# aschneuw/road-segmentation-unet

Measured on AMD Instinct MI355X. Metric: 388x388 patches/sec fwd+bwd (1/2/4/8 GPU) + conv MFMA % of peak, higher is better.
Workload: dtype bf16; 1 GPU; U-Net fwd+bwd+momentum step, num_layers=5 root_size=64 patch_size=388 input=572; batch_per_gpu=4, global_batch=4, parallelism=dp1

## Files before the change

### road_segmentation_unet_amd/_lib.py

```python
import ctypes
import os

_HERE = os.path.dirname(os.path.abspath(__file__))
LIB_PATH = os.environ.get("RSU_LIB_PATH") or os.path.join(_HERE, "librsu_hip.so")

_vp, _i, _l, _f, _sz, _u = ctypes.c_void_p, ctypes.c_int, ctypes.c_long, ctypes.c_float, ctypes.c_size_t, ctypes.c_uint


class RsuSrc(ctypes.Structure):
    _fields_ = [("ptr", _vp), ("H", _i), ("W", _i), ("C", _i), ("oy", _i), ("ox", _i)]


class RsuWgradJob(ctypes.Structure):
    _fields_ = [("kind", _i), ("src", RsuSrc), ("dz", _vp), ("dw", _vp), ("db", _vp), ("Ho", _i), ("Wo", _i),
                ("Cin_total", _i), ("ci_off", _i), ("Cout", _i), ("dil", _i)]


WGRAD_CONV3X3, WGRAD_CONVT2X2, WGRAD_GROUP_MAX = 0, 1, 16


class RsuPlanRow(ctypes.Structure):
    _fields_ = [(n, _i) for n in ("kind", "level", "Hin", "Win", "Cin", "Hout", "Wout", "Cout", "dilation", "nsrc")]


# ... 100 lines not shown
    "rsu_extract_tiles": (_i, [_vp, _vp, _i, _i, _i, _i, _i, _l, _l, _vp]),
    "rsu_overlap_add": (_i, [_vp, _vp, _vp, _i, _i, _i, _i, _l, _l, _vp]),
    "rsu_overlap_finish": (_i, [_vp, _vp, _vp, _l, _vp]),
    "rsu_tile_grid": (_i, [_i, _i, _i, _i, _PI, _PI]),
    "rsu_extract_tiles_rect": (_i, [_vp, _vp, _i, _i, _i, _i, _i, _i, _l, _l, _vp]),
    "rsu_overlap_add_rect": (_i, [_vp, _vp, _vp, _i, _i, _i, _i, _i, _l, _l, _vp]),
    "rsu_affine_patches": (_i, [_vp, _vp, ctypes.POINTER(RsuAffine), _i, _i, _i, _i, _i, _i, _vp, _vp, _vp]),
    "rsu_elastic_patches": (_i, [_vp, _vp, ctypes.POINTER(RsuElastic), _i, _i, _i, _i, _i, _i, _vp, _vp, _vp]),
    "rsu_color_jitter_ws_bytes": (_sz, [_i, _i]),
    "rsu_color_jitter": (_i, [_vp, ctypes.POINTER(RsuJitter), _i, _i, _vp, _vp]),
    "rsu_quantize_mask": (_i, [_vp, _vp, _i, _i, _i, _f, _vp]),
    "rsu_quantize_mask_rect": (_i, [_vp, _vp, _i, _i, _i, _i, _f, _vp]),
    "rsu_labels_for_patches": (_i, [_vp, _vp, _i, _i, _i, _f, _vp]),
    "rsu_confusion_counts": (_i, [_vp, _vp, _l, _vp, _vp]),
    "rsu_plan": (_i, [_i, _i, _i, _i, _i, ctypes.POINTER(RsuPlanRow), _i, _PI, ctypes.POINTER(RsuPlanTotals)]),
}

SIGNATURES_OPTIM = {
    "rsu_update_table_run_decay": (_i, [_vp, _i, _i, _f, _f, _f, _f, _i, _vp, _vp]),
    "rsu_update_table_run_adam_decay": (_i, [_vp, _i, _i, _f, _f, _f, _f, _f, _f, _i, _vp, _vp]),
}

SIGNATURES_LOSS = {
    "rsu_head_fwd_bwd_focal": (_i, [_vp, _vp, _vp, _vp, _vp, _vp, _f, _vp, _f, _f, _vp, _vp, _vp, _vp, _vp, _vp, _vp, _l, _i, _f, _vp]),
    "rsu_head_eval_focal": (_i, [_vp, _vp, _vp, _vp, _vp, _vp, _f, _vp, _vp, _vp, _vp, _l, _i, _vp]),
}

SIGNATURES_CLDICE = {
    "rsu_cldice_ws_floats": (_sz, [_i, _i, _i, _i]),
    "rsu_cldice_fwd": (_i, [_vp, _vp, _i, _vp, _vp, _vp, _vp, _i, _i, _i, _vp]),
    "rsu_cldice_bwd": (_i, [_vp, _vp, _vp, _vp, _vp, _i, _f, _f, _vp, _vp, _i, _i, _i, _vp]),
    "rsu_head_fwd_bwd_aux": (_i, [_vp, _vp, _vp, _vp, _vp, _vp, _f, _vp, _f, _f, _vp, _vp, _vp, _vp, _vp, _vp, _vp, _l, _i, _f, _vp, _vp]),
}

SIGNATURES_LOVASZ = {
    "rsu_lovasz_ws_bytes": (_sz, [_i, _i, _i]),
    "rsu_lovasz_fwd": (_i, [_vp, _vp, _vp, _vp, _i, _i, _i, _vp]),
    "rsu_lovasz_fwd_bwd": (_i, [_vp, _vp, _f, _i, _vp, _vp, _vp, _i, _i, _i, _vp]),
}

SIGNATURES_COMPONENTS = {
    "rsu_components_ws_bytes": (_sz, [_i, _i, _i]),
    "rsu_components_label": (_i, [_vp, _f, _i, _i, _vp, _vp, _vp, _vp, _i, _i, _i, _vp]),
    "rsu_components_filter": (_i, [_vp, _f, _i, _i, _i, _vp, _vp, _vp, _i, _i, _i, _vp]),
    "rsu_components_pair_count": (_i, [_vp, _f, _vp, _i, _vp, _vp, _i, _i, _i, _vp]),
}

SIGNATURES_DISTANCE = {
    "rsu_distance_ws_bytes": (_sz, [_i, _i, _i]),
    "rsu_mask_distance": (_i, [_vp, _f, _vp, _vp, _vp, _vp, _i, _i, _i, _vp]),
    "rsu_distance_hist": (_i, [_vp, _f, _vp, _vp, _vp, _i, _i, _i, _vp]),
}

_lib = None


class RsuError(RuntimeError):
    pass


def lib():
    global _lib
    if _lib is None:
        if not os.path.exists(LIB_PATH):
            raise RsuError("HIP extension missing: %s (build it with `python -c 'import __graft_entry__ as g; g.build()'` "
                           "or `make -C road_segmentation_unet_amd/csrc`); there is no fallback path" % LIB_PATH)
        L = ctypes.CDLL(LIB_PATH)
        for name, (res, args) in list(SIGNATURES.items()) + list(SIGNATURES_OPTIM.items()) + list(SIGNATURES_LOSS.items()) \
                + list(SIGNATURES_CLDICE.items()) + list(SIGNATURES_LOVASZ.items()) + list(SIGNATURES_COMPONENTS.items()) \
                + list(SIGNATURES_DISTANCE.items()):
            fn = getattr(L, name)
            fn.restype = res
            fn.argtypes = args
        _lib = L
    return _lib


TUNE_OFF, TUNE_LOOKUP, TUNE_MEASURE = 0, 1, 2
EVAL_BINS = 256
BORDER_D2_INF, BORDER_MAX_SIDE = 0x7fffffff, 1024
CLIP_STATE_BYTES, CLIP_CLIPPED, CLIP_NONFINITE, GRAD_NORM_BLOCK_FLOATS = 32, 1, 2, 16384
GRAD_ACCUMULATE_BLOCK_FLOATS = 8192
DECAY_L2, DECAY_DECOUPLED = 0, 1
AFFINE_MAX_LAUNCH = 32
ELASTIC_MAX_LAUNCH, ELASTIC_MAX_GRID = 32, 16
JITTER_MAX_LAUNCH = 32
CLDICE_MAX_ITERS = 16
DIST_BINS, DIST_NONE, DIST_MAX_SIDE = 64, 0x7fffffff, 1024
E2BIG = -7


def check(rc, what):
    if rc == E2BIG:
        raise RsuError("%s: a tensor of this call reaches 2 GiB (the kernels address tensors through 32-bit byte offsets): "
                       "use a smaller per-GPU batch" % what)
    if rc != 0:
        raise RsuError("%s failed: rc=%d (hip error %d)" % (what, rc, lib().rsu_last_hip_error()))


_TRACE = os.environ.get("RSU_TRACE", "0") == "1"


def call(name, *args):
    if _TRACE:
        import sys
        import torch
        print("[rsu]", name, [a if isinstance(a, (int, float)) else "." for a in args], file=sys.stderr, flush=True)
        check(getattr(lib(), name)(*args), name)
        torch.cuda.synchronize()
        return
    check(getattr(lib(), name)(*args), name)


_hip = None
_fork_rings = {}


def _hip_runtime():
    global _hip
    if _hip is None:
        path = "libamdhip64.so"
        try:
            with open("/proc/self/maps") as f:
# ... 42 lines not shown
```

### road_segmentation_unet_amd/csrc/conv_first.hip

```cpp
#include "igemm.h"

namespace {
__device__ __forceinline__ unsigned relu_pk(unsigned x) {
    typedef __attribute__((ext_vector_type(2))) short s2;
    return __builtin_bit_cast(unsigned, __builtin_elementwise_max(__builtin_bit_cast(s2, x), s2{0, 0}));
}
}

struct ConvFirstParams {
    const float* x;
    const float* cw;
    const float* cb;
    const bf16_t* in16;
    const bf16_t* wp;
    const float* bias;
    bf16_t* y;
    int N, H, W, Ho, Wo, Cout, dil, relu, ntiles_w;
    int ntx;
    unsigned ntx_magic, ho_magic;
    int npieces;
};

#ifndef CF_TRS
#define CF_TRS 1
#endif
template <bool FUSED>
__global__ void __launch_bounds__(256) __attribute__((amdgpu_waves_per_eu(3))) k_conv_first_fwd(const ConvFirstParams p) {
#if CF_TRS
    __shared__ __attribute__((aligned(16))) char trs[4 * 2048];
#endif
    const int lane = threadIdx.x & 63, l15 = lane & 15, g4 = lane >> 4;
    const int wave = __builtin_amdgcn_readfirstlane((int)(blockIdx.x * 4 + (threadIdx.x >> 6)));
    const int nwaves = gridDim.x * 4;
    const int cb = blockIdx.y;
    const __amdgpu_buffer_rsrc_t rin = __builtin_amdgcn_make_buffer_rsrc((void*)p.in16, 0, (int)((long)p.N * p.H * p.W * 32), 0x00020000);
    const __amdgpu_buffer_rsrc_t rout = __builtin_amdgcn_make_buffer_rsrc((void*)p.y, 0, 0x7fffffff, 0x00020000);
    bf16x8 fa[5][4];
#pragma unroll
    for (int j = 0; j < 5; ++j) {
        const int tap = 2 * j + (g4 >> 1);
#pragma unroll
        for (int ct = 0; ct < 4; ++ct) {
            const int tile = cb * 4 + ct;
            bf16x8 v = {0, 0, 0, 0, 0, 0, 0, 0};
            if (tap < 9 && tile < p.ntiles_w) v = *(const bf16x8*)(p.wp + ((long)(tap * p.ntiles_w + tile) * 64 + l15 + 16 * (g4 & 1)) * 8);
            fa[j][ct] = v;
        }
    }
    f32x4 binit[4];
#pragma unroll
    for (int ct = 0; ct < 4; ++ct)
#pragma unroll
        for (int i = 0; i < 4; ++i) {
            const int co = cb * 64 + (ct >> 1) * 32 + 8 * g4 + (ct & 1) * 4 + i;
            binit[ct][i] = (p.bias && co < p.Cout) ? p.bias[co] : 0.f;
        }
    unsigned voff[5];
#pragma unroll
    for (int j = 0; j < 5; ++j) {
        const int tap = min(2 * j + (g4 >> 1), 8), ky = tap / 3, kx = tap - 3 * ky;
        voff[j] = (unsigned)((((ky * p.W + kx) * p.dil + l15) * 16 + 8 * (g4 & 1)) * 2);
    }
    auto decode = [&](int t, int& n, int& y, int& x0) {
        unsigned row = __umulhi((unsigned)t, p.ntx_magic);
        int xt = t - (int)row * p.ntx;
        if (xt >= p.ntx) { ++row; xt -= p.ntx; }
        unsigned nn = __umulhi(row, p.ho_magic);
        int yy = (int)row - (int)nn * p.Ho;
        if (yy >= p.Ho) { ++nn; yy -= p.Ho; }
        n = (int)nn; y = yy; x0 = xt * 16;
    };
    typedef __attribute__((ext_vector_type(3))) float f32x3;
    const __amdgpu_buffer_rsrc_t rx = __builtin_amdgcn_make_buffer_rsrc((void*)p.x, 0, FUSED ? (int)((long)p.N * p.H * p.W * 12) : 0, 0x00020000);
    unsigned xoff[5];
#pragma unroll
    for (int j = 0; j < 5; ++j) {
        const int tap = min(2 * j + (g4 >> 1), 8), ky = tap / 3, kx = tap - 3 * ky;
        xoff[j] = (g4 & 1) ? 0x80000000u : (unsigned)(((ky * p.W + kx) * p.dil + l15) * 12);
    }
    auto load = [&](int t, bf16x8 (&fb)[5]) {
        int n, y, x0;
        decode(t, n, y, x0);
        if constexpr (FUSED) {
            const unsigned soff = (unsigned)(((long)(n * p.H + y) * p.W + x0) * 12);
#pragma unroll
            for (int j = 0; j < 5; ++j) {
                const f32x3 v = __builtin_bit_cast(f32x3, __builtin_amdgcn_raw_buffer_load_b96(rx, xoff[j], soff, 0));
                fb[j] = __builtin_bit_cast(bf16x8, f32x4{v[0], v[1], v[2], 0.f});
            }
// ... 15 lines not shown
#pragma unroll
            for (int j = 0; j < 5; ++j) {
                const f32x4 v = __builtin_bit_cast(f32x4, fb[j]);
                const float xc[3] = {v[0] - 0.5f, v[1] - 0.5f, v[2] - 0.5f};
                float f[3];
#pragma unroll
                for (int c = 0; c < 3; ++c) f[c] = fmaf(xc[2], cw[6 + c], fmaf(xc[1], cw[3 + c], fmaf(xc[0], cw[c], cbias[c])));
                const u32x4 o = {pack_bf2(f[0], f[1]), pack_bf2(f[2], 0.f), 0u, 0u};
                fb[j] = (g4 & 1) ? bf16x8{0, 0, 0, 0, 0, 0, 0, 0} : __builtin_bit_cast(bf16x8, o);
            }
        }
    };
    int t = wave;
    if (t >= p.npieces) return;
    bf16x8 fb[5], fbn[5];
    load(t, fb);
    while (true) {
        const int tn = t + nwaves;
        const bool more = tn < p.npieces;
        load(more ? tn : t, fbn);
        f32x4 acc[4];
#pragma unroll
        for (int ct = 0; ct < 4; ++ct) acc[ct] = binit[ct];
        convert(fb);
#pragma unroll
        for (int j = 0; j < 5; ++j)
#pragma unroll
            for (int ct = 0; ct < 4; ++ct) acc[ct] = __builtin_amdgcn_mfma_f32_16x16x32_bf16(fa[j][ct], fb[j], acc[ct], 0, 0, 0);
        int n, y, x0;
        decode(t, n, y, x0);
        const unsigned sbase = (unsigned)((((long)(n * p.Ho + y) * p.Wo + x0) * p.Cout + cb * 64) * 2);
#if CF_TRS
        {
            __attribute__((address_space(3))) char* wl = (__attribute__((address_space(3))) char*)trs + (threadIdx.x >> 6) * 2048;
#pragma unroll
            for (int pp = 0; pp < 2; ++pp) {
                u32x4 r = {pack_bf2(acc[2 * pp][0], acc[2 * pp][1]), pack_bf2(acc[2 * pp][2], acc[2 * pp][3]),
                           pack_bf2(acc[2 * pp + 1][0], acc[2 * pp + 1][1]), pack_bf2(acc[2 * pp + 1][2], acc[2 * pp + 1][3])};
                if (p.relu) {
#pragma unroll
                    for (int i = 0; i < 4; ++i) r[i] = relu_pk(r[i]);
                }
                *(__attribute__((address_space(3))) u32x4*)(wl + l15 * 128 + (((pp * 4 + g4) ^ (l15 & 7)) << 4)) = r;
            }
            asm volatile("s_waitcnt lgkmcnt(0)" ::: "memory");
            const int q8 = lane & 7;
#pragma unroll
            for (int h = 0; h < 2; ++h) {
                const int P = (lane >> 3) + 8 * h;
                const u32x4 r = *(const __attribute__((address_space(3))) u32x4*)(wl + P * 128 + ((q8 ^ (P & 7)) << 4));
                const bool ok = (x0 + P < p.Wo) && (cb * 64 + q8 * 8 < p.Cout);
                const unsigned vo = ok ? (unsigned)((P * p.Cout + q8 * 8) * 2) : 0x80000000u;
                asm volatile("s_waitcnt lgkmcnt(0)\n\ts_nop 4\n\tbuffer_store_dwordx4 %0, %1, %2, %3 offen\n\ts_nop 3" ::"v"(r), "v"(vo), "s"(rout), "s"(sbase) : "memory");
            }
        }
#else
        const bool pok = x0 + l15 < p.Wo;
#pragma unroll
        for (int pp = 0; pp < 2; ++pp) {
            u32x4 r = {pack_bf2(acc[2 * pp][0], acc[2 * pp][1]), pack_bf2(acc[2 * pp][2], acc[2 * pp][3]),
                       pack_bf2(acc[2 * pp + 1][0], acc[2 * pp + 1][1]), pack_bf2(acc[2 * pp + 1][2], acc[2 * pp + 1][3])};
            if (p.relu) {
#pragma unroll
                for (int i = 0; i < 4; ++i) r[i] = relu_pk(r[i]);
            }
            const bool cok = cb * 64 + pp * 32 + 8 * g4 < p.Cout;
            const unsigned vo = (pok && cok) ? (unsigned)((l15 * p.Cout + pp * 32 + 8 * g4) * 2) : 0x80000000u;
            asm volatile("s_nop 4\n\tbuffer_store_dwordx4 %0, %1, %2, %3 offen\n\ts_nop 3" ::"v"(r), "v"(vo), "s"(rout), "s"(sbase) : "memory");
        }
#endif
        if (!more) break;
        t = tn;
#pragma unroll
        for (int j = 0; j < 5; ++j) fb[j] = fbn[j];
    }
}

static unsigned floor_magic(int d) { return d <= 1 ? 0xffffffffu : (unsigned)(0x100000000ull / (unsigned)d); }

hipError_t conv_first_fwd_launch(const void* in16, const void* wp, int ntiles_w, const float* bias, void* y, int N, int H, int W, int Cout, int dil,
                                 int relu, int ncu, hipStream_t st, const float* x, const float* cw, const float* cb) {
    ConvFirstParams p;
    p.x = x; p.cw = cw; p.cb = cb;
    p.in16 = (const bf16_t*)in16; p.wp = (const bf16_t*)wp; p.bias = bias; p.y = (bf16_t*)y;
    p.N = N; p.H = H; p.W = W; p.Ho = H - 2 * dil; p.Wo = W - 2 * dil; p.Cout = Cout; p.dil = dil; p.relu = relu; p.ntiles_w = ntiles_w;
    p.ntx = (p.Wo + 15) / 16;
    p.ntx_magic = floor_magic(p.ntx);
    p.ho_magic = floor_magic(p.Ho);
    const long np = (long)N * p.Ho * p.ntx;
    if (np >= (1l << 31) / 2 || p.Ho < 1 || p.Wo < 1) return hipErrorInvalidValue;
    p.npieces = (int)np;
    long blocks = (long)ncu * 3;
    if (blocks * 4 > np) blocks = (np + 3) / 4;
    if (x) hipLaunchKernelGGL(k_conv_first_fwd<true>, dim3((unsigned)blocks, (unsigned)((Cout + 63) / 64)), dim3(256), 0, st, p);
    else hipLaunchKernelGGL(k_conv_first_fwd<false>, dim3((unsigned)blocks, (unsigned)((Cout + 63) / 64)), dim3(256), 0, st, p);
    return hipGetLastError();
}
```

### road_segmentation_unet_amd/csrc/igemm.h

```cpp
#pragma once
#include "rsu_common.h"

struct IgSrc {
    const bf16_t* ptr;
    int H, W, C;
    int oy, ox;
};

struct IgFwdParams {
    IgSrc src[3];
    int nsrc;
    int nchunk[3];
    const bf16_t* wp;
    long wp_y_stride;
    int ntiles_w;
    int tile_off;
    const float* bias;
    bf16_t* out;
    const bf16_t* mask_src;
    bf16_t* pool_out;
    unsigned char* pool_code;
    const void* zero_page;
    int N, Hin, Win;
    int Ho, Wo;
    int Cout;
    int outC;
    int dil, stride, pad;
    int oH, oW, ostride;
    int relu, accumulate;
    int ncob;
    int lsw;
    int ksplit, cob_group;
    float* kslab;
    long kslab_stride;
    int dbg;
    unsigned* stamps;
    TileGeo g;
};

struct IgFwdCfgInfo { int TN, TM, threads; };
enum { IGF2_CFG_128x256 = 0, IGF2_CFG_64x512 = 1, IGF2_CFG_128x128 = 2, IGF2_CFG_64x256 = 3, IGF2_CFG_128x192 = 4, IGF2_CFG_64x384 = 5,
       IGF2_CFG_128x320 = 6, IGF2_CFG_64x640 = 7, IGF2_NCFG = 8 };
IgFwdCfgInfo igemm_fwd2_cfg_info(int cfg);
int igemm_fwd2_max_pieces(int cfg, int ntap);
size_t igemm_fwd2_lds_bytes(int cfg, int ntap, int npix_max);
hipError_t igemm_fwd2_launch(int cfg, int ntap, const IgFwdParams& p, int grid_x, int grid_y, hipStream_t st);
hipError_t igemm_pp_launch(int cfg, const IgFwdParams& p, int grid_x, hipStream_t st);
hipError_t igemm_pp_d2_launch(int cfg, const IgFwdParams& p, int grid_x, hipStream_t st);
bool igemm_pp_d2_supports(int cfg, const IgFwdParams& p);
bool igemm_pp_has(int cfg);
bool igemm_pp_has_ksplit(int cfg);
bool igemm_pp_supports(int cfg, const IgFwdParams& p);
int igemm_pp_pool_lsw_mask(int cfg);
size_t igemm_pp_slab_floats(int cfg, const IgFwdParams& p);
hipError_t igemm_pp_finish_launch(int cfg, const IgFwdParams& p, hipStream_t st);

struct IgCtParams {
    const bf16_t* a;
    int Ca;
    int nchunk;
    int N, H, W;
    unsigned magic_hw, magic_w;
    const bf16_t* wp;
    long wp_phase_stride;
    int ntiles_w;
    const float* bias;
    bf16_t* out;
    int outC;
    int Cn;
    const bf16_t* mask_src;
    int ncob, nnb;
};
bool igemm_ct_supports(int mode, int N, int H, int W, int Ca, int Cn);
hipError_t igemm_ct_launch(int mode, const IgCtParams& p, int grid_x, hipStream_t st);
hipError_t conv_first_fwd_launch(const void* in16, const void* wp, int ntiles_w, const float* bias, void* y, int N, int H, int W, int Cout, int dil,
                                 int relu, int ncu, hipStream_t st, const float* x = nullptr, const float* cw = nullptr, const float* cb = nullptr);

struct IgWgradParams {
    const bf16_t* F;
    int Hf, Wf, Cf;
    IgSrc S;
    float* slab;
    float* bslab;
    float* sbslab;
    long slab_stride;
    int CsOut, CfOut, cs_off;
    const void* zero_page;
    int N, dil, stride;
    int nsplit, ntiles_total;
    int lsw;
    int nbuf, nsw;
    int dbg;
    TileGeo g;
};
enum { IGW_CFG_64x64 = 0, IGW_CFG_64x16 = 1, IGW_CFG_128x64 = 2, IGW_NCFG = 3 };
size_t igemm_wgrad_lds_bytes(int cfg, int npix_max, int nbuf);
int igemm_wgrad_nsw(int cfg, int npix_max);
int igemm_wgrad_tmk(int cfg);
int igemm_wgrad_cfb(int cfg);
int igemm_wgrad_csb(int cfg);
int igemm_wgrad_kgroups(int cfg);
hipError_t igemm_wgrad_launch(int cfg, int ntap, const IgWgradParams& p, int grid_x, int grid_y, int grid_z,
                              hipStream_t st);
bool igemm_wgt_supports(int N, int H, int W, int Cin, int Cout);
int igemm_wgt_blocks(int Cin, int Cout);
int igemm_wgt_tiles(int N, int H, int W);
hipError_t igemm_wgt_launch(const void* x, const void* dy, float* slab, float* sbslab, long slab_stride, int N, int H, int W, int Cin, int Cout,
                            int nsplit, hipStream_t st);
bool igemm_wg1_supports(int N, int H, int W, int Cout, int dil);
int igemm_wg1_blocks(int Cout);
int igemm_wg1_tiles(int N, int Ho, int Wo);
hipError_t igemm_wg1_launch(const void* in16, const void* dz, float* slab, float* bslab, long slab_stride, int N, int H, int W, int Cout, int dil,
                            int nsplit, hipStream_t st);
enum { IGW_FAM_WGPP3 = 0, IGW_FAM_WGPP4 = 1, IGW_FAM_WGPP5 = 2, IGW_FAM_WGPP6 = 3, IGW_FAM_WGP64_4 = 4, IGW_FAM_WGP64_5 = 5,
       IGW_FAM_GENERIC = 8  };
#define IGW_GROUP_MAX 16
#define IGW_UNITS_MAX 2048
struct IgWgJob {
    IgWgradParams p;
    int gx, gy, gz;
    int family;
    int pad_;
};
struct IgWgGroupParams {
    int njobs, nwg;
    IgWgJob job[IGW_GROUP_MAX];
    int wg_first[257];
    unsigned unit[IGW_UNITS_MAX];
};
// ... 9 lines not shown
```

### road_segmentation_unet_amd/csrc/igemm_fwd2.hip

```cpp
#include <type_traits>

#include "igemm.h"

#define RSU_WAIT_VMCNT(N) asm volatile("s_waitcnt vmcnt(%0)" ::"n"(N) : "memory")

template <int SPC, int WPS, int NA, int DA, int DW>
__device__ __forceinline__ constexpr int vm_allowed(int j) {
    return SPC == 1 ? WPS + (DA - 1) * (NA + WPS) : (j == 0 ? (DW - 1) * WPS : (DW - 1) * WPS + NA);
}

__device__ __forceinline__ void bdma16(__amdgpu_buffer_rsrc_t rsrc, unsigned voff, unsigned soff, void* lds_wave_base) {
    __builtin_amdgcn_raw_ptr_buffer_load_lds(rsrc, (__attribute__((address_space(3))) void*)lds_wave_base, 16, voff, soff, 0, 0);
}
__device__ __forceinline__ unsigned relu_pk_bf16(unsigned x) {
    typedef __attribute__((ext_vector_type(2))) short s2;
    s2 h = __builtin_bit_cast(s2, x);
    h = __builtin_elementwise_max(h, s2{0, 0});
    return __builtin_bit_cast(unsigned, h);
}
#define RSU_SENT 0x80000000u

template <int WCO, int WPX, int CT, int PT, int NTAP, int KW, int TPS, int NA, int NAB, int DWS>
__global__ void __launch_bounds__(WCO* WPX * 64) __attribute__((amdgpu_waves_per_eu(WCO* WPX / 4, WCO* WPX / 4)))
igemm_fwd2_kernel(const IgFwdParams p) {
    constexpr int NW = WCO * WPX;
    static_assert(NW == 8, "eight waves: two per SIMD");
    constexpr int TN = WCO * CT * 16, TM = WPX * PT * 16;
    constexpr int WT = TN / 16;
    constexpr int SPC = NTAP / TPS;
    constexpr int WBUF = TPS * WT * 1024;
    constexpr int DA = NAB - 1, DW = DWS;
    constexpr int NWB = DW + 1;
    constexpr int WPS = (TPS * WT + NW - 1) / NW;
    constexpr int NST = (CT / 2) * PT;
    static_assert(NTAP % TPS == 0 && (CT % 2) == 0 && SPC <= 3, "bad config");
    static_assert(SPC == 1 || NAB == 2, "deep halo rings only for one-stage-per-chunk kernels");
    static_assert(SPC == 1 ? DW == NAB : (DW >= 2 && DW <= SPC), "weight distance");
    extern __shared__ __attribute__((aligned(16))) char smem[];
    __attribute__((address_space(3))) char* lds = (__attribute__((address_space(3))) char*)smem;
    const int ABUF = p.g.npix_max * 64;
    const int a_base = NWB * WBUF;
    const int dummy_base = a_base + NAB * ABUF;

    const int lane = threadIdx.x & 63;
    const int wave = __builtin_amdgcn_readfirstlane(threadIdx.x >> 6);
    const int wco = wave / WPX, wpx = wave % WPX;
    const int g4 = lane >> 4, l15 = lane & 15;
    const int SW = p.g.SW, CW = p.g.CW, lsw = p.lsw, TR = TM >> lsw;
    const int ph = blockIdx.y;
    const bf16_t* wp = p.wp + (long)ph * p.wp_y_stride;
    const int ooffy = ph >> 1, ooffx = ph & 1;

    int vid = blockIdx.x;
    if (!(p.dbg & 64)) {
        const int q = gridDim.x >> 3, r = gridDim.x & 7, x = vid & 7;
        vid = (x < r ? x * (q + 1) : r * (q + 1) + (x - r) * q) + (vid >> 3);
    }
    const int cob = vid % p.ncob;
    const int tile0 = vid / p.ncob, tstride = gridDim.x / p.ncob;
    const int tpi = p.g.nstrips * p.g.tiles_per_strip;
    const int ntile_m = p.N * tpi;
    const int my_tiles = tile0 < ntile_m ? (ntile_m - tile0 + tstride - 1) / tstride : 0;
    if (my_tiles == 0) return;
    const int nchunks = p.nchunk[0] + p.nchunk[1] + p.nchunk[2];
    const int GC = my_tiles * nchunks;

    struct Tile { int n, x0, y0; };
    auto decode = [&](int k) {
        Tile T;
        int t = tile0 + k * tstride;
        T.n = t / tpi;
        t -= T.n * tpi;
        const int strip = t / p.g.tiles_per_strip;
        T.x0 = strip * SW;
        T.y0 = (t - strip * p.g.tiles_per_strip) * TR;
// ... 75 lines not shown
            a_voff[q] = ok ? (unsigned)(((rr * sW + cc) * sC + kg8) * 2) : RSU_SENT;
        }
    };
    auto issue_a = [&]() {
        const __amdgpu_buffer_rsrc_t rs = mk(a_ptr);
        const int dst = a_base + ia_slot * ABUF;
        ia_slot = ia_slot == NAB - 1 ? 0 : ia_slot + 1;
        if (a_crem >= 32) {
#pragma unroll
            for (int q = 0; q < NA; ++q) {
                const int j = q * NW + wave;
                bdma16(rs, a_voff[q], a_soff, (void*)(lds + (j < npieces ? dst + j * 1024 : dummy_base)));
            }
        } else {
#pragma unroll
            for (int q = 0; q < NA; ++q) {
                const int j = q * NW + wave;
                const int hp = j * 16 + lq;
                const int kg8 = ((lane & 3) ^ ((hp >> 1) & 2)) * 8;
                bdma16(rs, kg8 < a_crem ? a_voff[q] : RSU_SENT, a_soff, (void*)(lds + (j < npieces ? dst + j * 1024 : dummy_base)));
            }
        }
        a_soff += 64;
        a_crem -= 32;
        a_cl = a_cl + 1 == nchunks ? 0 : a_cl + 1;
    };

    const int bias_base = dummy_base + 1024;
    if (threadIdx.x < TN) {
        const int co = cob * TN + threadIdx.x;
        const float bvv = (p.bias && co < p.Cout) ? p.bias[co] : 0.f;
        *(__attribute__((address_space(3))) float*)(lds + bias_base + threadIdx.x * 4) = bvv;
    }
    asm volatile("s_waitcnt vmcnt(0)" ::: "memory");
    __syncthreads();

    auto out_sbase = [&](const Tile& T) {
        return (unsigned)((((long)(T.n * p.oH + T.y0 * p.ostride + ooffy) * p.oW + T.x0 * p.ostride + ooffx) * p.outC + cob * TN +
                           wco * (CT / 2) * 32) * 2);
    };
    auto out_voff = [&](const Tile& T, int e) {
        const int pt = e / (CT / 2), pp = e % (CT / 2);
        const int ml = (wpx * PT + pt) * 16 + l15;
        const int ty = ml >> lsw, tx = ml & (SW - 1);
        const bool pok = (T.y0 + ty < p.Ho) && (T.x0 + tx < p.Wo);
        const int ovoff_pt = ((ty * p.ostride * p.oW + tx * p.ostride) * p.outC + 8 * g4) * 2;
        const int co = cob * TN + (wco * (CT / 2) + pp) * 32 + 8 * g4;
        return (pok && co < p.Cout) ? (unsigned)(ovoff_pt + pp * 64) : RSU_SENT;
    };
    auto epilogue = [&](const Tile& T, f32x4(&acc)[CT][PT]) {
        const __amdgpu_buffer_rsrc_t orsrc = mk(p.out);
        const __amdgpu_buffer_rsrc_t mrsrc = mk(p.mask_src ? (const void*)p.mask_src : (const void*)p.out);
        const unsigned sbase = out_sbase(T);
        if (!p.accumulate) {
            typedef __attribute__((ext_vector_type(2))) short s2;
            const short fl = p.relu ? (short)0 : (short)-32768;
            const s2 floor2 = {fl, fl};
            unsigned ones_pk = 0x00010001u;
            asm volatile("" : "+v"(ones_pk));
            constexpr int MB = NST % 4 == 0 ? 4 : 2;
#pragma unroll
            for (int b0 = 0; b0 < NST; b0 += MB) {
                unsigned voffs[MB];
                u32x4 mk4[MB];
#pragma unroll
                for (int e = 0; e < MB; ++e) {
                    voffs[e] = out_voff(T, b0 + e);
                    if (p.mask_src) mk4[e] = __builtin_amdgcn_raw_buffer_load_b128(mrsrc, voffs[e], sbase, 0);
                }
#pragma unroll
                for (int e = 0; e < MB; ++e) {
                    const int pt = (b0 + e) / (CT / 2), pp = (b0 + e) % (CT / 2);
                    u32x4 r;
#pragma unroll
                    for (int i = 0; i < 2; ++i) {
                        const unsigned lo = pack_bf2(acc[2 * pp][pt][2 * i], acc[2 * pp][pt][2 * i + 1]);
                        const unsigned hi = pack_bf2(acc[2 * pp + 1][pt][2 * i], acc[2 * pp + 1][pt][2 * i + 1]);
                        r[i] = __builtin_bit_cast(unsigned, __builtin_elementwise_max(__builtin_bit_cast(s2, lo), floor2));
                        r[2 + i] = __builtin_bit_cast(unsigned, __builtin_elementwise_max(__builtin_bit_cast(s2, hi), floor2));
                    }
                    if (p.mask_src) {
#pragma unroll
                            for (int i = 0; i < 4; ++i) r[i] &= pos_mask_pk_bf16(mk4[e][i], ones_pk);
                    }
                    asm volatile("buffer_store_dwordx4 %0, %1, %2, %3 offen\n\ts_nop 3" ::"v"(r), "v"(voffs[e]), "s"(orsrc), "s"(sbase) : "memory");
                }
                if (p.mask_src) __builtin_amdgcn_sched_barrier(0);
            }
            return;
        }
        constexpr int EB = NST % 4 == 0 ? 4 : 2;
        static_assert(NST % EB == 0, "epilogue batches");
#pragma unroll
        for (int b0 = 0; b0 < NST; b0 += EB) {
            unsigned voffs[EB];
            u32x4 mk4[EB], ob4[EB];
#pragma unroll
            for (int e = 0; e < EB; ++e) {
                voffs[e] = out_voff(T, b0 + e);
                if (p.mask_src) mk4[e] = __builtin_amdgcn_raw_buffer_load_b128(mrsrc, voffs[e], sbase, 0);
                if (p.accumulate) ob4[e] = __builtin_amdgcn_raw_buffer_load_b128(orsrc, voffs[e], sbase, 0);
            }
#pragma unroll
            for (int e = 0; e < EB; ++e) {
                const int pt = (b0 + e) / (CT / 2), pp = (b0 + e) % (CT / 2);
                float v[8];
#pragma unroll
                for (int i = 0; i < 4; ++i) {
                    v[i] = acc[2 * pp][pt][i];
                    v[4 + i] = acc[2 * pp + 1][pt][i];
                }
                if (p.mask_src) {
#pragma unroll
                    for (int i = 0; i < 4; ++i) {
                        if (!(bf_lo(mk4[e][i]) > 0.f)) v[2 * i] = 0.f;
                        if (!(bf_hi(mk4[e][i]) > 0.f)) v[2 * i + 1] = 0.f;
                    }
                }
                if (p.accumulate) {
#pragma unroll
                    for (int i = 0; i < 4; ++i) {
                        v[2 * i] += bf_lo(ob4[e][i]);
                        v[2 * i + 1] += bf_hi(ob4[e][i]);
                    }
                }
                unsigned r0 = pack_bf2(v[0], v[1]), r1 = pack_bf2(v[2], v[3]), r2 = pack_bf2(v[4], v[5]), r3 = pack_bf2(v[6], v[7]);
                if (p.relu) {
                    r0 = relu_pk_bf16(r0);
                    r1 = relu_pk_bf16(r1);
                    r2 = relu_pk_bf16(r2);
                    r3 = relu_pk_bf16(r3);
                }
                const u32x4 r = {r0, r1, r2, r3};
                asm volatile("buffer_store_dwordx4 %0, %1, %2, %3 offen\n\ts_nop 3" ::"v"(r), "v"(voffs[e]), "s"(orsrc), "s"(sbase)
                             : "memory");
            }
            __builtin_amdgcn_sched_barrier(0);
        }
    };

    Tile ptile = decode(0);
    int pk = 0;
    setup_a(ptile, 0);
    a_next_src = p.nchunk[0];
    bool a_started = false;
    auto issue_a_next = [&]() {
        if (a_cl == 0) {
            if (a_started) {
                ++pk;
                ptile = decode(pk);
                a_si = 0;
                a_next_src = p.nchunk[0];
                setup_a(ptile, 0);
            }
        } else if (a_cl == a_next_src) {
            ++a_si;
            a_next_src += a_si == 1 ? p.nchunk[1] : p.nchunk[2];
            setup_a(ptile, a_si);
        }
        a_started = true;
        issue_a();
    };
    if constexpr (SPC == 1) {
#pragma unroll
        for (int k = -DW; k < 0; ++k) {
            if (k + DA >= 0 && k + DA < GC) issue_a_next();
            if (k + DW < GC) issue_w();
        }
    } else {
        issue_w();
// ... 122 lines not shown
};
template <> struct Fwd2Cfg<IGF2_CFG_128x320> {
    static constexpr int WCO = 2, WPX = 4, CT = 4, PT = 5;
    static constexpr int na(int ntap) { return ntap == 1 ? 3 : 5; }
};
template <> struct Fwd2Cfg<IGF2_CFG_64x640> {
    static constexpr int WCO = 1, WPX = 8, CT = 4, PT = 5;
    static constexpr int na(int ntap) { return ntap == 1 ? 5 : 7; }
};

static constexpr int tps2_for(int TN, int ntap) { return ntap == 9 ? 3 : (ntap == 4 ? (TN <= 64 ? 4 : 2) : 1); }
static constexpr int nab_for(int TN, int ntap) { return ntap / tps2_for(TN, ntap) == 1 ? 4 : 2; }
static constexpr int dws_for(int TN, int ntap, int PT) { return ntap / tps2_for(TN, ntap) == 1 ? nab_for(TN, ntap) : 2; }

IgFwdCfgInfo igemm_fwd2_cfg_info(int cfg) {
    switch (cfg) {
#define CASE(C) \
    case C: return IgFwdCfgInfo{Fwd2Cfg<C>::WCO * Fwd2Cfg<C>::CT * 16, Fwd2Cfg<C>::WPX * Fwd2Cfg<C>::PT * 16, Fwd2Cfg<C>::WCO * Fwd2Cfg<C>::WPX * 64};
        CASE(IGF2_CFG_128x256)
        CASE(IGF2_CFG_64x512)
        CASE(IGF2_CFG_128x128)
        CASE(IGF2_CFG_64x256)
        CASE(IGF2_CFG_128x192)
        CASE(IGF2_CFG_64x384)
        CASE(IGF2_CFG_128x320)
        CASE(IGF2_CFG_64x640)
#undef CASE
    }
    return IgFwdCfgInfo{0, 0, 0};
}
int igemm_fwd2_max_pieces(int cfg, int ntap) {
    switch (cfg) {
#define CASE(C) case C: return Fwd2Cfg<C>::na(ntap) * Fwd2Cfg<C>::WCO * Fwd2Cfg<C>::WPX;
        CASE(IGF2_CFG_128x256)
        CASE(IGF2_CFG_64x512)
        CASE(IGF2_CFG_128x128)
        CASE(IGF2_CFG_64x256)
        CASE(IGF2_CFG_128x192)
        CASE(IGF2_CFG_64x384)
        CASE(IGF2_CFG_128x320)
        CASE(IGF2_CFG_64x640)
#undef CASE
    }
    return 0;
}
size_t igemm_fwd2_lds_bytes(int cfg, int ntap, int npix_max) {
    const IgFwdCfgInfo ci = igemm_fwd2_cfg_info(cfg);
    const int tps = tps2_for(ci.TN, ntap), nab = nab_for(ci.TN, ntap);
    const int pt = ci.TM / 16 / (ci.threads / 64 / (ci.TN / 64));
    const int dws = dws_for(ci.TN, ntap, pt);
    return (size_t)(dws + 1) * tps * (ci.TN / 16) * 1024 + (size_t)nab * npix_max * 64 + 1024 + 512;
}

template <int CFG, int NTAP, int KW>
static hipError_t launch2_one(const IgFwdParams& p, int gx, int gy, hipStream_t st) {
    using C = Fwd2Cfg<CFG>;
    constexpr int TN = C::WCO * C::CT * 16;
    constexpr int TPS = tps2_for(TN, NTAP);
    auto kern = igemm_fwd2_kernel<C::WCO, C::WPX, C::CT, C::PT, NTAP, KW, TPS, C::na(NTAP), nab_for(TN, NTAP), dws_for(TN, NTAP, C::PT)>;
    const size_t lds = igemm_fwd2_lds_bytes(CFG, NTAP, p.g.npix_max);
    static size_t lds_set = 0;
    if (lds > lds_set) {
        hipError_t e = hipFuncSetAttribute((const void*)kern, hipFuncAttributeMaxDynamicSharedMemorySize, (int)lds);
        if (e != hipSuccess) return e;
        lds_set = lds;
    }
    hipLaunchKernelGGL(kern, dim3(gx, gy), dim3(C::WCO * C::WPX * 64), lds, st, p);
    return hipGetLastError();
}
template <int CFG>
static hipError_t launch2_cfg(int ntap, const IgFwdParams& p, int gx, int gy, hipStream_t st) {
    switch (ntap) {
        case 9: return launch2_one<CFG, 9, 3>(p, gx, gy, st);
        case 4: return launch2_one<CFG, 4, 2>(p, gx, gy, st);
        case 1: return launch2_one<CFG, 1, 1>(p, gx, gy, st);
    }
    return hipErrorInvalidValue;
}
hipError_t igemm_fwd2_launch(int cfg, int ntap, const IgFwdParams& p, int gx, int gy, hipStream_t st) {
    switch (cfg) {
        case IGF2_CFG_128x256: return launch2_cfg<IGF2_CFG_128x256>(ntap, p, gx, gy, st);
        case IGF2_CFG_64x512: return launch2_cfg<IGF2_CFG_64x512>(ntap, p, gx, gy, st);
        case IGF2_CFG_128x128: return launch2_cfg<IGF2_CFG_128x128>(ntap, p, gx, gy, st);
        case IGF2_CFG_64x256: return launch2_cfg<IGF2_CFG_64x256>(ntap, p, gx, gy, st);
        case IGF2_CFG_128x192: return launch2_cfg<IGF2_CFG_128x192>(ntap, p, gx, gy, st);
        case IGF2_CFG_64x384: return launch2_cfg<IGF2_CFG_64x384>(ntap, p, gx, gy, st);
        case IGF2_CFG_128x320: return launch2_cfg<IGF2_CFG_128x320>(ntap, p, gx, gy, st);
        case IGF2_CFG_64x640: return launch2_cfg<IGF2_CFG_64x640>(ntap, p, gx, gy, st);
    }
    return hipErrorInvalidValue;
}
```

### road_segmentation_unet_amd/csrc/igemm_pp.hip

```cpp
#include <cstring>
#include <type_traits>

#include "igemm.h"

#ifndef PP_CLIP_PAD
#define PP_CLIP_PAD 1
#endif
#ifndef PP_DIL
#define PP_DIL 1
#endif

#define RSU_WAIT_VMCNT(N) asm volatile("s_waitcnt vmcnt(%0)" ::"n"(N) : "memory")
#define RSU_SENT 0x80000000u

namespace {
__device__ __forceinline__ void bdma16(__amdgpu_buffer_rsrc_t rsrc, unsigned voff, unsigned soff, void* lds_wave_base) {
    __builtin_amdgcn_raw_ptr_buffer_load_lds(rsrc, (__attribute__((address_space(3))) void*)lds_wave_base, 16, voff, soff, 0, 0);
}
__device__ __forceinline__ unsigned relu_pk_bf16(unsigned x) {
    typedef __attribute__((ext_vector_type(2))) short s2;
    s2 h = __builtin_bit_cast(s2, x);
    h = __builtin_elementwise_max(h, s2{0, 0});
    return __builtin_bit_cast(unsigned, h);
}
}

#define PP_NSTAMP 640
namespace {
constexpr int pp_na_slot(int NAW, int k) { return (NAW >> (4 * k)) & 15; }
constexpr int pp_na(int NAW, int g, int j) { return g == 0 ? pp_na_slot(NAW, 2 * j) : (j < 2 ? pp_na_slot(NAW, 2 * j + 1) : 0); }
constexpr int pp_na_first(int NAW, int g, int j) {
    int n = 0;
    for (int k = 0; k < (g == 0 ? 2 * j : 2 * j + 1); ++k) n += pp_na_slot(NAW, k);
    return n;
}
constexpr int pp_na_total(int NAW, int g) { return pp_na(NAW, g, 0) + pp_na(NAW, g, 1) + pp_na(NAW, g, 2); }
constexpr int pp_na_idx(int NAW, int g, int j) {
    int n = 0;
    for (int k = 0; k < j; ++k) n += pp_na(NAW, g, k);
    return n;
}
}
template <int WCO, int WPX, int CT, int PT, int LSW, int NAW, int WP0, bool STAMP, bool DBG, bool POOLK = false, bool KS = false, int DIL = PP_DIL>
__global__ void __launch_bounds__(512) __attribute__((amdgpu_waves_per_eu(2, 2)))
igemm_pp_kernel(const IgFwdParams p) {
    constexpr int NW = 8, NG = 4, KW = 3, TPS = 3;
    static_assert(WCO * WPX == NW, "eight waves: two per SIMD");
    constexpr int TN = WCO * CT * 16, TM = WPX * PT * 16;
    constexpr int WT = TN / 16;
    constexpr int WBUF = TPS * WT * 1024;
    constexpr int NWB = 3, NAB = 2;
    constexpr int WP1 = TPS * WT / 4 - WP0;
    constexpr int WPM = WP1 > WP0 ? WP1 : (WP0 > 0 ? WP0 : 1);
    constexpr int NAV = pp_na_total(NAW, 0) > pp_na_total(NAW, 1) ? pp_na_total(NAW, 0) : pp_na_total(NAW, 1);
    static_assert((WP0 + WP1) * 4 == TPS * WT && WP0 >= 0 && WP1 >= 1, "weight pieces per stage");
    constexpr int NST = (CT / 2) * PT;
    static_assert((CT % 2) == 0, "bad config");
    extern __shared__ __attribute__((aligned(16))) char smem[];
    __attribute__((address_space(3))) char* lds = (__attribute__((address_space(3))) char*)smem;
    constexpr int SW = 1 << LSW, lsw = LSW, TR = TM >> LSW;
    constexpr int CW = (SW + 2 * DIL + 7) / 8 * 8;
    constexpr int NPIX = ((TR + 2 * DIL) * CW + 31) / 32 * 32;
    constexpr int ABUF = NPIX * 64;
    constexpr int ROWB = DIL * CW * 64;
    constexpr int a_base = 0;
    constexpr int WBASE = NAB * ABUF;
    constexpr int dummy_base = WBASE + NWB * WBUF;
    static_assert(ABUF + 2 * ROWB < 65536, "halo offsets must fit the 16-bit offset field of ds_read");

    const int lane = threadIdx.x & 63;
    const int wave = __builtin_amdgcn_readfirstlane(threadIdx.x >> 6);
    const int grp = wave >> 2, w4 = wave & 3;
    const int wco = wave / WPX, wpx = wave % WPX;
    const int g4 = lane >> 4, l15 = lane & 15;

    auto sgpr = [](int v) { return __builtin_amdgcn_readfirstlane(v); };
    int vid = blockIdx.x;
    {
        const int q = gridDim.x >> 3, r = gridDim.x & 7, x = vid & 7;
        vid = (x < r ? x * (q + 1) : r * (q + 1) + (x - r) * q) + (vid >> 3);
    }
    const int ksplit = (KS && p.ksplit > 1) ? p.ksplit : 1;
    const int nck = p.ncob * ksplit;
    const int cgrp = (p.cob_group > 0 && p.cob_group < nck) ? p.cob_group : nck;
    const int tstride = sgpr(gridDim.x / nck);
    const int u_in = vid % cgrp, u_r = vid / cgrp;
    const int unit = sgpr((u_r / tstride) * cgrp + u_in);
    const int tile0 = sgpr(u_r % tstride);
    const int cob = sgpr(unit % p.ncob), ks = KS ? sgpr(unit / p.ncob) : 0;
    const int tpi = p.g.nstrips * p.g.tiles_per_strip;
    const int ntile_m = p.N * tpi;
    const int my_tiles = (unit < nck && tile0 < ntile_m) ? (ntile_m - tile0 + tstride - 1) / tstride : 0;
    if (my_tiles == 0) return;
    const int nchunks = p.nchunk[0] + p.nchunk[1] + p.nchunk[2];
    const int c_lo = KS ? sgpr(ks * nchunks / ksplit) : 0, c_hi = KS ? sgpr((ks + 1) * nchunks / ksplit) : nchunks;
    const int nloc = c_hi - c_lo;
// ... 171 lines not shown
    const int stamp_base = bias_base + 512;
    int stamp_i = 0;
    unsigned long long seg_sum[8] = {0, 0, 0, 0, 0, 0, 0, 0}, seg_t0 = 0;
    auto seg_begin = [&]() {
        if constexpr (STAMP) seg_t0 = __builtin_amdgcn_s_memtime();
    };
    auto seg_end = [&](int k) {
        if constexpr (STAMP) {
            const unsigned long long t = __builtin_amdgcn_s_memtime();
            seg_sum[k] += t - seg_t0;
            seg_t0 = t;
        }
    };
    auto stamp = [&]() {
        if constexpr (STAMP) {
            if (stamp_i < PP_NSTAMP - 10) {
                const unsigned t = (unsigned)__builtin_amdgcn_s_memtime();
                if (lane == 0) *(__attribute__((address_space(3))) unsigned*)(lds + stamp_base + (wave * PP_NSTAMP + stamp_i) * 4) = t;
            }
            ++stamp_i;
        }
    };
    if (threadIdx.x < TN) {
        const int co = cob * TN + threadIdx.x;
        const float bvv = (p.bias && co < p.Cout && ks == 0) ? p.bias[co] : 0.f;
        *(__attribute__((address_space(3))) float*)(lds + bias_base + threadIdx.x * 4) = bvv;
    }
    asm volatile("s_waitcnt vmcnt(0)" ::: "memory");

    auto out_sbase = [&](const Tile& T) {
        return (unsigned)((((long)(T.n * p.oH + T.y0) * p.oW + T.x0) * p.outC + cob * TN + wco * (CT / 2) * 32) * 2);
    };
    auto out_voff = [&](const Tile& T, int e, const int ql15, const int qg4) {
        const int pt = e / (CT / 2), pp = e % (CT / 2);
        const int ml = (wpx * PT + pt) * 16 + ql15;
        const int ty = ml >> lsw, tx = ml & (SW - 1);
        const bool pok = (T.y0 + ty < p.Ho) && (T.x0 + tx < p.Wo);
        const int ovoff_pt = ((ty * p.oW + tx) * p.outC + 8 * qg4) * 2;
        const int co = cob * TN + (wco * (CT / 2) + pp) * 32 + 8 * qg4;
        return (pok && co < p.Cout) ? (unsigned)(ovoff_pt + pp * 64) : RSU_SENT;
    };
#define PP_STORE(R, VOFF) \
    asm volatile("s_nop 4\n\tbuffer_store_dwordx4 %0, %1, %2, %3 offen\n\ts_nop 3" ::"v"(R), "v"(VOFF), "s"(orsrc), "s"(sbase) : "memory")
#define PP_STORE64(R, VOFF) \
    asm volatile("s_nop 4\n\tbuffer_store_dwordx4 %0, %1, %2, %3 offen offset:64\n\ts_nop 3" ::"v"(R), "v"(VOFF), "s"(orsrc), "s"(sbase) : "memory")
    unsigned ovoff[PT];
#pragma unroll
    for (int pt = 0; pt < PT; ++pt) {
        const int ml = (wpx * PT + pt) * 16 + l15;
        const int ty = ml >> lsw, tx = ml & (SW - 1);
        ovoff[pt] = (unsigned)(((ty * p.oW + tx) * p.outC + 8 * g4) * 2);
    }
    const bool co_inside = cob * TN + TN <= p.Cout;
    constexpr bool POOL_OK = POOLK && ((PT == 4 && (LSW == 4 || LSW == 5)) || (PT == 2 && LSW == 4));
    auto pool_body = [&](const Tile& T, f32x4(&acc)[CT][PT], const unsigned (&voffs)[NST], const __amdgpu_buffer_rsrc_t orsrc, const unsigned sbase)
                         __attribute__((always_inline)) {
        typedef __attribute__((ext_vector_type(2))) short s2;
        typedef __attribute__((ext_vector_type(2))) unsigned short us2;
        constexpr int NPAIR = PT / 2, PSTEP = (LSW == 5) ? 2 : 1;
        const int pH = p.oH >> 1, pW = p.oW >> 1;
        const __amdgpu_buffer_rsrc_t prsrc = mk(p.pool_out);
        const __amdgpu_buffer_rsrc_t crsrc = mk(p.pool_code ? (const void*)p.pool_code : (const void*)p.pool_out);
        const unsigned psbase = (unsigned)((((long)(T.n * pH + (T.y0 >> 1)) * pW + (T.x0 >> 1)) * p.outC + cob * TN + wco * (CT / 2) * 32) * 2);
        const short fl = p.relu ? (short)0 : (short)-32768;
        const s2 floor2 = {fl, fl};
        auto pk = [&](int ct2, int pt) {
            u32x4 r;
#pragma unroll
            for (int i = 0; i < 2; ++i) {
                const unsigned lo = pack_bf2(acc[ct2][pt][2 * i], acc[ct2][pt][2 * i + 1]);
                const unsigned hi = pack_bf2(acc[ct2 + 1][pt][2 * i], acc[ct2 + 1][pt][2 * i + 1]);
                r[i] = __builtin_bit_cast(unsigned, __builtin_elementwise_max(__builtin_bit_cast(s2, lo), floor2));
                r[2 + i] = __builtin_bit_cast(unsigned, __builtin_elementwise_max(__builtin_bit_cast(s2, hi), floor2));
            }
            return r;
        };
        auto swap1 = [](unsigned v) { return (unsigned)__builtin_amdgcn_mov_dpp((int)v, 0xB1, 0xF, 0xF, true); };
        auto umin1 = [](unsigned v) {
            const us2 one = {1, 1};
            return __builtin_bit_cast(unsigned, __builtin_elementwise_min(__builtin_bit_cast(us2, v), one));
        };
        auto sub16 = [](unsigned a, unsigned b) { return __builtin_bit_cast(unsigned, (us2)(__builtin_bit_cast(us2, a) - __builtin_bit_cast(us2, b))); };
        auto mul16 = [](unsigned a, unsigned b) { return __builtin_bit_cast(unsigned, (us2)(__builtin_bit_cast(us2, a) * __builtin_bit_cast(us2, b))); };
        auto add16 = [](unsigned a, unsigned b) { return __builtin_bit_cast(unsigned, (us2)(__builtin_bit_cast(us2, a) + __builtin_bit_cast(us2, b))); };
#pragma unroll
        for (int q = 0; q < NPAIR; ++q) {
            const int pa = (LSW == 5) ? q : 2 * q, pb = pa + PSTEP;
            const int ml = (wpx * PT + pa) * 16 + l15;
            const int ty = ml >> lsw, tx = ml & (SW - 1);
            const bool pok = ((l15 & 1) == 0) && (T.y0 + ty < p.Ho) && (T.x0 + tx < p.Wo);
            const unsigned pvoff = (unsigned)((((ty >> 1) * pW + (tx >> 1)) * p.outC + 8 * g4) * 2);
#pragma unroll
            for (int pp = 0; pp < CT / 2; ++pp) {
                const u32x4 ra = pk(2 * pp, pa), rb = pk(2 * pp, pb);
                PP_STORE(ra, voffs[pa * (CT / 2) + pp]);
                PP_STORE(rb, voffs[pb * (CT / 2) + pp]);
                u32x4 pooled;
                unsigned cw[4];
#pragma unroll
                for (int i = 0; i < 4; ++i) {
                    const unsigned v00 = ra[i], v10 = rb[i], v01 = swap1(ra[i]), v11 = swap1(rb[i]);
                    const unsigned mv = __builtin_bit_cast(unsigned, __builtin_elementwise_max(__builtin_bit_cast(s2, v00), __builtin_bit_cast(s2, v10)));
                    const unsigned mh = __builtin_bit_cast(unsigned, __builtin_elementwise_max(__builtin_bit_cast(s2, v01), __builtin_bit_cast(s2, v11)));
                    const unsigned mx = __builtin_bit_cast(unsigned, __builtin_elementwise_max(__builtin_bit_cast(s2, mv), __builtin_bit_cast(s2, mh)));
                    pooled[i] = mx;
                    const unsigned g = umin1(v00) | (umin1(v01) << 1) | (umin1(v10) << 2) | (umin1(v11) << 3);
// ... 5 lines not shown
                const unsigned pv = (pok && cok) ? pvoff + pp * 64 : RSU_SENT;
                asm volatile("s_nop 4\n\tbuffer_store_dwordx4 %0, %1, %2, %3 offen\n\ts_nop 3" ::"v"(pooled), "v"(pv), "s"(prsrc), "s"(psbase) : "memory");
                if (p.pool_code) {
                    u32x2 cd = {__builtin_amdgcn_perm(cw[1], cw[0], 0x06040200u), __builtin_amdgcn_perm(cw[3], cw[2], 0x06040200u)};
                    const unsigned cv = (pok && cok) ? (pvoff + pp * 64) >> 1 : RSU_SENT;
                    asm volatile("s_nop 4\n\tbuffer_store_dwordx2 %0, %1, %2, %3 offen\n\ts_nop 3" ::"v"(cd), "v"(cv), "s"(crsrc), "s"(psbase >> 1) : "memory");
                }
            }
        }
    };
    auto epilogue = [&](const Tile& T, const int tidx, f32x4(&acc)[CT][PT]) {
        if constexpr (KS) {
            const unsigned long long kaddr = (unsigned long long)(p.kslab + (long)ks * p.kslab_stride);
            const __amdgpu_buffer_rsrc_t krsrc = mk((const void*)(((unsigned long long)(unsigned)sgpr((int)(kaddr >> 32)) << 32) | (unsigned)sgpr((int)kaddr)));
            const unsigned kbase = (unsigned)sgpr((((tidx * p.ncob + cob) * NW + wave) * NST) * 2048);
            const unsigned kvoff = (unsigned)lane * 16u;
#pragma unroll
            for (int e = 0; e < NST; ++e) {
                const int pt = e / (CT / 2), pp = e % (CT / 2);
                asm volatile("s_nop 4\n\tbuffer_store_dwordx4 %0, %1, %2, %3 offen\n\ts_nop 3" ::"v"(acc[2 * pp][pt]), "v"(kvoff), "s"(krsrc),
                             "s"(kbase + (unsigned)(e * 2048)) : "memory");
                asm volatile("s_nop 4\n\tbuffer_store_dwordx4 %0, %1, %2, %3 offen\n\ts_nop 3" ::"v"(acc[2 * pp + 1][pt]), "v"(kvoff), "s"(krsrc),
                             "s"(kbase + (unsigned)(e * 2048 + 1024)) : "memory");
            }
            return;
        }
        const __amdgpu_buffer_rsrc_t orsrc = mk(p.out);
        const __amdgpu_buffer_rsrc_t mrsrc = mk(p.mask_src ? (const void*)p.mask_src : (const void*)p.out);
        const unsigned sbase = out_sbase(T);
        const bool inside = co_inside && (T.y0 + TR <= p.Ho) && (T.x0 + SW <= p.Wo);
        {
            typedef __attribute__((ext_vector_type(2))) short s2;
            const short fl = p.relu ? (short)0 : (short)-32768;
            const s2 floor2 = {fl, fl};
            unsigned voffs[NST];
            auto fill_voffs = [&](const bool tr) __attribute__((always_inline)) {
                const int ql15 = tr ? (lane >> 2) : l15, qg4 = tr ? (lane & 3) : g4;
                if (inside) {
#pragma unroll
                    for (int e = 0; e < NST; ++e) {
                        const int pt = e / (CT / 2);
                        unsigned o = ovoff[pt];
                        if (tr) {
                            const int ml = (wpx * PT + pt) * 16 + ql15;
                            o = (unsigned)((((ml >> lsw) * p.oW + (ml & (SW - 1))) * p.outC + 8 * qg4) * 2);
                        }
                        voffs[e] = o + (e % (CT / 2)) * 64;
                    }
                } else {
#pragma unroll
                    for (int e = 0; e < NST; ++e) voffs[e] = out_voff(T, e, ql15, qg4);
                }
            };
            auto body = [&](const bool MASK) __attribute__((always_inline)) {
                const bool TRS = MASK;
                const int tr_src = (((lane & 3) << 4) | (lane >> 2)) << 2;
                fill_voffs(TRS);
                seg_end(6);
                unsigned ones_pk = 0x00010001u;
                asm volatile("" : "+v"(ones_pk));
                u32x4 mk4[NST];
                if (MASK) {
#pragma unroll
                    for (int e = 0; e < NST; ++e)
                        asm volatile("buffer_load_dwordx4 %0, %1, %2, %3 offen" : "=&v"(mk4[e]) : "v"(voffs[e]), "s"(mrsrc), "s"(sbase) : "memory");
                }
                const int LA = TRS ? (NST < 8 ? NST : 8) : 1;
                u32x4 rr[NST];
                auto pack = [&](const int e) __attribute__((always_inline)) {
                    const int pt = e / (CT / 2), pp = e % (CT / 2);
                    unsigned q[4];
#pragma unroll
                    for (int i = 0; i < 2; ++i) {
                        const unsigned lo = pack_bf2(acc[2 * pp][pt][2 * i], acc[2 * pp][pt][2 * i + 1]);
                        const unsigned hi = pack_bf2(acc[2 * pp + 1][pt][2 * i], acc[2 * pp + 1][pt][2 * i + 1]);
                        q[i] = __builtin_bit_cast(unsigned, __builtin_elementwise_max(__builtin_bit_cast(s2, lo), floor2));
                        q[2 + i] = __builtin_bit_cast(unsigned, __builtin_elementwise_max(__builtin_bit_cast(s2, hi), floor2));
                    }
                    if (TRS) {
#pragma unroll
                        for (int i = 0; i < 4; ++i) asm volatile("ds_bpermute_b32 %0, %1, %2" : "=v"(q[i]) : "v"(tr_src), "v"(q[i]));
                    }
                    rr[e] = u32x4{q[0], q[1], q[2], q[3]};
                };
#pragma unroll
                for (int e = 0; e < NST; ++e) {
                    if (e == 0) {
#pragma unroll
                        for (int k = 0; k < LA; ++k) pack(k);
                        if (MASK) {
                            asm volatile("s_waitcnt vmcnt(0)" ::: "memory");
#pragma unroll
                            for (int k = 0; k < NST; ++k) asm volatile("" : "+v"(mk4[k]));
                        }
                    } else if (e + LA - 1 < NST) {
                        pack(e + LA - 1);
                    }
                    u32x4 r = rr[e];
                    if (TRS) {
                        const int ahead = (e + LA < NST ? e + LA : NST) - e - 1;
                        asm volatile("s_waitcnt lgkmcnt(%1)" : "+v"(r) : "n"(4 * ahead < 15 ? 4 * ahead : 15));
                    }
                    if (MASK) {
#pragma unroll
                        for (int i = 0; i < 4; ++i) r[i] &= pos_mask_pk_bf16(mk4[e][i], ones_pk);
                    }
                    if (DBG && (p.dbg & 512)) {
                        asm volatile("" ::"v"(r));
                    } else {
                        PP_STORE(r, voffs[e]);
                    }
                }
            };
            if constexpr (POOL_OK) {
                if (p.pool_out) {
                    fill_voffs(false);
                    pool_body(T, acc, voffs, orsrc, sbase);
                    return;
                }
            }
            if (p.mask_src) body(true); else body(false);
            return;
        }
    };
    auto bar = [&]() {
        asm volatile("" ::: "memory");
        __builtin_amdgcn_s_barrier();
        asm volatile("" ::: "memory");
    };

    setup_a(ptile, src_lo, coff_lo);
    a_next_src = next_rel;
    a_begin();
    if (!(DBG && (p.dbg & 2))) {
        if (grp) {
            a_pieces(std::integral_constant<int, 1>{}, std::integral_constant<int, 0>{});
            a_pieces(std::integral_constant<int, 1>{}, std::integral_constant<int, 1>{});
        } else {
            a_pieces(std::integral_constant<int, 0>{}, std::integral_constant<int, 0>{});
            a_pieces(std::integral_constant<int, 0>{}, std::integral_constant<int, 1>{});
            a_pieces(std::integral_constant<int, 0>{}, std::integral_constant<int, 2>{});
        }
    }
    a_end();
    if (!(DBG && (p.dbg & 1))) {
        if (grp) {
            issue_w(std::integral_constant<int, 1>{}, 0);
            issue_w(std::integral_constant<int, 1>{}, 1);
        } else {
            issue_w(std::integral_constant<int, 0>{}, 0);
            issue_w(std::integral_constant<int, 0>{}, 1);
        }
    }
    asm volatile("s_waitcnt vmcnt(0) lgkmcnt(0)" ::: "memory");
    bar();
    if (grp) bar();

    unsigned long long clk0 = 0, rt0 = 0;
    if constexpr (STAMP) {
        clk0 = __builtin_amdgcn_s_memtime();
        rt0 = __builtin_amdgcn_s_memrealtime();
    }
    f32x4 acc[CT][PT];
    auto run_stream = [&](auto gconst) {
        constexpr int G = decltype(gconst)::value;
        int c = 0;
        int ck = 0;
        Pos cpos = split(tile0);
        Tile ctile = tile_at(cpos);
        bf16x8 fa[TPS][CT], fb[TPS][PT];
        auto bias_init = [&]() {
            if (!(DBG && (p.dbg & 16))) {
                const unsigned baddr = (unsigned)(bias_base + (wco * (CT / 2) * 32 + 8 * g4) * 4);
#pragma unroll
                for (int ct = 0; ct < CT; ++ct)
#pragma unroll
                    for (int pt = 0; pt < PT; ++pt)
                        asm volatile("ds_read_b128 %0, %1 offset:%2" : "=v"(acc[ct][pt]) : "v"(baddr), "n"(((ct >> 1) * 32 + (ct & 1) * 4) * 4) : "memory");
            }
        };
        auto r_reads = [&](auto parc, auto jc) {
            constexpr int PAR = decltype(parc)::value, J = decltype(jc)::value;
            seg_begin();
            if (!(DBG && (p.dbg & 32))) {
#pragma unroll
                for (int tl = 0; tl < TPS; ++tl) {
#pragma unroll
                    for (int ct = 0; ct < CT; ++ct)
                        fa[tl][ct] = *(const __attribute__((address_space(3))) bf16x8*)(lds + afrag + J * WBUF + (tl * WT + ct) * 1024);
#pragma unroll
                    for (int pt = 0; pt < PT; ++pt)
                        fb[tl][pt] = *(const __attribute__((address_space(3))) bf16x8*)(lds + boff[pt][tl] + (a_base + PAR * ABUF + J * ROWB));
                }
            }
            seg_end(3);
        };
        auto r_issue = [&](auto jc, const bool after_epi) {
            constexpr int J = decltype(jc)::value;
            if constexpr (pp_na(NAW, G, J) > 0 || J == 0) {
                if (!(DBG && (p.dbg & 2))) {
                    if constexpr (J == 0) {
                        a_begin();
                        seg_end(7);
                    }
                    a_pieces(gconst, jc);
                }
            }
            if constexpr (J == 2) a_end();
            if constexpr ((G ? WP1 : WP0) > 0) {
                if (!(DBG && (p.dbg & 1))) issue_w(gconst, (J + 2) % NWB);
            }
            seg_end(4);
            if constexpr (G == 1) {
                if (J == 0 && after_epi) {
                    RSU_WAIT_VMCNT(pp_na(NAW, 1, J) + WP1 + NST);
                } else {
                    RSU_WAIT_VMCNT(pp_na(NAW, 1, J) + WP1);
                }
            }
        };
        auto r_part = [&](auto parc, auto jc, const bool after_epi) {
            r_reads(parc, jc);
            r_issue(jc, after_epi);
            asm volatile("s_waitcnt lgkmcnt(0)" ::: "memory");
            seg_end(5);
        };
        auto m_part = [&](auto jc, const bool after_epi, const bool last_of_tile) {
            constexpr int J = decltype(jc)::value;
            __builtin_amdgcn_sched_barrier(0);
            __builtin_amdgcn_s_setprio(1);
            if (!(DBG && (p.dbg & 32)))
#pragma unroll
            for (int tl = 0; tl < TPS; ++tl)
#pragma unroll
                for (int pt = 0; pt < PT; ++pt)
#pragma unroll
                    for (int ct = 0; ct < CT; ++ct) mfma_bf16_inplace(acc[ct][pt], fa[tl][ct], fb[tl][pt]);
            __builtin_amdgcn_s_setprio(0);
            __builtin_amdgcn_sched_barrier(0);
            if constexpr (G == 0) {
                if (J == 0 && after_epi) {
                    RSU_WAIT_VMCNT(pp_na(NAW, 0, J) + WP0 + NST);
                } else if (J == 2) {
                    RSU_WAIT_VMCNT(WP0);
                } else {
                    RSU_WAIT_VMCNT(pp_na(NAW, 0, J) + WP0);
                }
            }
            if (J == 2 && last_of_tile) mfma_results_fence();
        };
        auto chunk = [&](auto parc, int gc) {
            constexpr int PAR = decltype(parc)::value;
            const bool after_epi = (c == 0) && gc > 0;
            const bool last_of_tile = c == nloc - 1;
            if (!(G == 0 && after_epi)) {
                seg_begin();
                if (c == 0) bias_init();
                seg_end(2);
                r_part(parc, std::integral_constant<int, 0>{}, after_epi);
                stamp();
                bar();
                stamp();
            }
            m_part(std::integral_constant<int, 0>{}, after_epi, last_of_tile);
            stamp();
            bar();
            stamp();
            r_part(parc, std::integral_constant<int, 1>{}, false);
            stamp();
            bar();
            stamp();
            m_part(std::integral_constant<int, 1>{}, false, last_of_tile);
            stamp();
            bar();
            stamp();
            r_part(parc, std::integral_constant<int, 2>{}, false);
            stamp();
            bar();
            stamp();
            m_part(std::integral_constant<int, 2>{}, false, last_of_tile);
            stamp();
            bar();
            stamp();
            if (last_of_tile) {
                const bool more = ck + 1 < my_tiles;
                if constexpr (G == 0) {
                    if (more) r_issue(std::integral_constant<int, 0>{}, false);
                    stamp();
                    bar();
                    stamp();
                }
                seg_begin();
                if (!(DBG && (p.dbg & 8))) epilogue(ctile, KS ? (cpos.n * p.g.nstrips + cpos.strip) * p.g.tiles_per_strip + cpos.row : 0, acc);
                seg_end(0);
                if constexpr (G == 0) {
// ... 6 lines not shown
#pragma unroll
                        for (int tl = 0; tl < TPS; ++tl) {
#pragma unroll
                            for (int ct = 0; ct < CT; ++ct) fa[tl][ct] = bf16x8{0, 0, 0, 0, 0, 0, 0, 0};
#pragma unroll
                            for (int pt = 0; pt < PT; ++pt) fb[tl][pt] = bf16x8{0, 0, 0, 0, 0, 0, 0, 0};
                        }
                    }
                }
                stamp();
                bar();
                stamp();
                c = 0;
                ++ck;
                if (ck < my_tiles && !(DBG && (p.dbg & 64))) {
                    advance(cpos);
                    ctile = tile_at(cpos);
                }
                seg_end(1);
            } else {
                ++c;
            }
        };
        for (int gc = 0; gc < GC; gc += 2) {
            chunk(std::integral_constant<int, 0>{}, gc);
            if (gc + 1 >= GC) break;
            chunk(std::integral_constant<int, 1>{}, gc + 1);
        }
    };
    if (grp) run_stream(std::integral_constant<int, 1>{}); else run_stream(std::integral_constant<int, 0>{});
    asm volatile("s_waitcnt vmcnt(0)" ::: "memory");
    if constexpr (STAMP) {
        if (p.stamps) {
            asm volatile("s_waitcnt vmcnt(0) lgkmcnt(0)" ::: "memory");
            const unsigned dclk = (unsigned)(__builtin_amdgcn_s_memtime() - clk0), drt = (unsigned)(__builtin_amdgcn_s_memrealtime() - rt0);
            for (int i = lane; i < PP_NSTAMP; i += 64)
                p.stamps[((long)blockIdx.x * NW + wave) * PP_NSTAMP + i] =
                    i == PP_NSTAMP - 2 ? dclk : (i == PP_NSTAMP - 1 ? drt :
                    (i >= PP_NSTAMP - 10 && i < PP_NSTAMP - 2) ? (unsigned)seg_sum[i - (PP_NSTAMP - 10)] :
                    (i < stamp_i ? *(__attribute__((address_space(3))) unsigned*)(lds + stamp_base + (wave * PP_NSTAMP + i) * 4) : 0u));
        }
    }
}

#if PP_DIL == 1
struct PpFinishParams {
    const float* slab;
    long slice_stride;
    int ksplit, nslots, ncob;
    int WCO, WPX, CT, PT, lsw, TR;
    int nstrips, tiles_per_strip;
    bf16_t* out;
    const bf16_t* mask_src;
    int Ho, Wo, oH, oW, outC, Cout, relu;
};
__global__ void __launch_bounds__(256) k_pp_splitk_finish(const PpFinishParams q) {
    const int NST = (q.CT / 2) * q.PT, TN = q.WCO * q.CT * 16;
    const long idx = (long)blockIdx.x * 256 + threadIdx.x;
    const int lane = (int)(idx & 63);
    long r = idx >> 6;
    const int e = (int)(r % NST); r /= NST;
    const int wave = (int)(r & 7); r >>= 3;
    const int slot = (int)r;
    if (slot >= q.nslots) return;
    const float* src = q.slab + ((long)(slot * 8 + wave) * NST + e) * 512 + lane * 4;
    f32x4 a = *(const f32x4*)src, b = *(const f32x4*)(src + 256);
    for (int z = 1; z < q.ksplit; ++z) {
        const float* sz = src + (long)z * q.slice_stride;
        a += *(const f32x4*)sz;
        b += *(const f32x4*)(sz + 256);
    }
    const int cob = slot % q.ncob, t = slot / q.ncob;
    const int tpi = q.nstrips * q.tiles_per_strip;
    const int n = t / tpi, tr = t - n * tpi;
    const int strip = tr / q.tiles_per_strip, row = tr - strip * q.tiles_per_strip;
    const int wco = wave / q.WPX, wpx = wave % q.WPX;
    const int pt = e / (q.CT / 2), pp = e % (q.CT / 2);
    const int g4 = lane >> 4, l15 = lane & 15;
    const int ml = (wpx * q.PT + pt) * 16 + l15;
    const int SW = 1 << q.lsw;
    const int y = row * q.TR + (ml >> q.lsw), x = strip * SW + (ml & (SW - 1));
    const int co = cob * TN + (wco * (q.CT / 2) + pp) * 32 + 8 * g4;
    if (y >= q.Ho || x >= q.Wo || co >= q.Cout) return;
    typedef __attribute__((ext_vector_type(2))) short s2;
    const short fl = q.relu ? (short)0 : (short)-32768;
    const s2 floor2 = {fl, fl};
    auto pk = [&](float lo, float hi) {
        return __builtin_bit_cast(unsigned, __builtin_elementwise_max(__builtin_bit_cast(s2, pack_bf2(lo, hi)), floor2));
    };
    u32x4 v = {pk(a[0], a[1]), pk(a[2], a[3]), pk(b[0], b[1]), pk(b[2], b[3])};
    const long off = (((long)n * q.oH + y) * q.oW + x) * q.outC + co;
    if (q.mask_src) {
        const u32x4 m = *(const u32x4*)(q.mask_src + off);
#pragma unroll
        for (int i = 0; i < 4; ++i) v[i] &= pos_mask_pk_bf16(m[i]);
    }
    *(u32x4*)(q.out + off) = v;
}

#endif
template <int CFG> struct PpCfg;
#define PP_NAS(a, b, c, d, e) ((a) | ((b) << 4) | ((c) << 8) | ((d) << 12) | ((e) << 16))
template <> struct PpCfg<IGF2_CFG_128x256> { static constexpr int WCO = 2, WPX = 4, CT = 4, PT = 4, NAS = PP_NAS(0, 2, 3, 1, 2), WP0 = 2; };
template <> struct PpCfg<IGF2_CFG_64x512> { static constexpr int WCO = 1, WPX = 8, CT = 4, PT = 4, NAS = PP_NAS(0, 4, 4, 2, 2), WP0 = 0; };
template <> struct PpCfg<IGF2_CFG_128x128> { static constexpr int WCO = 2, WPX = 4, CT = 4, PT = 2, NAS = PP_NAS(0, 1, 2, 1, 2), WP0 = 2; };
template <> struct PpCfg<IGF2_CFG_64x256> { static constexpr int WCO = 1, WPX = 8, CT = 4, PT = 2, NAS = PP_NAS(0, 2, 3, 1, 2), WP0 = 0; };
template <> struct PpCfg<IGF2_CFG_128x192> { static constexpr int WCO = 2, WPX = 4, CT = 4, PT = 3, NAS = PP_NAS(0, 2, 3, 1, 2), WP0 = 2; };
template <> struct PpCfg<IGF2_CFG_64x384> { static constexpr int WCO = 1, WPX = 8, CT = 4, PT = 3, NAS = PP_NAS(0, 3, 3, 2, 2), WP0 = 0; };
template <int WCO, int WPX, int CT, int PT, int LSW, int NAS, int WP0, bool STAMP, bool DBG, bool POOLK = false, bool KS = false>
static hipError_t pp_launch_kernel3(int cfg, const IgFwdParams& p, int gx, hipStream_t st) {
    auto kern = igemm_pp_kernel<WCO, WPX, CT, PT, LSW, NAS, WP0, STAMP, DBG, POOLK, KS, PP_DIL>;
    const size_t lds = igemm_fwd2_lds_bytes(cfg, 9, p.g.npix_max) + (STAMP ? 8 * PP_NSTAMP * 4 : 0);
    static size_t lds_set = 0;
    if (lds > lds_set) {
        hipError_t e = hipFuncSetAttribute((const void*)kern, hipFuncAttributeMaxDynamicSharedMemorySize, (int)lds);
        if (e != hipSuccess) return e;
        lds_set = lds;
    }
    hipLaunchKernelGGL(kern, dim3(gx, 1), dim3(512), lds, st, p);
    return hipGetLastError();
}
template <int WCO, int WPX, int CT, int PT, int LSW, int NAS, int WP0, bool STAMP, bool DBG>
static hipError_t pp_launch_kernel2(int cfg, const IgFwdParams& p, int gx, hipStream_t st) {
    if constexpr (PP_DIL == 1 && !STAMP && !DBG && ((PT == 4 && (LSW == 4 || LSW == 5)) || (PT == 2 && LSW == 4))) {
        if (p.pool_out) return pp_launch_kernel3<WCO, WPX, CT, PT, LSW, NAS, WP0, false, false, true>(cfg, p, gx, st);
    }
    if (p.pool_out) return hipErrorInvalidValue;
    if (p.ksplit > 1) {
        if constexpr (!STAMP && !DBG && WCO == 2) {
            if (!p.kslab) return hipErrorInvalidValue;
            return pp_launch_kernel3<WCO, WPX, CT, PT, LSW, NAS, WP0, false, false, false, true>(cfg, p, gx, st);
        }
        return hipErrorInvalidValue;
    }
    return pp_launch_kernel3<WCO, WPX, CT, PT, LSW, NAS, WP0, STAMP, DBG, false>(cfg, p, gx, st);
}
constexpr bool pp_geo_ok(int TM, int LSW, int NAS) {
    const int SW = 1 << LSW, TR = TM >> LSW;
    if (TR < 1 || TR * SW != TM) return false;
    const int CW = (SW + 2 * PP_DIL + 7) / 8 * 8, NPIX = ((TR + 2 * PP_DIL) * CW + 31) / 32 * 32;
    int pieces = 0;
    for (int k = 0; k < 5; ++k) pieces += pp_na_slot(NAS, k);
    return NPIX <= pieces * 4 * 16 && NPIX * 64 + 2 * PP_DIL * CW * 64 < 65536;
}
template <int WCO, int WPX, int CT, int PT, int NAS, int WP0, bool STAMP, bool DBG = false>
static hipError_t pp_launch_kernel(int cfg, const IgFwdParams& p, int gx, hipStream_t st) {
    constexpr int TM = WPX * PT * 16;
    const int SW = 1 << p.lsw, TR = TM >> p.lsw;
    const int CW = (SW + 2 * PP_DIL + 7) / 8 * 8, NPIX = ((TR + 2 * PP_DIL) * CW + 31) / 32 * 32;
    if (p.dil != PP_DIL || p.g.SW != SW || p.g.CW != CW || p.g.npix_max != NPIX || TR < 1) return hipErrorInvalidValue;
    switch (p.lsw) {
        case 3: if constexpr (pp_geo_ok(TM, 3, NAS)) return pp_launch_kernel2<WCO, WPX, CT, PT, 3, NAS, WP0, STAMP, DBG>(cfg, p, gx, st); break;
        case 4: if constexpr (pp_geo_ok(TM, 4, NAS)) return pp_launch_kernel2<WCO, WPX, CT, PT, 4, NAS, WP0, STAMP, DBG>(cfg, p, gx, st); break;
        case 5: if constexpr (pp_geo_ok(TM, 5, NAS)) return pp_launch_kernel2<WCO, WPX, CT, PT, 5, NAS, WP0, STAMP, DBG>(cfg, p, gx, st); break;
        case 6: if constexpr (pp_geo_ok(TM, 6, NAS)) return pp_launch_kernel2<WCO, WPX, CT, PT, 6, NAS, WP0, STAMP, DBG>(cfg, p, gx, st); break;
    }
    return hipErrorInvalidValue;
}
template <int CFG, bool STAMP = false, bool DBG = false>
static hipError_t pp_launch_one(const IgFwdParams& p, int gx, hipStream_t st) {
    using C = PpCfg<CFG>;
    return pp_launch_kernel<C::WCO, C::WPX, C::CT, C::PT, C::NAS, C::WP0, STAMP, DBG>(CFG, p, gx, st);
}
#if PP_DIL == 1
bool igemm_pp_has(int cfg) { return cfg >= 0 && cfg < IGF2_NCFG && cfg != IGF2_CFG_128x320 && cfg != IGF2_CFG_64x640; }
#endif
#if PP_DIL == 1
bool igemm_pp_has_ksplit(int cfg) { return cfg == IGF2_CFG_128x256 || cfg == IGF2_CFG_128x128 || cfg == IGF2_CFG_128x192; }
#endif
bool igemm_pp_supports(int cfg, const IgFwdParams& p) {
    if (!igemm_pp_has(cfg) || p.stride != 1 || p.ostride != 1 || p.dil != PP_DIL || p.lsw < 3 || p.lsw > 6 || p.accumulate) return false;
    if (p.ksplit > 1 && (!igemm_pp_has_ksplit(cfg) || p.pool_out || !p.kslab)) return false;
    if (p.pool_out && PP_DIL != 1) return false;
    const int TM = igemm_fwd2_cfg_info(cfg).TM;
    const int SW = 1 << p.lsw, TR = TM >> p.lsw;
    const int CW = (SW + 2 * PP_DIL + 7) / 8 * 8, NPIX = ((TR + 2 * PP_DIL) * CW + 31) / 32 * 32;
    if (TR < 1 || p.g.SW != SW || p.g.CW != CW || p.g.npix_max != NPIX) return false;
    int nas = 0;
    switch (cfg) {
#define PP_CASE(C) case C: nas = PpCfg<C>::NAS; break;
        PP_CASE(IGF2_CFG_128x256) PP_CASE(IGF2_CFG_64x512) PP_CASE(IGF2_CFG_128x128) PP_CASE(IGF2_CFG_64x256)
        PP_CASE(IGF2_CFG_128x192) PP_CASE(IGF2_CFG_64x384)
#undef PP_CASE
    }
    return pp_geo_ok(TM, p.lsw, nas);
}
// ... 3 lines not shown
        case IGF2_CFG_128x256: case IGF2_CFG_64x512: return (1 << 4) | (1 << 5);
        case IGF2_CFG_128x128: case IGF2_CFG_64x256: return 1 << 4;
    }
    return 0;
}
#endif
hipError_t igemm_pp_launch(int cfg, const IgFwdParams& p, int gx, hipStream_t st) {
    if (p.stride != 1 || p.ostride != 1) return hipErrorInvalidValue;
#ifdef RSU_DEV_KERNELS
    if ((p.dbg & 128) && p.stamps) {
        if (cfg == IGF2_CFG_128x256 && (p.dbg & ~128)) return pp_launch_one<IGF2_CFG_128x256, true, true>(p, gx, st);
        if (cfg == IGF2_CFG_128x256) return pp_launch_one<IGF2_CFG_128x256, true>(p, gx, st);
        if (cfg == IGF2_CFG_64x512) return pp_launch_one<IGF2_CFG_64x512, true>(p, gx, st);
    }
    if (p.dbg & (63 | 64 | 256 | 512)) {
        if (cfg == IGF2_CFG_128x256) return pp_launch_one<IGF2_CFG_128x256, false, true>(p, gx, st);
        if (cfg == IGF2_CFG_64x512) return pp_launch_one<IGF2_CFG_64x512, false, true>(p, gx, st);
    }
#endif
    switch (cfg) {
        case IGF2_CFG_128x256: return pp_launch_one<IGF2_CFG_128x256>(p, gx, st);
        case IGF2_CFG_64x512: return pp_launch_one<IGF2_CFG_64x512>(p, gx, st);
        case IGF2_CFG_128x128: return pp_launch_one<IGF2_CFG_128x128>(p, gx, st);
        case IGF2_CFG_64x256: return pp_launch_one<IGF2_CFG_64x256>(p, gx, st);
        case IGF2_CFG_128x192: return pp_launch_one<IGF2_CFG_128x192>(p, gx, st);
        case IGF2_CFG_64x384: return pp_launch_one<IGF2_CFG_64x384>(p, gx, st);
    }
    return hipErrorInvalidValue;
}

#if PP_DIL == 1
static void pp_cfg_dims(int cfg, int& WCO, int& WPX, int& CT, int& PT) {
    WCO = WPX = CT = PT = 0;
    switch (cfg) {
#define PP_CASE(C) case C: WCO = PpCfg<C>::WCO; WPX = PpCfg<C>::WPX; CT = PpCfg<C>::CT; PT = PpCfg<C>::PT; break;
        PP_CASE(IGF2_CFG_128x256) PP_CASE(IGF2_CFG_64x512) PP_CASE(IGF2_CFG_128x128) PP_CASE(IGF2_CFG_64x256)
        PP_CASE(IGF2_CFG_128x192) PP_CASE(IGF2_CFG_64x384)
#undef PP_CASE
    }
}
size_t igemm_pp_slab_floats(int cfg, const IgFwdParams& p) {
    const IgFwdCfgInfo ci = igemm_fwd2_cfg_info(cfg);
    return (size_t)p.N * p.g.nstrips * p.g.tiles_per_strip * p.ncob * ci.TN * ci.TM;
}
hipError_t igemm_pp_finish_launch(int cfg, const IgFwdParams& p, hipStream_t st) {
    PpFinishParams q;
    memset(&q, 0, sizeof(q));
    pp_cfg_dims(cfg, q.WCO, q.WPX, q.CT, q.PT);
    if (!q.CT || p.ksplit < 2 || !p.kslab) return hipErrorInvalidValue;
    q.slab = p.kslab; q.slice_stride = p.kslab_stride; q.ksplit = p.ksplit;
    q.nslots = p.N * p.g.nstrips * p.g.tiles_per_strip * p.ncob; q.ncob = p.ncob;
    q.lsw = p.lsw; q.TR = (q.WPX * q.PT * 16) >> p.lsw;
    q.nstrips = p.g.nstrips; q.tiles_per_strip = p.g.tiles_per_strip;
    q.out = p.out; q.mask_src = p.mask_src;
    q.Ho = p.Ho; q.Wo = p.Wo; q.oH = p.oH; q.oW = p.oW; q.outC = p.outC; q.Cout = p.Cout; q.relu = p.relu;
    const long threads = (long)q.nslots * 8 * (q.CT / 2) * q.PT * 64;
    hipLaunchKernelGGL(k_pp_splitk_finish, dim3((unsigned)((threads + 255) / 256)), dim3(256), 0, st, q);
    return hipGetLastError();
}
#endif
```

### road_segmentation_unet_amd/csrc/rsu_api.hip

```cpp
#include <array>
#include <atomic>
#include <cmath>
#include <cstdlib>
#include <cstring>
#include <algorithm>
#include <cstddef>
#include <map>
#include <mutex>
#include <vector>

#include "../../include/rsu.h"
#include "../../include/rsu_optim.h"
#include "../../include/rsu_loss.h"
#include "../../include/rsu_cldice.h"
#include "../../include/rsu_lovasz.h"
#include "../../include/rsu_components.h"
#include "../../include/rsu_distance.h"
#include "affine_patches.h"
#include "color_jitter.h"
#include "border_map.h"
#include "elementwise.h"
#include "head.h"
#include "cldice.h"
#include "lovasz.h"
#include "components.h"
#include "distance.h"
#include "optim.h"
#include "igemm.h"

static std::atomic<int> g_last_hip_error{0};
static void rsu_set_hip_error(int e) { g_last_hip_error.store(e); }

__device__ uint4 g_zero_page_dev[256];

static const void* zero_page() {
    static void* ptr[64] = {nullptr};
    int dev = 0;
    if (hipGetDevice(&dev) != hipSuccess || dev < 0 || dev >= 64) return nullptr;
    if (!ptr[dev]) {
        void* q = nullptr;
        if (hipGetSymbolAddress(&q, HIP_SYMBOL(g_zero_page_dev)) != hipSuccess) return nullptr;
        ptr[dev] = q;
    }
    return ptr[dev];
}

static inline int cdiv(int a, int b) { return (a + b - 1) / b; }
static inline int rup(int a, int b) { return cdiv(a, b) * b; }
static inline unsigned magic32(int d) { return (unsigned)((0x100000000ull + (unsigned)d - 1) / (unsigned)d); }
static inline int env_int(const char* name, int dflt) {
    const char* s = getenv(name);
    return s ? atoi(s) : dflt;
}

extern "C" const char* rsu_version(void) { return "rsu-hip 0.1 (gfx950)"; }
extern "C" int rsu_last_hip_error(void) { return g_last_hip_error.load(); }
static std::atomic<int> g_cu_budget{256};
extern "C" int rsu_set_cu_budget(int ncu) {
    if (ncu < 32 || ncu > 256) return RSU_EINVAL;
    g_cu_budget.store(ncu);
    return RSU_OK;
}
extern "C" int rsu_get_cu_budget(void) { return g_cu_budget.load(); }
static int launch_ncu(int ncu) {
    if (ncu == 0) return g_cu_budget.load();
    return (ncu < 32 || ncu > 256) ? -1 : ncu;
}
static std::atomic<int> g_autotune{RSU_TUNE_LOOKUP};
static std::mutex g_tune_mutex;
static std::map<std::array<int, 16>, int> g_tuned;
// ... 462 lines not shown
            best.g = g;
            best.ncob = ncob;
            best.grid_x = (int)(workers * ncob);
            best.lsw = lsw;
            best.cost = cost;
            best.ksplit = 1;
            best.cob_group = (ntap == 9 && stride == 1 && dil == 1 && gy == 1) ? pick_cob_group(best.grid_x, ncob, 1, ci.TN, ktot, g.npix_max, nchunks) : 0;
            have = true;
        }
    }
    return have;
}

static bool pp_supports(int cfg, const IgFwdParams& p) { return p.dil == 2 ? igemm_pp_d2_supports(cfg, p) : igemm_pp_supports(cfg, p); }
static bool plan_split(Fwd2Plan& pl, int N, int Ho, int Wo, int Cout, int ktot, size_t kws_floats, int dil = 1) {
    if (kws_floats == 0 || Cout < 128 || env_int("RSU_KSPLIT", 1) == 0 || env_int("RSU_FWD_GEN", 3) < 3 || env_int("RSU_FWD2_CFG", -1) >= 0) return false;
    const int nchunks = ktot / (32 * 9);
    const int cands[2] = {IGF2_CFG_128x256, IGF2_CFG_128x128};
    for (int k = 0; k < 2; ++k) {
        const int cfg = cands[k];
        const IgFwdCfgInfo ci = igemm_fwd2_cfg_info(cfg);
        const long fixed = (long)igemm_fwd2_lds_bytes(cfg, 9, 0);
        const long per_pix = (long)igemm_fwd2_lds_bytes(cfg, 9, 1) - fixed;
        int cap = (int)((160 * 1024 - fixed) / per_pix);
        const int cap2 = igemm_fwd2_max_pieces(cfg, 9) * 16;
        if (cap2 < cap) cap = cap2;
        TileGeo g;
        int lsw = 0;
        if (!plan_geo_aligned(g, lsw, Ho, Wo, ci.TM, 3, 3, dil, 1, cap)) continue;
        const int ncob = cdiv(Cout, ci.TN);
        const long P = (long)N * g.nstrips * g.tiles_per_strip * ncob;
        if (P > 128) continue;
        int S = (int)(256 / P);
        if (S > nchunks / 4) S = nchunks / 4;
        if (S > 16) S = 16;
        if (S < 2) continue;
        if (k == 0 && P * S < 192 && nchunks / 4 > S) continue;
        if ((size_t)S * (size_t)P * ci.TM * ci.TN > kws_floats) continue;
        {
            IgFwdParams t;
            memset(&t, 0, sizeof(t));
            t.stride = t.ostride = 1; t.dil = dil; t.lsw = lsw; t.g = g; t.ksplit = S; t.kslab = (float*)16;
            if (!pp_supports(cfg, t)) continue;
        }
        pl.cfg = cfg; pl.g = g; pl.ncob = ncob; pl.lsw = lsw; pl.ksplit = S;
        pl.grid_x = (int)(P * S);
        pl.cost = ((double)ci.TM * ci.TN * (k ? 1.5 : 1.0) / S + 4096.0) * (double)cdiv((int)(P * S), 256);
        pl.cob_group = pick_cob_group(pl.grid_x, ncob, S, ci.TN, ktot, g.npix_max, nchunks);
        return true;
    }
    return false;
}

static hipError_t launch_persistent(int pp, int cfg, int ntap, const IgFwdParams& p, int gx, int gy, hipStream_t st) {
    if (pp && pp_supports(cfg, p)) {
        hipError_t e = p.dil == 2 ? igemm_pp_d2_launch(cfg, p, gx, st) : igemm_pp_launch(cfg, p, gx, st);
        if (e == hipSuccess && p.ksplit > 1) e = igemm_pp_finish_launch(cfg, p, st);
        return e;
    }
    if (p.ksplit > 1) return hipErrorInvalidValue;
    return igemm_fwd2_launch(cfg, ntap, p, gx, gy, st);
}

static int run_fwd(const rsu_src_t* srcs, int nsrc, const void* wp, long wp_y_stride, int ntiles_w, int tile_off, const float* bias,
                   void* out, const void* mask_src, int N, int Hin, int Win, int Ho, int Wo, int Cout, int outC, int ntap, int kw,
                   int dil, int stride, int pad, int oH, int oW, int ostride, int gy, int relu, int accumulate, int ncu_arg, hipStream_t st,
                   void* pool_out = nullptr, void* pool_code = nullptr, float* kws = nullptr, size_t kws_floats = 0) {
    const int kh = ntap / kw;
    const bool pool = pool_out != nullptr;
    const int ncu = launch_ncu(ncu_arg);
    if (ncu < 0) return RSU_EINVAL;
    const long out_bytes = (long)N * oH * oW * outC * 2;
    const int gen = env_int("RSU_FWD_GEN", 3);
    if (out_bytes >= 0x7ffffff0L) return RSU_E2BIG;
    const bool pp_ok = gen >= 3 && ntap == 9 && stride == 1 && ostride == 1 && gy == 1 && (dil == 1 || (dil == 2 && env_int("RSU_PP_DIL2", 1) != 0));
    for (int i = 0; i < nsrc; ++i)
        if ((long)N * srcs[i].H * srcs[i].W * srcs[i].C * 2 >= 0x7ffffff0L) return RSU_E2BIG;
    Fwd2Plan pl2;
    int ktot = 0;
    for (int i = 0; i < nsrc; ++i) ktot += rup(srcs[i].C, 32) * ntap;
    const int env_cfg = env_int("RSU_FWD2_CFG", -1);
    const int tune_mode = env_int("RSU_AUTOTUNE", 1) != 0 ? g_autotune.load() : RSU_TUNE_OFF;
    const bool tunable = env_cfg < 0 && !accumulate && tune_mode != RSU_TUNE_OFF;
    std::array<int, 16> tkey = {N, Ho, Wo, Cout, outC, ntap, kw, dil, stride, pad, gy, ktot, nsrc,
                                (mask_src ? 1 : 0) | (relu ? 2 : 0) | (bias ? 4 : 0) | (pool ? 8 : 0) | (pool_code ? 16 : 0), ostride, ncu * 8 + gen};
    int tuned_cfg = -1, tuned_pp = -1;
    if (!kws || accumulate) kws_floats = 0;
    Fwd2Plan pls;
    const bool split = pp_ok && !pool && kws_floats > 0 && plan_split(pls, N, Ho, Wo, Cout, ktot, kws_floats, dil);
    bool tune_now = false;
    if (tunable && !split) {
        std::lock_guard<std::mutex> lk(g_tune_mutex);
        auto it = g_tuned.find(tkey);
        if (it != g_tuned.end()) {
            tuned_cfg = it->second & 255;
            tuned_pp = it->second >> 8;
        } else {
            tune_now = tune_mode == RSU_TUNE_MEASURE;
        }
    }
    if (split) {
        pl2 = pls;
    } else if (!plan_fwd2(pl2, ncu, N, Ho, Wo, Cout, ntap, kh, kw, dil, stride, gy, ktot, tuned_cfg >= 0 ? tuned_cfg : env_cfg, pool)) {
        if (tuned_cfg >= 0) {
            std::lock_guard<std::mutex> lk(g_tune_mutex);
            g_tuned.erase(tkey);
            tuned_pp = -1;
        }
        if (!((env_cfg >= 0 || tuned_cfg >= 0) && plan_fwd2(pl2, ncu, N, Ho, Wo, Cout, ntap, kh, kw, dil, stride, gy, ktot, -1, pool)))
            return RSU_EINVAL;
    }
    IgFwdParams p;
    memset(&p, 0, sizeof(p));
    p.nsrc = nsrc;
    for (int i = 0; i < nsrc; ++i) {
        if (!srcs[i].ptr || srcs[i].C % 8) return RSU_EINVAL;
        if (srcs[i].oy < 0 || srcs[i].ox < 0 || srcs[i].oy + Hin > srcs[i].H || srcs[i].ox + Win > srcs[i].W) return RSU_EINVAL;
        p.src[i].ptr = (const bf16_t*)srcs[i].ptr;
        p.src[i].H = srcs[i].H;
        p.src[i].W = srcs[i].W;
        p.src[i].C = srcs[i].C;
        p.src[i].oy = srcs[i].oy;
        p.src[i].ox = srcs[i].ox;
        p.nchunk[i] = cdiv(srcs[i].C, 32);
    }
    p.wp = (const bf16_t*)wp;
    p.wp_y_stride = wp_y_stride;
    p.ntiles_w = ntiles_w;
    p.tile_off = tile_off;
    p.bias = bias;
    p.out = (bf16_t*)out;
    p.mask_src = (const bf16_t*)mask_src;
    p.pool_out = (bf16_t*)pool_out;
    p.pool_code = (unsigned char*)pool_code;
    p.zero_page = zero_page();
    if (!p.zero_page) return RSU_EHIP;
    p.N = N; p.Hin = Hin; p.Win = Win; p.Ho = Ho; p.Wo = Wo;
    p.Cout = Cout; p.outC = outC;
    p.dil = dil; p.stride = stride; p.pad = pad;
    p.oH = oH; p.oW = oW; p.ostride = ostride;
    p.relu = relu; p.accumulate = accumulate;
    {
        const int pp = (pp_ok && !accumulate && igemm_pp_has(pl2.cfg) && (gen >= 4 || tuned_pp != 0 || pool || pl2.ksplit > 1)) ? 1 : 0;
        if (pool && !pp) return RSU_EINVAL;
        auto apply_plan = [&](IgFwdParams& q, const Fwd2Plan& pl) {
            q.ncob = pl.ncob;
            q.g = pl.g;
            q.lsw = pl.lsw;
            q.ksplit = pl.ksplit;
            q.cob_group = pl.cob_group;
            q.kslab = pl.ksplit > 1 ? kws : nullptr;
            q.kslab_stride = pl.ksplit > 1 ? (long)igemm_pp_slab_floats(pl.cfg, q) : 0;
        };
        apply_plan(p, pl2);
        if (p.ksplit > 1 && (!pp || (size_t)p.ksplit * (size_t)p.kslab_stride > kws_floats)) return RSU_EINVAL;
#ifdef RSU_DEV_KERNELS
        p.dbg = env_int("RSU_FWD_DBG", 0);
        if (p.dbg & 128) {
            const char* sp = getenv("RSU_STAMP_PTR");
            p.stamps = sp ? (unsigned*)strtoull(sp, nullptr, 0) : nullptr;
        }
#endif
        if (env_int("RSU_PLAN_DEBUG", 0)) {
            const IgFwdCfgInfo ci = igemm_fwd2_cfg_info(pl2.cfg);
            const long tiles = (long)N * pl2.g.nstrips * pl2.g.tiles_per_strip;
            const long workers = pl2.grid_x / (pl2.ncob * pl2.ksplit);
            const long rounds = (tiles + workers - 1) / workers;
            fprintf(stderr, "[plan fwd2] N%d %dx%d Cout%d ntap%d pad%d: cfg%d TN%d TM%d SW%d strips%d tps%d halo%d tiles%ld grid%d rounds%ld ksplit%d cgrp%d pix_util %.3f total_util %.3f pool%d\n",
                    N, Ho, Wo, Cout, ntap, pad, pl2.cfg, ci.TN, ci.TM, pl2.g.SW, pl2.g.nstrips, pl2.g.tiles_per_strip, pl2.g.npix_max, tiles,
                    pl2.grid_x, rounds, pl2.ksplit, pl2.cob_group, (double)N * Ho * Wo / ((double)tiles * ci.TM),
                    (double)N * Ho * Wo * Cout / ((double)rounds * pl2.grid_x * ci.TM * ci.TN) * pl2.ksplit, pool ? 1 : 0);
        }
        if (tune_now && !split) {
            const int tn_model = igemm_fwd2_cfg_info(pl2.cfg).TN;
            struct EventPair {
                hipEvent_t a = nullptr, b = nullptr;
                ~EventPair() {
                    if (a) (void)hipEventDestroy(a);
                    if (b) (void)hipEventDestroy(b);
                }
            } ev;
            HIP_CHECK_RET(hipEventCreate(&ev.a));
            HIP_CHECK_RET(hipEventCreate(&ev.b));
            const hipEvent_t e0 = ev.a, e1 = ev.b;
            HIP_CHECK_RET(hipDeviceSynchronize());
            float best_ms = 1e30f, model_ms = 1e30f;
            int best_cfg = pl2.cfg | (pp << 8);
            const int model_code = best_cfg;
            for (int cfg = 0; cfg < IGF2_NCFG; ++cfg) {
                if (igemm_fwd2_cfg_info(cfg).TN != tn_model) continue;
                Fwd2Plan pc;
                if (!plan_fwd2(pc, ncu, N, Ho, Wo, Cout, ntap, kh, kw, dil, stride, gy, ktot, cfg, pool)) continue;
                IgFwdParams pt = p;
                apply_plan(pt, pc);
                for (int vpp = 0; vpp < 2; ++vpp) {
                    if (vpp == 1 && !(pp_ok && !accumulate && pp_supports(cfg, pt))) continue;
                    if (vpp == 0 && pool) continue;
                    if (!vpp && gen >= 4 && pp_ok && !accumulate && pp_supports(cfg, pt)) continue;
                    float ms_min = 1e30f;
                    for (int rep = 0; rep < 6; ++rep) {
                        HIP_CHECK_RET(hipEventRecord(e0, st));
                        HIP_CHECK_RET(launch_persistent(vpp, pc.cfg, ntap, pt, pc.grid_x, gy, st));
                        HIP_CHECK_RET(hipEventRecord(e1, st));
                        HIP_CHECK_RET(hipEventSynchronize(e1));
                        float ms = 0.f;
                        HIP_CHECK_RET(hipEventElapsedTime(&ms, e0, e1));
                        if (rep > 0 && ms < ms_min) ms_min = ms;
                    }
                    if (env_int("RSU_PLAN_DEBUG", 0)) fprintf(stderr, "[tune fwd2] cfg%d pp%d %.1f us\n", cfg, vpp, ms_min * 1e3f);
                    const int code = cfg | (vpp << 8);
                    if (code == model_code) model_ms = ms_min;
                    if (ms_min < best_ms) {
                        best_ms = ms_min;
                        best_cfg = code;
                    }
                }
            }
            if (best_ms > 0.97f * model_ms) best_cfg = model_code;
            if (env_int("RSU_PLAN_DEBUG", 0)) fprintf(stderr, "[tune fwd2] model cfg%d pp%d -> measured cfg%d pp%d\n", pl2.cfg, (int)pp, best_cfg & 255, best_cfg >> 8);
            std::lock_guard<std::mutex> lk(g_tune_mutex);
            g_tuned[tkey] = best_cfg;
            return RSU_OK;
        }
        HIP_CHECK_RET(launch_persistent(pp, pl2.cfg, ntap, p, pl2.grid_x, gy, st));
        return RSU_OK;
    }
}

extern "C" size_t rsu_conv_splitk_ws_floats(void) { return (size_t)256 * 128 * 256 + 1024; }
extern "C" int rsu_conv2d_fwd_k(const rsu_src_t* srcs, int nsrc, const void* packed_fwd, const float* bias, void* y, int N, int Hin,
                                int Win, int Cout, int dil, int relu, int ncu, float* kws, size_t kws_floats, rsu_stream_t stream) {
    if (!srcs || nsrc < 1 || nsrc > 3 || !packed_fwd || !y || Cout % 8 || (dil != 1 && dil != 2)) return RSU_EINVAL;
    const int Ho = Hin - 2 * dil, Wo = Win - 2 * dil;
    if (Ho < 1 || Wo < 2) return RSU_EINVAL;
    return run_fwd(srcs, nsrc, packed_fwd, 0, rup(Cout, 128) / 16, 0, bias, y, nullptr, N, Hin, Win, Ho, Wo, Cout, Cout, 9, 3, dil, 1, 0,
                   Ho, Wo, 1, 1, relu, 0, ncu, (hipStream_t)stream, nullptr, nullptr, kws, kws_floats);
}
extern "C" int rsu_conv2d_fwd(const rsu_src_t* srcs, int nsrc, const void* packed_fwd, const float* bias, void* y, int N, int Hin,
                              int Win, int Cout, int dil, int relu, int ncu, rsu_stream_t stream) {
    return rsu_conv2d_fwd_k(srcs, nsrc, packed_fwd, bias, y, N, Hin, Win, Cout, dil, relu, ncu, nullptr, 0, stream);
}

extern "C" int rsu_conv2d_fwd_pool_k(const rsu_src_t* srcs, int nsrc, const void* packed_fwd, const float* bias, void* y, void* pooled, void* code,
                                     int N, int Hin, int Win, int Cout, float keep, unsigned key, int ncu, float* kws, size_t kws_floats, rsu_stream_t stream);
extern "C" int rsu_conv2d_fwd_pool(const rsu_src_t* srcs, int nsrc, const void* packed_fwd, const float* bias, void* y, void* pooled, void* code,
                                   int N, int Hin, int Win, int Cout, float keep, unsigned key, int ncu, rsu_stream_t stream) {
    return rsu_conv2d_fwd_pool_k(srcs, nsrc, packed_fwd, bias, y, pooled, code, N, Hin, Win, Cout, keep, key, ncu, nullptr, 0, stream);
}
extern "C" int rsu_conv2d_fwd_pool_k(const rsu_src_t* srcs, int nsrc, const void* packed_fwd, const float* bias, void* y, void* pooled, void* code,
                                     int N, int Hin, int Win, int Cout, float keep, unsigned key, int ncu, float* kws, size_t kws_floats, rsu_stream_t stream) {
    if (!srcs || nsrc < 1 || nsrc > 3 || !packed_fwd || !y || !pooled || Cout % 8 || !keep_ok(keep)) return RSU_EINVAL;
    const int Ho = Hin - 2, Wo = Win - 2;
    if (Ho < 2 || Wo < 2) return RSU_EINVAL;
    if (code && ((Ho | Wo) & 1)) return RSU_EINVAL;
    const bool even = ((Ho | Wo) & 1) == 0;
    const int fuse = env_int("RSU_POOL_FUSED", 1);
    bool worth = fuse >= 2;
    if (fuse == 1) {
        Fwd2Plan a, b;
        const int n = launch_ncu(ncu), kt = 0;
        int ktot = 0;
        for (int i = 0; i < nsrc; ++i) ktot += rup(srcs[i].C, 32) * 9;
        (void)kt;
        Fwd2Plan sp;
        worth = n > 0 && !(kws && plan_split(sp, N, Ho, Wo, Cout, ktot, kws_floats)) &&
                plan_fwd2(a, n, N, Ho, Wo, Cout, 9, 3, 3, 1, 1, 1, ktot, -1, false) &&
                plan_fwd2(b, n, N, Ho, Wo, Cout, 9, 3, 3, 1, 1, 1, ktot, -1, true) && b.cost <= 1.08 * a.cost;
    }
    if (keep == 1.f && even && worth && env_int("RSU_FWD_GEN", 3) >= 3 && env_int("RSU_FWD2_CFG", -1) < 0) {
        const int rc = run_fwd(srcs, nsrc, packed_fwd, 0, rup(Cout, 128) / 16, 0, bias, y, nullptr, N, Hin, Win, Ho, Wo, Cout, Cout, 9, 3, 1, 1, 0, Ho, Wo,
                               1, 1, 1, 0, ncu, (hipStream_t)stream, pooled, code);
        if (rc != RSU_EINVAL) return rc;
    }
    const int rc = rsu_conv2d_fwd_k(srcs, nsrc, packed_fwd, bias, y, N, Hin, Win, Cout, 1, 1, ncu, kws, kws_floats, stream);
    if (rc != RSU_OK) return rc;
    return rsu_maxpool2x2_fwd_code(y, pooled, code, N, Ho, Wo, Cout, keep, key, stream);
}

extern "C" size_t rsu_packed_first_bytes(int Cout) {
    int seg[1] = {3};
    return rsu_packed_bytes(9, Cout, seg, 1);
}
extern "C" int rsu_pack_conv_first(const float* w, void* packed, int Cout, rsu_stream_t stream) {
    int seg[1] = {3};
    return do_pack(w, packed, 9, Cout, seg, 1, (long)3 * Cout, 1, Cout, 0, (hipStream_t)stream);
}
extern "C" int rsu_conv_first_fwd(const void* in16, const void* packed, const float* b, void* y, int N, int H, int W, int Cout, int dil,
                                  int ncu, rsu_stream_t stream) {
    if (!in16 || !packed || !y || Cout % 8 || H <= 2 * dil || W <= 2 * dil + 1 || (dil != 1 && dil != 2)) return RSU_EINVAL;
    rsu_src_t s;
    s.ptr = in16; s.H = H; s.W = W; s.C = 16; s.oy = 0; s.ox = 0;
    const int Ho = H - 2 * dil, Wo = W - 2 * dil;
    if (env_int("RSU_FIRST_GEN", 1) != 0) {
        const int n = launch_ncu(ncu);
        if (n < 0) return RSU_EINVAL;
        if ((long)N * Ho * Wo * Cout * 2 >= 0x7ffffff0L || (long)N * H * W * 32 >= 0x7ffffff0L) return RSU_E2BIG;
        HIP_CHECK_RET(conv_first_fwd_launch(in16, packed, rup(Cout, 128) / 16, b, y, N, H, W, Cout, dil, 1, n, (hipStream_t)stream));
        return RSU_OK;
    }
    return run_fwd(&s, 1, packed, 0, rup(Cout, 128) / 16, 0, b, y, nullptr, N, H, W, Ho, Wo, Cout, Cout, 9, 3, dil, 1, 0, Ho, Wo, 1, 1, 1, 0,
                   ncu, (hipStream_t)stream);
}

extern "C" int rsu_color_conv_first_fwd(const float* x, const float* w0, const float* b0, const void* packed, const float* b, void* y, int N, int H,
                                        int W, int Cout, int dil, int ncu, rsu_stream_t stream) {
    if (!x || !w0 || !b0 || !packed || !y || Cout % 8 || H <= 2 * dil || W <= 2 * dil + 1 || (dil != 1 && dil != 2)) return RSU_EINVAL;
    const int Ho = H - 2 * dil, Wo = W - 2 * dil;
    const int n = launch_ncu(ncu);
    if (n < 0) return RSU_EINVAL;
    if ((long)N * Ho * Wo * Cout * 2 >= 0x7ffffff0L || (long)N * H * W * 12 >= 0x7ffffff0L) return RSU_E2BIG;
    HIP_CHECK_RET(conv_first_fwd_launch(nullptr, packed, rup(Cout, 128) / 16, b, y, N, H, W, Cout, dil, 1, n, (hipStream_t)stream, x, w0, b0));
    return RSU_OK;
}

extern "C" int rsu_conv2d_bwd_data_k(const void* dz, const void* packed_bwd, void* dx, const void* relu_src, int accumulate, int N, int H,
                                     int W, int Cin_total, int ci_off, int ci_cnt, int Cout, int dil, int ncu, float* kws, size_t kws_floats, rsu_stream_t stream);
extern "C" int rsu_conv2d_bwd_data(const void* dz, const void* packed_bwd, void* dx, const void* relu_src, int accumulate, int N, int H,
                                   int W, int Cin_total, int ci_off, int ci_cnt, int Cout, int dil, int ncu, rsu_stream_t stream) {
    return rsu_conv2d_bwd_data_k(dz, packed_bwd, dx, relu_src, accumulate, N, H, W, Cin_total, ci_off, ci_cnt, Cout, dil, ncu, nullptr, 0, stream);
}
extern "C" int rsu_conv2d_bwd_data_k(const void* dz, const void* packed_bwd, void* dx, const void* relu_src, int accumulate, int N, int H,
                                     int W, int Cin_total, int ci_off, int ci_cnt, int Cout, int dil, int ncu, float* kws, size_t kws_floats, rsu_stream_t stream) {
    if (!dz || !packed_bwd || !dx || Cout % 8 || ci_cnt % 8 || ci_off % 32 || ci_off + ci_cnt > Cin_total || (dil != 1 && dil != 2))
        return RSU_EINVAL;
    const int Hd = H - 2 * dil, Wd = W - 2 * dil;
    if (Hd < 1 || Wd < 1 || W < 2) return RSU_EINVAL;
    rsu_src_t s;
    s.ptr = dz; s.H = Hd; s.W = Wd; s.C = Cout; s.oy = 0; s.ox = 0;
    return run_fwd(&s, 1, packed_bwd, 0, rup(Cin_total, 128) / 16, ci_off / 16, nullptr, dx, relu_src, N, Hd, Wd, H, W, ci_cnt, ci_cnt, 9,
                   3, dil, 1, 2 * dil, H, W, 1, 1, 0, accumulate, ncu, (hipStream_t)stream, nullptr, nullptr, kws, kws_floats);
}

static unsigned magic_floor32(int d) { return d <= 1 ? 0xffffffffu : (unsigned)(0x100000000ull / (unsigned)d); }
static int run_ct(int mode, const void* a, int Ca, int N, int H, int W, const void* wp, long phase_stride, int ntiles_w, const float* bias,
                  void* out, int outC, int Cn, const void* mask_src, int ncu_arg, hipStream_t st) {
    const int ncu = launch_ncu(ncu_arg);
    if (ncu < 0) return RSU_EINVAL;
    IgCtParams p;
    memset(&p, 0, sizeof(p));
    p.a = (const bf16_t*)a;
    p.Ca = Ca;
    p.nchunk = cdiv(Ca, 32);
    p.N = N; p.H = H; p.W = W;
    p.magic_hw = magic_floor32(H * W);
    p.magic_w = magic_floor32(W);
    p.wp = (const bf16_t*)wp;
    p.wp_phase_stride = phase_stride;
    p.ntiles_w = ntiles_w;
    p.bias = bias;
    p.out = (bf16_t*)out;
    p.outC = outC;
    p.Cn = Cn;
    p.mask_src = (const bf16_t*)mask_src;
    p.nnb = cdiv((mode == 0 ? 2 : 1) * Cn, 128);
    p.ncob = (mode == 0 ? 2 : 1) * p.nnb;
    const int ntile_m = cdiv(N * H * W, 256);
    int cols = ncu / p.ncob;
    if (cols < 1) cols = 1;
    if (cols > ntile_m) cols = ntile_m;
    HIP_CHECK_RET(igemm_ct_launch(mode, p, cols * p.ncob, st));
    return RSU_OK;
}

extern "C" int rsu_convT2x2_fwd(const void* x, const void* packed_fwd, const float* bias, void* y, int N, int H, int W, int Cin, int Cout,
                                int ncu, rsu_stream_t stream) {
    if (!x || !packed_fwd || !y || Cin % 8 || Cout % 8 || W < 2) return RSU_EINVAL;
    rsu_src_t s;
    s.ptr = x; s.H = H; s.W = W; s.C = Cin; s.oy = 0; s.ox = 0;
    int seg[1] = {Cin};
    const long per = (long)(rsu_packed_bytes(1, Cout, seg, 1) / 2);
    if (env_int("RSU_CT_GEN", 2) >= 2 && igemm_ct_supports(0, N, H, W, Cin, Cout) && (long)N * 4 * H * W * Cout * 2 < 0x7ffffff0L)
        return run_ct(0, x, Cin, N, H, W, packed_fwd, per, rup(Cout, 128) / 16, bias, y, Cout, Cout, nullptr, ncu, (hipStream_t)stream);
    return run_fwd(&s, 1, packed_fwd, per, rup(Cout, 128) / 16, 0, bias, y, nullptr, N, H, W, H, W, Cout, Cout, 1, 1, 1, 1, 0, 2 * H, 2 * W,
                   2, 4, 0, 0, ncu, (hipStream_t)stream);
}

extern "C" int rsu_convT2x2_bwd_data(const void* dy, const void* packed_bwd, void* dx, const void* relu_src, float out_scale, int N, int H,
                                     int W, int Cin, int Cout, int ncu, rsu_stream_t stream) {
    if (!dy || !packed_bwd || !dx || Cin % 8 || Cout % 8 || W < 2 || !(out_scale > 0.f)) return RSU_EINVAL;
    rsu_src_t s;
    s.ptr = dy; s.H = 2 * H; s.W = 2 * W; s.C = Cout; s.oy = 0; s.ox = 0;
    const bool ct = env_int("RSU_CT_GEN", 2) >= 2 && igemm_ct_supports(1, N, H, W, Cout, Cin) && (long)N * 4 * H * W * Cout * 2 < 0x7ffffff0L;
    const int rc = ct ? run_ct(1, dy, Cout, N, H, W, packed_bwd, 0, rup(Cin, 128) / 16, nullptr, dx, Cin, Cin, relu_src, ncu, (hipStream_t)stream)
// ... 839 lines not shown
```

### road_segmentation_unet_amd/csrc/rsu_common.h

```cpp
#pragma once
#include <hip/hip_runtime.h>
#include <stdint.h>

typedef uint16_t bf16_t;
typedef __attribute__((ext_vector_type(8))) short bf16x8;
typedef __attribute__((ext_vector_type(4))) short bf16x4;
typedef __attribute__((ext_vector_type(4))) float f32x4;
typedef __attribute__((ext_vector_type(4))) unsigned int u32x4;
typedef __attribute__((ext_vector_type(16))) float f32x16;
typedef __attribute__((ext_vector_type(2))) unsigned int u32x2;

#define RSU_LDS_PTR(T, p) ((__attribute__((address_space(3))) T*)(p))

__device__ __forceinline__ float bf2f(bf16_t v) { return __uint_as_float(((uint32_t)v) << 16); }
__device__ __forceinline__ float bf_lo(uint32_t u) { return __uint_as_float(u << 16); }
__device__ __forceinline__ float bf_hi(uint32_t u) { return __uint_as_float(u & 0xffff0000u); }
__device__ __forceinline__ uint32_t pack_bf2(float lo, float hi) {
    typedef __attribute__((ext_vector_type(2))) float f2;
    typedef __attribute__((ext_vector_type(2))) __bf16 b2;
    f2 v = {lo, hi};
    b2 r = __builtin_convertvector(v, b2);
    return __builtin_bit_cast(uint32_t, r);
}
__device__ __forceinline__ bf16_t f2bf(float f) {
    __bf16 r = (__bf16)f;
    return __builtin_bit_cast(bf16_t, r);
}
__device__ __forceinline__ void unpack8(const u32x4 v, float* f) {
#pragma unroll
    for (int i = 0; i < 4; ++i) {
        f[2 * i] = bf_lo(v[i]);
        f[2 * i + 1] = bf_hi(v[i]);
    }
}
__device__ __forceinline__ u32x4 pack8(const float* f) {
    u32x4 r;
#pragma unroll
    for (int i = 0; i < 4; ++i) r[i] = pack_bf2(f[2 * i], f[2 * i + 1]);
    return r;
}

__device__ __forceinline__ unsigned pos_mask_pk_bf16(unsigned m, unsigned  = 0) {
    unsigned t;
    asm("v_pk_sub_i16 %0, 0, %1 clamp\n\tv_pk_ashrrev_i16 %0, 15, %0 op_sel_hi:[0,1]" : "=&v"(t) : "v"(m));
    return t;
}

__device__ __forceinline__ void mfma_bf16_inplace(f32x4& acc, const bf16x8& a, const bf16x8& b) {
    asm volatile("v_mfma_f32_16x16x32_bf16 %0, %1, %2, %0" : "+v"(acc) : "v"(a), "v"(b));
}
__device__ __forceinline__ int xcd_contiguous_id(int hw_id, int total) {
    const int q = total >> 3, r = total & 7, x = hw_id & 7;
    return (x < r ? x * (q + 1) : r * (q + 1) + (x - r) * q) + (hw_id >> 3);
}
__device__ __forceinline__ void mfma_results_fence() { asm volatile("s_nop 15\n\ts_nop 15" ::: "memory"); }

__device__ __forceinline__ void dma16(const void* gsrc, void* lds_wave_base) {
    __builtin_amdgcn_global_load_lds((const __attribute__((address_space(1))) void*)gsrc,
                                     (__attribute__((address_space(3))) void*)lds_wave_base, 16, 0, 0);
}

__device__ __forceinline__ int div_magic(int n, unsigned magic) { return (int)__umulhi((unsigned)n, magic); }

struct TileGeo {
    int SW;
    int nstrips;
    int tiles_per_strip;
    int CW;
    int npix_max;
    unsigned inv_SW, inv_CW;
};

static inline int grid_for(long total, int block, int cap = 256 * 16) {
    long g = (total + block - 1) / block;
    if (g > cap) g = cap;
    if (g < 1) g = 1;
    return (int)g;
}

#define HIP_CHECK_RET(x)                   \
    do {                                     \
        hipError_t e__ = (x);                \
        if (e__ != hipSuccess) {             \
            rsu_set_hip_error((int)e__);     \
            return RSU_EHIP;                 \
        }                                    \
    } while (0)
```

### road_segmentation_unet_amd/hostio.py

```python
import glob
import os

import numpy as np

FOREGROUND_THRESHOLD = .25
IMG_PATCH_SIZE = 16
PIXEL_DEPTH = 255


def img_float_to_uint8(img):
    return (np.asarray(img) * PIXEL_DEPTH).round().astype(np.uint8)


def load(directory):
    from PIL import Image
    out = []
    for path in sorted(glob.glob(os.path.join(directory, '*.png'))):
        a = np.asarray(Image.open(path))
        out.append(a.astype(np.float32) / (65535.0 if a.dtype == np.uint16 else 255.0))
    print("Loaded {} images from {}".format(len(out), directory))
    shapes = sorted({a.shape for a in out})
    if len(shapes) > 1:
        raise ValueError("the images of {} differ in shape ({}): one call handles images of one common shape, put each shape into a "
                         "directory of its own".format(directory, ", ".join("x".join(str(d) for d in sh) for sh in shapes)))
# ... 909 lines not shown
    ys = np.arange(H, dtype=np.int64)[None, :, None]
    above = np.maximum.accumulate(np.where(m, ys, -big), axis=1)
    below = np.minimum.accumulate(np.where(m, ys, big)[:, ::-1], axis=1)[:, ::-1]
    g = np.minimum(ys - above, below - ys)
    sq = np.where(g < big // 2, g * g, big)
    best = sq.copy()
    d = 1
    while d < W and d * d < int(best.max()):
        np.minimum(best[:, :, d:], sq[:, :, :-d] + d * d, out=best[:, :, d:])
        np.minimum(best[:, :, :-d], sq[:, :, d:] + d * d, out=best[:, :, :-d])
        d += 1
    out[live] = best
    return out.astype(np.int32)


def mask_distance(prob, threshold, labels=None):
    p, t, lab = _dist_check(prob, threshold, labels, False)
    pred, true = _dist_masks(p, t, lab)
    return _dist_transform(pred), _dist_transform(true)


_DIST_SQUARES = np.arange(DIST_BINS, dtype=np.int64) ** 2


def distance_bin(d2):
    return np.minimum(np.searchsorted(_DIST_SQUARES, np.asarray(d2, np.int64), side="left"), DIST_BINS - 1).astype(np.int64)


def distance_hist(prob, threshold, labels):
    p, t, lab = _dist_check(prob, threshold, labels, True)
    pred, true = _dist_masks(p, t, lab)
    d2_pred, d2_true = _dist_transform(pred), _dist_transform(true)
    hist = np.zeros((2, DIST_BINS), np.int64)
    hist[0] = np.bincount(distance_bin(d2_true[pred]), minlength=DIST_BINS)
    hist[1] = np.bincount(distance_bin(d2_pred[true]), minlength=DIST_BINS)
    return hist


def relaxed_metrics(hist, slack):
    h = np.asarray(hist)
    if h.shape != (2, DIST_BINS) or h.dtype.kind not in "iu":
        raise ValueError("relaxed_metrics: hist must be an integer array [2, %d], not %s %r" % (DIST_BINS, h.dtype, h.shape))
    if isinstance(slack, bool) or not isinstance(slack, (int, np.integer)) or not 0 <= slack <= DIST_BINS - 2:
        raise ValueError("relaxed_metrics: slack must be an integer in [0, %d], not %r" % (DIST_BINS - 2, slack))
    h = h.astype(np.int64)
    tot = [int(h[0].sum()), int(h[1].sum())]
    precision, recall = [float(int(h[s][:int(slack) + 1].sum())) / max(tot[s], 1) for s in (0, 1)]
    idx = np.arange(DIST_BINS, dtype=np.int64)
    mean = [float(int((h[s] * idx).sum())) / max(tot[s], 1) for s in (0, 1)]
    far = [float(int(h[s][-1])) / max(tot[s], 1) for s in (0, 1)]
    f1 = 2.0 * precision * recall / (precision + recall) if precision + recall > 0.0 else 0.0
    return {"relaxed_precision": precision, "relaxed_recall": recall, "relaxed_f1": f1, "mean_dist_pred": mean[0], "mean_dist_true": mean[1],
            "far_pred": far[0], "far_true": far[1]}
```

### road_segmentation_unet_amd/unet.py

```python
import ctypes
import math
import os

import numpy as np
import torch

from . import _lib
from ._lib import RsuSrc, RsuWgradJob, call
from .optim import (DECAY_MODES, DEFAULT_LR_SCHEDULE, EMA_SUFFIX, LR_SCHEDULES, OPTIMIZERS, OptimizerStep,
                    _PACK_CONV_BWD, _PACK_CONV_FIRST, _PACK_CONV_FWD, _PACK_CONVT_BWD, _PACK_CONVT_FWD, _accumulate_arg, _clip_arg,
                    _decay_args, _ema_arg, _int_arg, _ptr, adam_scalars, clip_scale, ema_decay_at, lr_at)
from .schedule import BackwardSchedule, cu_shares

NUM_CHANNELS = 3
NUM_LABELS = 2


def input_size_needed(output_size, num_layers):
    for i in range(num_layers - 1):
        assert output_size % 2 == 0, 'expand layer {} has size {} not divisible by 2' \
            .format(num_layers - i, output_size)
        output_size = (output_size + 4) / 2
    for i in range(num_layers - 1):
        output_size = (output_size + 4) * 2
# ... 4 lines not shown
    shapes = [("color_space_adjust/kernel", (1, 1, 3, 3)), ("color_space_adjust/bias", (3,))]
    nf, cin = root_size, NUM_CHANNELS
    for i in range(num_layers):
        if dilated_layers:
            shapes += [("conv_dilut_%d/atrous_conv1/kernel" % i, (3, 3, cin, nf)), ("conv_dilut_%d/atrous_conv1/bias" % i, (nf,)),
                       ("conv_dilut_%d/atrous_conv2/kernel" % i, (3, 3, nf, nf)), ("conv_dilut_%d/atrous_conv2/bias" % i, (nf,))]
        shapes += [("conv_%d/conv1/kernel" % i, (3, 3, cin, nf)), ("conv_%d/conv1/bias" % i, (nf,)),
                   ("conv_%d/conv2/kernel" % i, (3, 3, nf, nf)), ("conv_%d/conv2/bias" % i, (nf,))]
        cin = nf
        nf *= 2
    nf //= 2
    for i in range(num_layers - 1):
        nf //= 2
        shapes += [("up_conv_%d/kernel" % i, (2, 2, nf, 2 * nf)), ("up_conv_%d/bias" % i, (nf,))]
        ccat = (3 if dilated_layers else 2) * nf
        j = num_layers + i
        shapes += [("conv_%d/conv1/kernel" % j, (3, 3, ccat, nf)), ("conv_%d/conv1/bias" % j, (nf,)),
                   ("conv_%d/conv2/kernel" % j, (3, 3, nf, nf)), ("conv_%d/conv2/bias" % j, (nf,))]
    shapes += [("weight_output/kernel", (1, 1, nf, NUM_LABELS)), ("weight_output/bias", (NUM_LABELS,))]
    return shapes


def _is_dead(name, num_layers):
    return name.startswith("conv_dilut_%d/" % (num_layers - 1))


def glorot_uniform_params(num_layers, root_size, dilated_layers, seed):
    rng = np.random.RandomState(seed)
    out = {}
    for name, shp in param_shapes(num_layers, root_size, dilated_layers):
        if name.endswith("kernel"):
            recept = shp[0] * shp[1]
            limit = math.sqrt(6.0 / (recept * shp[2] + recept * shp[3]))
            out[name] = rng.uniform(-limit, limit, size=shp).astype(np.float32)
        else:
            out[name] = np.zeros(shp, np.float32)
    return out


def dropout_key_value(seed, site, global_step, micro_step=0):
    return (seed * 0x9E3779B9 + site * 0x85EBCA6B + global_step * 0xC2B2AE35 + micro_step * 0x27D4EB2F) & 0xFFFFFFFF


def _src(t, h, w):
    H, W, C = t.shape[1], t.shape[2], t.shape[3]
    return RsuSrc(t.data_ptr(), H, W, C, (H - h) // 2, (W - w) // 2)


class UNet(OptimizerStep):

    def __init__(self, num_layers, root_size, dilated_layers, batch_size, patch_size, device="cuda:0", params=None, seed=2017,
                 training=True, optimizer="momentum", class_weights=None, dice_weight=0.0, dice_smooth=1.0, border_weight=0.0, border_sigma=5.0,
                 clip_grad_norm=None, ema_decay=None, ema_warmup=True, accumulate_steps=None, weight_decay=None, weight_decay_mode="decoupled",
                 focal_gamma=0.0, cldice_weight=0.0, cldice_iters=10, cldice_smooth=1.0, lovasz_weight=0.0):
        self._init_optimizer(training, optimizer, clip_grad_norm, ema_decay, ema_warmup, accumulate_steps, weight_decay, weight_decay_mode)
        assert root_size % 8 == 0 and (root_size // 8) & (root_size // 8 - 1) == 0, "root_size must be 8 * 2^k for the HIP path"
        self.L, self.root, self.dilated = num_layers, root_size, bool(dilated_layers)
        self.B, self.P = batch_size, patch_size
        self.S = input_size_needed(patch_size, num_layers)
        self.device = torch.device(device)
        if self.device.type == "cuda":
            torch.cuda.set_device(self.device)
        self.training = training
        self.class_weights = class_weights
        self.pixel_weights = None
        self.dice_weight, self.dice_smooth = dice_weight, dice_smooth
        self.focal_gamma = focal_gamma
        self.cldice_weight, self.cldice_iters, self.cldice_smooth = cldice_weight, cldice_iters, cldice_smooth
        if self._cldice_weight > 0.0 and not training:
            raise _lib.RsuError("a forward-only net has no loss to add a clDice term to")
        self.cldice_sums = self.eval_cldice_sums = self.skel_p = self.skel_y = self.gprob = self._cldice_ws = None
        self.lovasz_weight = lovasz_weight
        if self._lovasz_weight > 0.0 and not training:
            raise _lib.RsuError("a forward-only net has no loss to add a Lovasz term to")
        self.lovasz_sum = self.eval_lovasz_sum = self._lovasz_ws = None
        self.border_weight, self.border_sigma = self._border_args(border_weight, border_sigma)
        self.border_map = None
        self.keep = 1.0
        self.dropout_seed = int(seed) if seed is not None else 0
        self.backward_cu_budget = None
        self._tuned = set()
        self.sched = BackwardSchedule(self.device, batch_size, training, self._timed)
        self.wstream = self.wstreams[0] if self.wstreams else None
        self.pool_code = {}
        self.prof = None
        self.on_grads = None
        _lib.lib()
        self._check_tensor_sizes()
        self._alloc_params(params if params is not None else glorot_uniform_params(num_layers, root_size, dilated_layers, seed))
        self._alloc_buffers()
        self.repack()

    @property
    def class_weights(self):
        return self._class_weights

    @class_weights.setter
    def class_weights(self, cw):
        if cw is not None:
            cw = tuple(float(v) for v in cw)
            if len(cw) != 2 or not all(math.isfinite(v) and v >= 0.0 for v in cw) or cw == (0.0, 0.0):
                raise _lib.RsuError("class_weights must be None or two finite floats >= 0, not both 0; got %r" % (cw,))
        self._class_weights = cw
        self._class_w_dev = torch.tensor(cw, dtype=torch.float32, device=self.device) if cw is not None else None

    @property
    def dice_weight(self):
        return self._dice_weight

    @dice_weight.setter
    def dice_weight(self, v):
        try:
            v = float(v)
        except (TypeError, ValueError):
            v = float("nan")
        if not (math.isfinite(v) and v >= 0.0):
# ... 228 lines not shown
        h = h - 4
        for i in range(L - 1):
            nf //= 2
            j = L + i
            self.act["up_%d" % i] = self._bf(B, 2 * h, 2 * h, nf)
            h = 2 * h
            self.act["c1_%d" % j] = self._bf(B, h - 2, h - 2, nf)
            self.act["c2_%d" % j] = self._bf(B, h - 4, h - 4, nf)
            h -= 4
        assert h == self.P, (h, self.P)
        self.last_name = "c2_%d" % (2 * L - 2) if L > 1 else "c2_0"
        self.prob = torch.zeros((B, self.P, self.P), dtype=torch.float32, device=dev)
        self.logits = torch.zeros((B, self.P, self.P, 2), dtype=torch.float32, device=dev)
        self.labels = torch.zeros((B, self.P, self.P), dtype=torch.int64, device=dev)
        self._loss_acc = torch.zeros(2, dtype=torch.float32, device=dev)
        self.loss_sum, self.weight_sum = self._loss_acc[0:1], self._loss_acc[1:2]
        self.dice_sums = torch.zeros(3, dtype=torch.float32, device=dev)
        self.eval_sums = torch.zeros(5, dtype=torch.float32, device=dev)
        self.eval_hist = torch.zeros((2, _lib.EVAL_BINS), dtype=torch.int64, device=dev)
        nk = int(_lib.lib().rsu_conv_splitk_ws_floats()) if os.environ.get("RSU_KSPLIT", "1") != "0" else 0
        self.sched.kws = torch.zeros(nk, dtype=torch.float32, device=dev) if nk else None
        self.sched.kws_side = [torch.zeros(nk, dtype=torch.float32, device=dev) for _ in self.wstreams] if (nk and self.dilated) else []
        if self.training:
            for k, t in self.act.items():
                if k.startswith("up_") or k.startswith("c") or k.startswith("d") or k.startswith("pool_"):
                    self.grad[k] = torch.zeros_like(t)
            for i in range(L - 1):
                up = self.act["up_%d" % i]
                self.grad["skip_%d" % i] = torch.zeros_like(up)
                if self.dilated:
                    self.grad["skipd_%d" % i] = torch.zeros_like(up)
            lib = _lib.lib()
            ws = [lib.rsu_head_ws_floats(B * self.P * self.P, self.root), lib.rsu_head_w_ws_floats(B * self.P * self.P, self.root),
                  lib.rsu_head_dice_ws_floats(B * self.P * self.P, self.root), lib.rsu_head_eval_ws_floats(B * self.P * self.P, self.root),
                  lib.rsu_conv_first_bwd_ws_floats(self.root)]
            for kind, n, s, segs in self._packed_kernels():
                if kind == _PACK_CONV_FWD:
                    for c in segs:
                        ws.append(lib.rsu_conv2d_bwd_weight_ws_floats(s[2], c, s[3]))
                    ws.append(lib.rsu_bias_grad_ws_floats(B * S * S, s[3]))
                elif kind == _PACK_CONVT_FWD:
                    ws.append(lib.rsu_convT2x2_bwd_weight_ws_floats(s[3], s[2]))
            ws.append(lib.rsu_wgrad_group_ws_floats())
            self.ws = torch.zeros(int(max(ws)) + 64, dtype=torch.float32, device=dev)
            self.sched.ws_side = [self.ws] + [torch.zeros_like(self.ws) for _ in self.wstreams[1:]]
            self.gfirst = torch.zeros((2, 9, 12, self.root), dtype=torch.float32, device=dev)
            if self._cldice_weight > 0.0:
                self._cldice_buffers()
            if self._lovasz_weight > 0.0:
                self._lovasz_buffers()
            if self.border_weight > 0.0:
                self.border_map = torch.zeros((B, self.P, self.P), dtype=torch.float32, device=dev)
                self._border_ws = torch.zeros(int(lib.rsu_border_map_ws_bytes(B, self.P, self.P)) // 4, dtype=torch.int32, device=dev)
            if os.environ.get("RSU_POOL_CODE", "1") == "1":
                for i in range(L - 1):
                    self.pool_code[i] = torch.zeros(self.act["pool_%d" % i].shape, dtype=torch.uint8, device=dev)

    def _conv_sources_c(self, name, shape):
        cin, cout = shape[2], shape[3]
        blk = int(name.split("/")[0].split("_")[-1]) if name.startswith("conv_") and not name.startswith("conv_dilut") else -1
        if name.endswith("conv1/kernel") and blk >= self.L:
            return [cout] * (3 if self.dilated else 2)
        return [cin]

    def _packed_kernels(self):
        for n, (_, _, s) in self._slices.items():
            if not n.endswith("kernel") or _is_dead(n, self.L):
                continue
            if n.startswith("up_conv"):
                yield _PACK_CONVT_FWD, n, s, None
            elif s[0] == 3 and s[2] == NUM_CHANNELS:
                yield _PACK_CONV_FIRST, n, s, None
            elif s[0] == 3:
                yield _PACK_CONV_FWD, n, s, self._conv_sources_c(n, s)

    def repack(self):
        lib = _lib.lib()
        st = ctypes.c_void_p(torch.cuda.current_stream(self.device).cuda_stream) if self.device.type == "cuda" else None
        if not hasattr(self, "pk"):
            self.pk = {}
            jobs = []

            def buf(nbytes):
                return torch.zeros(nbytes // 2, dtype=torch.bfloat16, device=self.device)
            for kind, n, s, segs in self._packed_kernels():
                if kind == _PACK_CONVT_FWD:
                    cout, cin = s[2], s[3]
                    self.pk[n, "fwd"] = buf(4 * lib.rsu_packed_bytes(1, cout, (ctypes.c_int * 1)(cin), 1))
                    self.pk[n, "bwd"] = buf(lib.rsu_packed_bytes(4, cin, (ctypes.c_int * 1)(cout), 1))
                    jobs.append((kind, n, self.pk[n, "fwd"], 2, cin, 0, cin, cout, None))
                    if self.training:
                        jobs.append((_PACK_CONVT_BWD, n, self.pk[n, "bwd"], 2, cin, 0, cin, cout, None))
                elif kind == _PACK_CONV_FIRST:
                    self.pk[n, "fwd"] = buf(lib.rsu_packed_first_bytes(s[3]))
                    jobs.append((kind, n, self.pk[n, "fwd"], 3, 3, 0, 3, s[3], None))
                else:
                    cin, cout = s[2], s[3]
                    self.pk[n, "fwd"] = buf(lib.rsu_packed_bytes(9, cout, (ctypes.c_int * len(segs))(*segs), len(segs)))
                    jobs.append((kind, n, self.pk[n, "fwd"], 3, cin, 0, cin, cout, segs))
                    off = 0
                    for si, c in enumerate(segs):
                        self.pk[n, "bwd", si] = buf(lib.rsu_packed_bytes(9, c, (ctypes.c_int * 1)(cout), 1))
                        if self.training:
                            jobs.append((_PACK_CONV_BWD, n, self.pk[n, "bwd", si], 3, cin, off, c, cout, None))
                        off += c
            esz = lib.rsu_pack_table_entry_bytes()
            host = ctypes.create_string_buffer(esz * (len(jobs) + 3 * sum(1 for j in jobs if j[0] == _PACK_CONVT_FWD)))
            idx = 0
            for kind, n, packed, k, cin, off, cnt, cout, segs in jobs:
                seg = (ctypes.c_int * len(segs))(*segs) if segs else None
                used = lib.rsu_pack_table_add(host, idx, kind, _ptr(self.w[n]), _ptr(packed), k, cin, off, cnt, cout, seg, len(segs) if segs else 0)
                if used < 1:
                    raise _lib.RsuError("rsu_pack_table_add(%s) failed: %d" % (n, used))
                idx += used
            nb = ctypes.c_int(0)
            _lib.check(lib.rsu_pack_table_finish(host, idx, ctypes.byref(nb)), "rsu_pack_table_finish")
            self._pack_n, self._pack_blocks = idx, nb.value
            self._pack_table = torch.frombuffer(bytearray(host.raw[:esz * idx]), dtype=torch.uint8).to(self.device)
        call("rsu_pack_table_run", _ptr(self._pack_table), self._pack_n, self._pack_blocks, st)

    def _stream(self):
        return ctypes.c_void_p(torch.cuda.current_stream(self.device).cuda_stream)

    def _timed(self, tag, flops, fn, *args):
        if self.prof is None:
            call(fn, *args)
            return
        e0, e1 = torch.cuda.Event(enable_timing=True), torch.cuda.Event(enable_timing=True)
        e0.record()
        call(fn, *args)
        e1.record()
        self.prof.append((tag, flops, e0, e1, (self.sched.ncu() or _lib.lib().rsu_get_cu_budget()) / 256.0))

    def _grads_ready(self, name):
        if self.on_grads is not None:
            self.sched.flush()
            self.on_grads(self._slices[name][0])

    def _conv(self, name, srcs, hin, out, dil=1):
        arr = (RsuSrc * len(srcs))(*srcs)
        cout = out.shape[3]
        cin = sum(s.C for s in srcs)
        ho = hin - 2 * dil
        kws = self.sched.kws_here()
        nb = out.shape[0]
        self._timed("conv3x3_fwd", 2.0 * nb * ho * ho * cout * cin * 9, "rsu_conv2d_fwd_k", arr, len(srcs),
                    _ptr(self.pk[name + "/kernel", "fwd"]), _ptr(self.w[name + "/bias"]), _ptr(out), nb, hin, hin, cout, dil, 1,
                    self.sched.ncu(), _ptr(kws), kws.numel() if kws is not None else 0, self._stream())

    def _conv_first(self, name, out, h, dil, st, in16=None, x=None):
        if x is not None:
            call("rsu_color_conv_first_fwd", _ptr(x), _ptr(self.w["color_space_adjust/kernel"]), _ptr(self.w["color_space_adjust/bias"]),
                 _ptr(self.pk[name + "/kernel", "fwd"]), _ptr(self.w[name + "/bias"]), _ptr(out), out.shape[0], h, h, self.root, dil,
                 self.sched.ncu(), st)
            return
        call("rsu_conv_first_fwd", _ptr(self.in16 if in16 is None else in16), _ptr(self.pk[name + "/kernel", "fwd"]), _ptr(self.w[name + "/bias"]),
             _ptr(out), out.shape[0], h, h, self.root, dil, self.sched.ncu(), st)

    def dropout_key(self, site):
        return dropout_key_value(self.dropout_seed, site, self.global_step, self.micro_step)

    @property
    def micro_step(self):
        return min(self._accum_calls, self.accumulate_steps - 1)

    def forward_device(self, want_logits=False, keep=1.0):
        keep = float(keep)
        assert 0.0 < keep <= 1.0, "dropout keep probability must be in (0, 1]"
        self.keep = keep
        for f in self._forward_steps(0, self.B, want_logits, keep):
            f()
        return self.act[self.last_name]

    def _forward_steps(self, b0, nb, want_logits, keep):
        L, S = self.L, self.S
        a = {k: t[b0:b0 + nb] for k, t in self.act.items()}
        x, in16, prob, logits = self.x[b0:b0 + nb], self.in16[b0:b0 + nb], self.prob[b0:b0 + nb], self.logits[b0:b0 + nb]
        code = {k: t[b0:b0 + nb] for k, t in self.pool_code.items()}
        steps = []

        def add(f):
            steps.append(f)
        fused_first = keep == 1.0 and not self.training
        xin = x if fused_first else None
        if not fused_first:
            add(lambda: call("rsu_color_adjust_fwd", _ptr(x), _ptr(self.w["color_space_adjust/kernel"]), _ptr(self.w["color_space_adjust/bias"]),
                             _ptr(in16), nb * S * S, keep, self.dropout_key(0), self._stream()))
        cur, h = None, S
        for i in range(L):
            last = i == L - 1
            if self.dilated and not last:
                def twin(i=i, cur=cur, h=h):
                    with self.sched.side():
                        if i == 0:
                            self._conv_first("conv_dilut_0/atrous_conv1", a["d1_0"], h, 2, self._stream(), in16, xin)
                        else:
                            self._conv("conv_dilut_%d/atrous_conv1" % i, [_src(cur, h, h)], h, a["d1_%d" % i], dil=2)
                        self._conv("conv_dilut_%d/atrous_conv2" % i, [_src(a["d1_%d" % i], h - 4, h - 4)], h - 4, a["d2_%d" % i], dil=2)
                add(twin)
            if i == 0:
                add(lambda h=h: self._conv_first("conv_0/conv1", a["c1_0"], h, 1, self._stream(), in16, xin))
            else:
                add(lambda i=i, cur=cur, h=h: self._conv("conv_%d/conv1" % i, [_src(cur, h, h)], h, a["c1_%d" % i]))
            if last:
                add(lambda i=i, h=h: self._conv("conv_%d/conv2" % i, [_src(a["c1_%d" % i], h - 2, h - 2)], h - 2, a["c2_%d" % i]))
            else:
                def conv2_pool(i=i, h=h):
                    c1, c2 = a["c1_%d" % i], a["c2_%d" % i]
                    nf_ = c2.shape[3]
                    src = (RsuSrc * 1)(_src(c1, h - 2, h - 2))
                    kws = self.sched.kws_here()
                    self._timed("conv3x3_fwd", 2.0 * nb * (h - 4) * (h - 4) * nf_ * c1.shape[3] * 9, "rsu_conv2d_fwd_pool_k", src, 1,
                                _ptr(self.pk["conv_%d/conv2/kernel" % i, "fwd"]), _ptr(self.w["conv_%d/conv2/bias" % i]), _ptr(c2),
                                _ptr(a["pool_%d" % i]), _ptr(code.get(i)), nb, h - 2, h - 2, nf_, keep, self.dropout_key(i + 1), self.sched.ncu(),
                                _ptr(kws), kws.numel() if kws is not None else 0, self._stream())
                add(conv2_pool)
                cur, h = a["pool_%d" % i], (h - 4) // 2
        net, h = a["c2_%d" % (L - 1)], h - 4
        if self.dilated:
            add(self.sched.join)
        for i in range(L - 1):
            j, lvl = L + i, L - 2 - i
            up = a["up_%d" % i]
            if keep < 1.0:
                if self.act.get("drop_%d" % i) is None:
                    self.act["drop_%d" % i] = torch.zeros_like(self.act["c2_%d" % (j - 1)] if i > 0 else self.act["c2_%d" % (L - 1)])
                drop = self.act["drop_%d" % i][b0:b0 + nb]
                add(lambda net=net, drop=drop, i=i: call("rsu_dropout_fwd", _ptr(net), _ptr(drop), net.numel(), keep, self.dropout_key(L + i), self._stream()))
                net = drop
            add(lambda net=net, up=up, i=i, h=h: call("rsu_convT2x2_fwd", _ptr(net), _ptr(self.pk["up_conv_%d/kernel" % i, "fwd"]),
                                                     _ptr(self.w["up_conv_%d/bias" % i]), _ptr(up), nb, h, h, net.shape[3], up.shape[3], self.sched.ncu(), self._stream()))
            h = 2 * h

            def dec(j=j, lvl=lvl, up=up, h=h):
                srcs = [_src(a["c2_%d" % lvl], h, h)]
                if self.dilated:
                    srcs.append(_src(a["d2_%d" % lvl], h, h))
                srcs.append(_src(up, h, h))
                self._conv("conv_%d/conv1" % j, srcs, h, a["c1_%d" % j])
            add(dec)
            add(lambda j=j, h=h: self._conv("conv_%d/conv2" % j, [_src(a["c1_%d" % j], h - 2, h - 2)], h - 2, a["c2_%d" % j]))
            net, h = a["c2_%d" % j], h - 4
        if not self.training or want_logits:
            add(lambda net=net: call("rsu_head_fwd", _ptr(net), _ptr(self.w["weight_output/kernel"]), _ptr(self.w["weight_output/bias"]), _ptr(prob),
                                     _ptr(logits) if want_logits else None, nb * self.P * self.P, self.root, self._stream()))
        return steps

    def reset_eval(self):
        self.eval_sums.zero_()
        self.eval_hist.zero_()
        if self.eval_cldice_sums is not None:
            self.eval_cldice_sums.zero_()
        if self.eval_lovasz_sum is not None:
            self.eval_lovasz_sum.zero_()

    def evaluate_device(self):
        if not self.training:
            raise _lib.RsuError("evaluate_device needs a training net (labels and the head's workspace); a forward-only net has no loss")
        if self.keep != 1.0:
            raise _lib.RsuError("evaluate_device follows forward_device(keep=1.0): the activations in flight were made with dropout")
        if self._focal_gamma > 0.0:
            call("rsu_head_eval_focal", _ptr(self.act[self.last_name]), _ptr(self.w["weight_output/kernel"]), _ptr(self.w["weight_output/bias"]),
                 _ptr(self.labels), _ptr(self._class_w_dev), _ptr(self._head_pixel_weights()), self._focal_gamma, _ptr(self.prob),
                 _ptr(self.eval_sums), _ptr(self.eval_hist), _ptr(self.ws), self.B * self.P * self.P, self.root, self._stream())
        else:
            call("rsu_head_eval", _ptr(self.act[self.last_name]), _ptr(self.w["weight_output/kernel"]), _ptr(self.w["weight_output/bias"]),
                 _ptr(self.labels), _ptr(self._class_w_dev), _ptr(self._head_pixel_weights()), _ptr(self.prob), _ptr(self.eval_sums),
                 _ptr(self.eval_hist), _ptr(self.ws), self.B * self.P * self.P, self.root, self._stream())
        if self._cldice_weight > 0.0:
            self._cldice_buffers()
            self._cldice_fwd(self.eval_cldice_sums)
        if self._lovasz_weight > 0.0:
            self._lovasz_buffers()
            call("rsu_lovasz_fwd", _ptr(self.prob), _ptr(self.labels), _ptr(self.eval_lovasz_sum), _ptr(self._lovasz_ws), self.B, self.P,
                 self.P, self._stream())

    def _wgrad(self, name, srcs_t, dz, hout, dil=1, block_done=False):
        cout = dz.shape[3]
        cin_total = self.w[name + "/kernel"].shape[2]
        off = 0
        if self.sched.grouped:
            for t, win in srcs_t:
                db = self.g[name + "/bias"] if off == 0 else None
                job = RsuWgradJob(_lib.WGRAD_CONV3X3, _src(t, win, win), dz.data_ptr(), self.g[name + "/kernel"].data_ptr(),
                                  db.data_ptr() if db is not None else None, hout, hout, cin_total, off, cout, dil)
                self.sched.queue(job, 2.0 * self.B * hout * hout * cout * t.shape[3] * 9, (name, off))
                off += t.shape[3]
            if block_done:
                self.sched.block_done()
            return
        with self.sched.side() as ws:
            st = self._stream()
            for t, win in srcs_t:
                s = _src(t, win, win)
                db = _ptr(self.g[name + "/bias"]) if off == 0 else None
                fl = 2.0 * self.B * hout * hout * cout * t.shape[3] * 9
                self._timed("conv3x3_bwd_weight", fl, "rsu_conv2d_bwd_weight", ctypes.byref(s), _ptr(dz), _ptr(self.g[name + "/kernel"]), db,
                            _ptr(ws), self.B, hout, hout, cin_total, off, cout, dil, self.sched.ncu(), st)
                off += t.shape[3]

    def _wgradT(self, i, upin, dup, hh, nf):
        if self.sched.grouped:
            job = RsuWgradJob(_lib.WGRAD_CONVT2X2, RsuSrc(upin.data_ptr(), hh, hh, upin.shape[3], 0, 0), dup.data_ptr(),
                              self.g["up_conv_%d/kernel" % i].data_ptr(), self.g["up_conv_%d/bias" % i].data_ptr(), 0, 0, 0, 0, nf, 1)
            self.sched.queue(job, 0.0, ("up_conv_%d" % i, upin.data_ptr()), transposed=True)
            return
        with self.sched.side() as ws:
            call("rsu_convT2x2_bwd_weight", _ptr(upin), _ptr(dup), _ptr(self.g["up_conv_%d/kernel" % i]), _ptr(self.g["up_conv_%d/bias" % i]),
                 _ptr(ws), self.B, hh, hh, upin.shape[3], nf, self.sched.ncu(), self._stream())

    def _wgrad_first(self, name, dz, h, dil, where):
        with where as ws:
            call("rsu_conv_first_bwd_weight", _ptr(self.in16), _ptr(dz), _ptr(self.g[name + "/kernel"]), _ptr(self.gfirst[dil - 1]),
                 _ptr(self.g[name + "/bias"]), _ptr(ws), self.B, h, h, self.root, dil, self.sched.ncu(), self._stream())

    def _bwd_data(self, name, dz, dx, hin, relu_src=None, accumulate=0, src_index=0, dil=1):
        cout = self.w[name + "/kernel"].shape[3]
        cnt = dx.shape[3]
        ho = hin - 2 * dil
        kws = self.sched.kws_here()
        self._timed("conv3x3_bwd_data", 2.0 * self.B * ho * ho * cout * cnt * 9, "rsu_conv2d_bwd_data_k", _ptr(dz),
                    _ptr(self.pk[name + "/kernel", "bwd", src_index]), _ptr(dx), _ptr(relu_src), accumulate, self.B, hin, hin, cnt, 0, cnt,
                    cout, dil, self.sched.ncu(), _ptr(kws), kws.numel() if kws is not None else 0, self._stream())

    def backward_device(self, inv_count, update=None, dice_scale=None, cldice_scale=None, lovasz_scale=None):
        self._not_averaged("backward_device")
        if update is not None and self.optimizer != "momentum":
            raise _lib.RsuError("backward_device(update=...) is the Momentum step; an %s net steps with apply_%s after the pass"
                                % (self.optimizer, self.optimizer))
        dice_scale = self._dice_weight if dice_scale is None else float(dice_scale)
        if not (math.isfinite(dice_scale) and dice_scale >= 0.0):
            raise _lib.RsuError("dice_scale must be a finite float >= 0, not %r" % (dice_scale,))
        cldice_scale = self._cldice_weight if cldice_scale is None else float(cldice_scale)
        if not (math.isfinite(cldice_scale) and cldice_scale >= 0.0):
            raise _lib.RsuError("cldice_scale must be a finite float >= 0, not %r" % (cldice_scale,))
        lovasz_scale = self._lovasz_weight if lovasz_scale is None else float(lovasz_scale)
        if not (math.isfinite(lovasz_scale) and lovasz_scale >= 0.0):
            raise _lib.RsuError("lovasz_scale must be a finite float >= 0, not %r" % (lovasz_scale,))
        st = self._stream()
        self.sched.begin(self.backward_cu_budget)
        try:
            self._backward_body(inv_count, dice_scale, cldice_scale, lovasz_scale)
        finally:
            self.sched.end()
        inv_keep = float(np.float32(1.0) / np.float32(self.keep))
        gk, gb = self.g["color_space_adjust/kernel"], self.g["color_space_adjust/bias"]
        call("rsu_color_adjust_bwd", _ptr(self.gfirst[0]), _ptr(self.w["conv_0/conv1/kernel"]), _ptr(gk), _ptr(gb), self.root, inv_keep, 0, st)
        if self.dilated and self.L > 1:
            call("rsu_color_adjust_bwd", _ptr(self.gfirst[1]), _ptr(self.w["conv_dilut_0/atrous_conv1/kernel"]), _ptr(gk), _ptr(gb), self.root,
                 inv_keep, 1, st)

    def _backward_body(self, inv_count, dice_scale=0.0, cldice_scale=0.0, lovasz_scale=0.0):
        B, L, st, a, g = self.B, self.L, self._stream(), self.act, self.grad
        keep = self.keep
        last = a[self.last_name]
        self._loss_acc.zero_()
        pixel_w = self._head_pixel_weights()
        if cldice_scale > 0.0 or lovasz_scale > 0.0:
            head = (_ptr(last), _ptr(self.w["weight_output/kernel"]), _ptr(self.w["weight_output/bias"]))
            npix = B * self.P * self.P
            if cldice_scale > 0.0:
                self._cldice_buffers()
            if lovasz_scale > 0.0:
                self._lovasz_buffers()
            if dice_scale > 0.0:
                call("rsu_head_dice_sums", *head, _ptr(self.labels), _ptr(pixel_w), _ptr(self.prob), _ptr(self.dice_sums), _ptr(self.ws), npix,
                     self.root, st)
            else:
                call("rsu_head_fwd", *head, _ptr(self.prob), None, npix, self.root, st)
            if cldice_scale > 0.0:
                self.cldice_sums.zero_()
                self._cldice_fwd(self.cldice_sums)
                call("rsu_cldice_bwd", _ptr(self.prob), _ptr(self.labels), _ptr(self.skel_p), _ptr(self.skel_y), _ptr(self.cldice_sums),
                     self._cldice_iters, cldice_scale, self._cldice_smooth, _ptr(self.gprob), _ptr(self._cldice_ws), B, self.P, self.P, st)
            if lovasz_scale > 0.0:
                self.lovasz_sum.zero_()
                call("rsu_lovasz_fwd_bwd", _ptr(self.prob), _ptr(self.labels), lovasz_scale, 1 if cldice_scale > 0.0 else 0, _ptr(self.gprob),
                     _ptr(self.lovasz_sum), _ptr(self._lovasz_ws), B, self.P, self.P, st)
            call("rsu_head_fwd_bwd_aux", *head, _ptr(self.labels), _ptr(self._class_w_dev), _ptr(pixel_w), self._focal_gamma,
                 _ptr(self.dice_sums) if dice_scale > 0.0 else None, dice_scale, self._dice_smooth, _ptr(self.prob), _ptr(self.loss_sum),
                 _ptr(self.weight_sum), _ptr(g[self.last_name]), _ptr(self.g["weight_output/kernel"]), _ptr(self.g["weight_output/bias"]),
                 _ptr(self.ws), npix, self.root, inv_count, _ptr(self.gprob), st)
        elif self._focal_gamma > 0.0:
            head = (_ptr(last), _ptr(self.w["weight_output/kernel"]), _ptr(self.w["weight_output/bias"]), _ptr(self.labels))
            npix = B * self.P * self.P
            if dice_scale > 0.0:
                call("rsu_head_dice_sums", *head, _ptr(pixel_w), _ptr(self.prob), _ptr(self.dice_sums), _ptr(self.ws), npix, self.root, st)
            call("rsu_head_fwd_bwd_focal", *head, _ptr(self._class_w_dev), _ptr(pixel_w), self._focal_gamma,
                 _ptr(self.dice_sums) if dice_scale > 0.0 else None, dice_scale, self._dice_smooth, _ptr(self.prob), _ptr(self.loss_sum),
                 _ptr(self.weight_sum), _ptr(g[self.last_name]), _ptr(self.g["weight_output/kernel"]), _ptr(self.g["weight_output/bias"]),
                 _ptr(self.ws), npix, self.root, inv_count, st)
        elif dice_scale > 0.0:
            head = (_ptr(last), _ptr(self.w["weight_output/kernel"]), _ptr(self.w["weight_output/bias"]), _ptr(self.labels))
            npix = B * self.P * self.P
            call("rsu_head_dice_sums", *head, _ptr(pixel_w), _ptr(self.prob), _ptr(self.dice_sums), _ptr(self.ws), npix, self.root, st)
            call("rsu_head_fwd_bwd_dice", *head, _ptr(self._class_w_dev), _ptr(pixel_w), _ptr(self.dice_sums), dice_scale,
                 self._dice_smooth, _ptr(self.prob), _ptr(self.loss_sum), _ptr(self.weight_sum), _ptr(g[self.last_name]),
                 _ptr(self.g["weight_output/kernel"]), _ptr(self.g["weight_output/bias"]), _ptr(self.ws), npix, self.root, inv_count, st)
        elif self.loss_is_weighted():
            call("rsu_head_fwd_bwd_w", _ptr(last), _ptr(self.w["weight_output/kernel"]), _ptr(self.w["weight_output/bias"]), _ptr(self.labels),
                 _ptr(self._class_w_dev), _ptr(pixel_w), _ptr(self.prob),
                 _ptr(self.loss_sum), _ptr(self.weight_sum), _ptr(g[self.last_name]), _ptr(self.g["weight_output/kernel"]),
                 _ptr(self.g["weight_output/bias"]), _ptr(self.ws), B * self.P * self.P, self.root, inv_count, st)
        else:
            call("rsu_head_fwd_bwd", _ptr(last), _ptr(self.w["weight_output/kernel"]), _ptr(self.w["weight_output/bias"]), _ptr(self.labels),
                 _ptr(self.prob), _ptr(self.loss_sum), _ptr(g[self.last_name]), _ptr(self.g["weight_output/kernel"]),
                 _ptr(self.g["weight_output/bias"]), _ptr(self.ws), B * self.P * self.P, self.root, inv_count, st)
        for i in reversed(range(L - 1)):
            j, lvl = L + i, L - 2 - i
            c1, c2, up = a["c1_%d" % j], a["c2_%d" % j], a["up_%d" % i]
            h = up.shape[1]
            nf = c2.shape[3]
            dz2, dz1 = g["c2_%d" % j], g["c1_%d" % j]
            self._wgrad("conv_%d/conv2" % j, [(c1, h - 2)], dz2, h - 4, block_done=True)
            self._bwd_data("conv_%d/conv2" % j, dz2, dz1, h - 2, relu_src=c1)
            srcs = [(a["c2_%d" % lvl], h)] + ([(a["d2_%d" % lvl], h)] if self.dilated else []) + [(up, h)]
            self._wgrad("conv_%d/conv1" % j, srcs, dz1, h - 2)
            self._bwd_data("conv_%d/conv1" % j, dz1, g["skip_%d" % i], h, src_index=0)
            if self.dilated:
                self._bwd_data("conv_%d/conv1" % j, dz1, g["skipd_%d" % i], h, src_index=1)
            dup = g["up_%d" % i]
            self._bwd_data("conv_%d/conv1" % j, dz1, dup, h, src_index=2 if self.dilated else 1)
            upin = a["c2_%d" % (j - 1)] if i > 0 else a["c2_%d" % (L - 1)]
            gin = g["c2_%d" % (j - 1)] if i > 0 else g["c2_%d" % (L - 1)]
            if keep < 1.0:
                upin = a["drop_%d" % i]
            hh = h // 2
            self._wgradT(i, upin, dup, hh, nf)
            call("rsu_convT2x2_bwd_data", _ptr(dup), _ptr(self.pk["up_conv_%d/kernel" % i, "bwd"]), _ptr(gin), _ptr(upin), float(np.float32(1.0) / np.float32(keep)), B, hh, hh,
                 upin.shape[3], nf, self.sched.ncu(), st)
            self._grads_ready("up_conv_%d/kernel" % i)
        for i in reversed(range(L)):
            c1, c2 = a["c1_%d" % i], a["c2_%d" % i]
            h = self.level_in[i]
            nf = c2.shape[3]
            dz2, dz1 = g["c2_%d" % i], g["c1_%d" % i]
            if i < L - 1:
                dec = L - 2 - i
                hs = a["up_%d" % dec].shape[1]
                call("rsu_pool_skip_relu_bwd_code", _ptr(c2), _ptr(self.pool_code.get(i)), _ptr(g["pool_%d" % i]), _ptr(g["skip_%d" % dec]), _ptr(dz2), B, h - 4, h - 4, nf, hs, hs,
                     keep, self.dropout_key(i + 1), st)
            self._wgrad("conv_%d/conv2" % i, [(c1, h - 2)], dz2, h - 4, block_done=i > 0 or self.dilated)
            self._bwd_data("conv_%d/conv2" % i, dz2, dz1, h - 2, relu_src=c1)
            if i > 0:
                pin = a["pool_%d" % (i - 1)]
                self._wgrad("conv_%d/conv1" % i, [(pin, h)], dz1, h - 2)
                self._bwd_data("conv_%d/conv1" % i, dz1, g["pool_%d" % (i - 1)], h)
            else:
                alone = not (self.dilated and L > 1)
                self.sched.flush(alone=alone)
                self._wgrad_first("conv_0/conv1", dz1, h, 1, self.sched.tail(alone))
            if self.dilated and i < L - 1:
                d1, d2 = a["d1_%d" % i], a["d2_%d" % i]
                dzd2, dzd1 = g["d2_%d" % i], g["d1_%d" % i]
                dec = L - 2 - i
                hs = a["up_%d" % dec].shape[1]
                call("rsu_pool_skip_relu_bwd", _ptr(d2), None, _ptr(g["skipd_%d" % dec]), _ptr(dzd2), B, h - 8, h - 8, nf, hs, hs, 1.0, 0, st)
                self._wgrad("conv_dilut_%d/atrous_conv2" % i, [(d1, h - 4)], dzd2, h - 8, dil=2, block_done=True)
                self._bwd_data("conv_dilut_%d/atrous_conv2" % i, dzd2, dzd1, h - 4, relu_src=d1, dil=2)
                if i > 0:
                    pin = a["pool_%d" % (i - 1)]
                    self._wgrad("conv_dilut_%d/atrous_conv1" % i, [(pin, h)], dzd1, h - 4, dil=2)
                    self._bwd_data("conv_dilut_%d/atrous_conv1" % i, dzd1, g["pool_%d" % (i - 1)], h, accumulate=1, dil=2)
                else:
                    self._wgrad_first("conv_dilut_0/atrous_conv1", dzd1, h, 2, self.sched.side(alone=True))
            if i > 0:
                first_name = ("conv_dilut_%d/atrous_conv1/kernel" if (self.dilated and i < L - 1) else "conv_%d/conv1/kernel") % i
                self._grads_ready(first_name)
        self.sched.flush(alone=True)
        self.sched.join()

    def tune(self, training=None, keep=1.0):
        lib = _lib.lib()
        training = self.training if training is None else (training and self.training)
        keep = float(keep)
        self._tuned.add((bool(training), self.backward_cu_budget, keep < 1.0))
        if lib.rsu_get_autotune() == _lib.TUNE_OFF or os.environ.get("RSU_AUTOTUNE", "1") == "0":
            return
        x0, l0 = self.x.clone(), self.labels.clone()
        g = torch.Generator(device="cpu").manual_seed(12345)
        self.x.copy_(torch.rand(tuple(self.x.shape), generator=g))
        self.labels.copy_((torch.rand(tuple(self.labels.shape), generator=g) < 0.2).to(torch.int64))
        on_grads, self.on_grads = self.on_grads, None
        prof, self.prof = self.prof, None
        call("rsu_set_autotune", _lib.TUNE_MEASURE)
        try:
            self.forward_device(keep=keep)
            if training:
                self.backward_device(1.0 / (self.B * self.P * self.P))
            if self.device.type == "cuda":
                torch.cuda.synchronize(self.device)
        finally:
            call("rsu_set_autotune", _lib.TUNE_LOOKUP)
            self.on_grads, self.prof = on_grads, prof
            self.x.copy_(x0)
            self.labels.copy_(l0)
# ... 28 lines not shown
```

Baseline: 892.4 patches/s.

## Store ReLU positivity as bitmasks in forward and use them in backward-data

The forward conv1 kernels (first conv, pp and fwd2 paths) now also write one bit per output channel recording whether the bf16 ReLU output is positive. Backward-data for conv2 reads that packed bitmask instead of the full bf16 c1 activation to apply the ReLU derivative, which cuts mask-read traffic by 16x. The cost is extra byte-sized stores in the forward epilogue, small uncoalesced byte loads in the backward epilogue, and more kernel template variants. A fallback to the old path remains when the bits were not written.

Result: slower. 873.9 patches/s (-2.1%).

```diff
diff --git a/include/rsu_relu_bits.h b/include/rsu_relu_bits.h
--- /dev/null
+++ b/include/rsu_relu_bits.h
@@ -0,0 +1,26 @@
+#ifndef RSU_RELU_BITS_H_
+#define RSU_RELU_BITS_H_
+
+#include "rsu.h"
+
+#ifdef __cplusplus
+extern "C" {
+#endif
+
+size_t rsu_relu_bits_bytes(int N, int H, int W, int C);
+int rsu_conv2d_fwd_bits_k(const rsu_src_t* srcs, int nsrc, const void* packed_fwd, const float* bias, void* y, void* bits_out,
+                          int* wrote_bits, int N, int Hin, int Win, int Cout, int dil, int relu, int ncu, float* kws, size_t kws_floats,
+                          rsu_stream_t stream);
+int rsu_conv_first_fwd_bits(const void* in16, const void* packed, const float* b, void* y, void* bits_out, int* wrote_bits, int N,
+                            int H, int W, int Cout, int dil, int ncu, rsu_stream_t stream);
+int rsu_conv2d_bwd_data_bits(const void* dz, const void* packed_bwd, void* dx, const void* relu_src, const void* relu_bits,
+                             int accumulate, int N, int H, int W, int Cin_total, int ci_off, int ci_cnt, int Cout, int dil, int ncu,
+                             rsu_stream_t stream);
+int rsu_conv2d_bwd_data_bits_k(const void* dz, const void* packed_bwd, void* dx, const void* relu_src, const void* relu_bits,
+                               int accumulate, int N, int H, int W, int Cin_total, int ci_off, int ci_cnt, int Cout, int dil, int ncu,
+                               float* kws, size_t kws_floats, rsu_stream_t stream);
+
+#ifdef __cplusplus
+}
+#endif
+#endif
diff --git a/road_segmentation_unet_amd/_lib.py b/road_segmentation_unet_amd/_lib.py
--- a/road_segmentation_unet_amd/_lib.py
+++ b/road_segmentation_unet_amd/_lib.py
@@ -176,6 +176,14 @@
     "rsu_distance_hist": (_i, [_vp, _f, _vp, _vp, _vp, _i, _i, _i, _vp]),
 }
 
+SIGNATURES_RELU_BITS = {
+    "rsu_relu_bits_bytes": (_sz, [_i, _i, _i, _i]),
+    "rsu_conv2d_fwd_bits_k": (_i, [_PS, _i, _vp, _vp, _vp, _vp, _PI, _i, _i, _i, _i, _i, _i, _i, _vp, _sz, _vp]),
+    "rsu_conv_first_fwd_bits": (_i, [_vp, _vp, _vp, _vp, _vp, _PI, _i, _i, _i, _i, _i, _i, _vp]),
+    "rsu_conv2d_bwd_data_bits": (_i, [_vp, _vp, _vp, _vp, _vp, _i, _i, _i, _i, _i, _i, _i, _i, _i, _i, _vp]),
+    "rsu_conv2d_bwd_data_bits_k": (_i, [_vp, _vp, _vp, _vp, _vp, _i, _i, _i, _i, _i, _i, _i, _i, _i, _i, _vp, _sz, _vp]),
+}
+
 _lib = None
 
 
@@ -192,7 +200,7 @@
         L = ctypes.CDLL(LIB_PATH)
         for name, (res, args) in list(SIGNATURES.items()) + list(SIGNATURES_OPTIM.items()) + list(SIGNATURES_LOSS.items()) \
                 + list(SIGNATURES_CLDICE.items()) + list(SIGNATURES_LOVASZ.items()) + list(SIGNATURES_COMPONENTS.items()) \
-                + list(SIGNATURES_DISTANCE.items()):
+                + list(SIGNATURES_DISTANCE.items()) + list(SIGNATURES_RELU_BITS.items()):
             fn = getattr(L, name)
             fn.restype = res
             fn.argtypes = args
diff --git a/road_segmentation_unet_amd/csrc/conv_first.hip b/road_segmentation_unet_amd/csrc/conv_first.hip
--- a/road_segmentation_unet_amd/csrc/conv_first.hip
+++ b/road_segmentation_unet_amd/csrc/conv_first.hip
@@ -15,6 +15,7 @@
     const bf16_t* wp;
     const float* bias;
     bf16_t* y;
+    unsigned char* bits;
     int N, H, W, Ho, Wo, Cout, dil, relu, ntiles_w;
     int ntx;
     unsigned ntx_magic, ho_magic;
@@ -24,7 +25,7 @@
 #ifndef CF_TRS
 #define CF_TRS 1
 #endif
-template <bool FUSED>
+template <bool FUSED, bool BITS = false>
 __global__ void __launch_bounds__(256) __attribute__((amdgpu_waves_per_eu(3))) k_conv_first_fwd(const ConvFirstParams p) {
 #if CF_TRS
     __shared__ __attribute__((aligned(16))) char trs[4 * 2048];
@@ -35,6 +36,7 @@
     const int cb = blockIdx.y;
     const __amdgpu_buffer_rsrc_t rin = __builtin_amdgcn_make_buffer_rsrc((void*)p.in16, 0, (int)((long)p.N * p.H * p.W * 32), 0x00020000);
     const __amdgpu_buffer_rsrc_t rout = __builtin_amdgcn_make_buffer_rsrc((void*)p.y, 0, 0x7fffffff, 0x00020000);
+    const __amdgpu_buffer_rsrc_t rbits = __builtin_amdgcn_make_buffer_rsrc((void*)((BITS && p.bits) ? (void*)p.bits : (void*)p.y), 0, 0x7fffffff, 0x00020000);
     bf16x8 fa[5][4];
 #pragma unroll
     for (int j = 0; j < 5; ++j) {
@@ -156,6 +158,7 @@
                 const bool ok = (x0 + P < p.Wo) && (cb * 64 + q8 * 8 < p.Cout);
                 const unsigned vo = ok ? (unsigned)((P * p.Cout + q8 * 8) * 2) : 0x80000000u;
                 asm volatile("s_waitcnt lgkmcnt(0)\n\ts_nop 4\n\tbuffer_store_dwordx4 %0, %1, %2, %3 offen\n\ts_nop 3" ::"v"(r), "v"(vo), "s"(rout), "s"(sbase) : "memory");
+                if (BITS && p.bits) __builtin_amdgcn_raw_buffer_store_b8((unsigned char)relu_bits_of8(r), rbits, relu_bits_voff(vo), sbase >> 4, 0);
             }
         }
 #else
@@ -171,6 +174,7 @@
             const bool cok = cb * 64 + pp * 32 + 8 * g4 < p.Cout;
             const unsigned vo = (pok && cok) ? (unsigned)((l15 * p.Cout + pp * 32 + 8 * g4) * 2) : 0x80000000u;
             asm volatile("s_nop 4\n\tbuffer_store_dwordx4 %0, %1, %2, %3 offen\n\ts_nop 3" ::"v"(r), "v"(vo), "s"(rout), "s"(sbase) : "memory");
+            if (BITS && p.bits) __builtin_amdgcn_raw_buffer_store_b8((unsigned char)relu_bits_of8(r), rbits, relu_bits_voff(vo), sbase >> 4, 0);
         }
 #endif
         if (!more) break;
@@ -183,9 +187,10 @@
 static unsigned floor_magic(int d) { return d <= 1 ? 0xffffffffu : (unsigned)(0x100000000ull / (unsigned)d); }
 
 hipError_t conv_first_fwd_launch(const void* in16, const void* wp, int ntiles_w, const float* bias, void* y, int N, int H, int W, int Cout, int dil,
-                                 int relu, int ncu, hipStream_t st, const float* x, const float* cw, const float* cb) {
+                                 int relu, int ncu, hipStream_t st, const float* x, const float* cw, const float* cb, void* bits_out) {
     ConvFirstParams p;
-    p.x = x; p.cw = cw; p.cb = cb;
+    if (bits_out && ((Cout % 32) || x)) return hipErrorInvalidValue;
+    p.x = x; p.cw = cw; p.cb = cb; p.bits = (unsigned char*)bits_out;
     p.in16 = (const bf16_t*)in16; p.wp = (const bf16_t*)wp; p.bias = bias; p.y = (bf16_t*)y;
     p.N = N; p.H = H; p.W = W; p.Ho = H - 2 * dil; p.Wo = W - 2 * dil; p.Cout = Cout; p.dil = dil; p.relu = relu; p.ntiles_w = ntiles_w;
     p.ntx = (p.Wo + 15) / 16;
@@ -197,6 +202,7 @@
     long blocks = (long)ncu * 3;
     if (blocks * 4 > np) blocks = (np + 3) / 4;
     if (x) hipLaunchKernelGGL(k_conv_first_fwd<true>, dim3((unsigned)blocks, (unsigned)((Cout + 63) / 64)), dim3(256), 0, st, p);
+    else if (p.bits) hipLaunchKernelGGL((k_conv_first_fwd<false, true>), dim3((unsigned)blocks, (unsigned)((Cout + 63) / 64)), dim3(256), 0, st, p);
     else hipLaunchKernelGGL(k_conv_first_fwd<false>, dim3((unsigned)blocks, (unsigned)((Cout + 63) / 64)), dim3(256), 0, st, p);
     return hipGetLastError();
 }
diff --git a/road_segmentation_unet_amd/csrc/igemm.h b/road_segmentation_unet_amd/csrc/igemm.h
--- a/road_segmentation_unet_amd/csrc/igemm.h
+++ b/road_segmentation_unet_amd/csrc/igemm.h
@@ -18,6 +18,8 @@
     const float* bias;
     bf16_t* out;
     const bf16_t* mask_src;
+    const unsigned char* mask_bits;
+    unsigned char* bits_out;
     bf16_t* pool_out;
     unsigned char* pool_code;
     const void* zero_page;
@@ -74,7 +76,8 @@
 bool igemm_ct_supports(int mode, int N, int H, int W, int Ca, int Cn);
 hipError_t igemm_ct_launch(int mode, const IgCtParams& p, int grid_x, hipStream_t st);
 hipError_t conv_first_fwd_launch(const void* in16, const void* wp, int ntiles_w, const float* bias, void* y, int N, int H, int W, int Cout, int dil,
-                                 int relu, int ncu, hipStream_t st, const float* x = nullptr, const float* cw = nullptr, const float* cb = nullptr);
+                                 int relu, int ncu, hipStream_t st, const float* x = nullptr, const float* cw = nullptr, const float* cb = nullptr,
+                                 void* bits_out = nullptr);
 
 struct IgWgradParams {
     const bf16_t* F;
diff --git a/road_segmentation_unet_amd/csrc/igemm_fwd2.hip b/road_segmentation_unet_amd/csrc/igemm_fwd2.hip
--- a/road_segmentation_unet_amd/csrc/igemm_fwd2.hip
+++ b/road_segmentation_unet_amd/csrc/igemm_fwd2.hip
@@ -20,7 +20,7 @@
 }
 #define RSU_SENT 0x80000000u
 
-template <int WCO, int WPX, int CT, int PT, int NTAP, int KW, int TPS, int NA, int NAB, int DWS>
+template <int WCO, int WPX, int CT, int PT, int NTAP, int KW, int TPS, int NA, int NAB, int DWS, bool MBITS = false>
 __global__ void __launch_bounds__(WCO* WPX * 64) __attribute__((amdgpu_waves_per_eu(WCO* WPX / 4, WCO* WPX / 4)))
 igemm_fwd2_kernel(const IgFwdParams p) {
     constexpr int NW = WCO * WPX;
@@ -202,6 +202,8 @@
         const __amdgpu_buffer_rsrc_t orsrc = mk(p.out);
         const __amdgpu_buffer_rsrc_t mrsrc = mk(p.mask_src ? (const void*)p.mask_src : (const void*)p.out);
         const unsigned sbase = out_sbase(T);
+        const __amdgpu_buffer_rsrc_t brsrc = mk((MBITS && p.mask_bits) ? (const void*)p.mask_bits : (const void*)p.out);
+        const unsigned bbase = sbase >> 4;
         if (!p.accumulate) {
             typedef __attribute__((ext_vector_type(2))) short s2;
             const short fl = p.relu ? (short)0 : (short)-32768;
@@ -213,10 +215,12 @@
             for (int b0 = 0; b0 < NST; b0 += MB) {
                 unsigned voffs[MB];
                 u32x4 mk4[MB];
+                unsigned mb[MB];
 #pragma unroll
                 for (int e = 0; e < MB; ++e) {
                     voffs[e] = out_voff(T, b0 + e);
                     if (p.mask_src) mk4[e] = __builtin_amdgcn_raw_buffer_load_b128(mrsrc, voffs[e], sbase, 0);
+                    if (MBITS && p.mask_bits) mb[e] = __builtin_amdgcn_raw_buffer_load_b8(brsrc, relu_bits_voff(voffs[e]), bbase, 0);
                 }
 #pragma unroll
                 for (int e = 0; e < MB; ++e) {
@@ -233,9 +237,13 @@
 #pragma unroll
                             for (int i = 0; i < 4; ++i) r[i] &= pos_mask_pk_bf16(mk4[e][i], ones_pk);
                     }
+                    if (MBITS && p.mask_bits) {
+#pragma unroll
+                        for (int i = 0; i < 4; ++i) r[i] &= relu_bits_mask2(mb[e], i);
+                    }
                     asm volatile("buffer_store_dwordx4 %0, %1, %2, %3 offen\n\ts_nop 3" ::"v"(r), "v"(voffs[e]), "s"(orsrc), "s"(sbase) : "memory");
                 }
-                if (p.mask_src) __builtin_amdgcn_sched_barrier(0);
+                if (p.mask_src || (MBITS && p.mask_bits)) __builtin_amdgcn_sched_barrier(0);
             }
             return;
         }
@@ -245,10 +253,12 @@
         for (int b0 = 0; b0 < NST; b0 += EB) {
             unsigned voffs[EB];
             u32x4 mk4[EB], ob4[EB];
+            unsigned mb[EB];
 #pragma unroll
             for (int e = 0; e < EB; ++e) {
                 voffs[e] = out_voff(T, b0 + e);
                 if (p.mask_src) mk4[e] = __builtin_amdgcn_raw_buffer_load_b128(mrsrc, voffs[e], sbase, 0);
+                if (MBITS && p.mask_bits) mb[e] = __builtin_amdgcn_raw_buffer_load_b8(brsrc, relu_bits_voff(voffs[e]), bbase, 0);
                 if (p.accumulate) ob4[e] = __builtin_amdgcn_raw_buffer_load_b128(orsrc, voffs[e], sbase, 0);
             }
 #pragma unroll
@@ -266,6 +276,11 @@
                         if (!(bf_lo(mk4[e][i]) > 0.f)) v[2 * i] = 0.f;
                         if (!(bf_hi(mk4[e][i]) > 0.f)) v[2 * i + 1] = 0.f;
                     }
+                }
+                if (MBITS && p.mask_bits) {
+#pragma unroll
+                    for (int i = 0; i < 8; ++i)
+                        if (!((mb[e] >> i) & 1u)) v[i] = 0.f;
                 }
                 if (p.accumulate) {
 #pragma unroll
@@ -494,12 +509,12 @@
     return (size_t)(dws + 1) * tps * (ci.TN / 16) * 1024 + (size_t)nab * npix_max * 64 + 1024 + 512;
 }
 
-template <int CFG, int NTAP, int KW>
+template <int CFG, int NTAP, int KW, bool MBITS = false>
 static hipError_t launch2_one(const IgFwdParams& p, int gx, int gy, hipStream_t st) {
     using C = Fwd2Cfg<CFG>;
     constexpr int TN = C::WCO * C::CT * 16;
     constexpr int TPS = tps2_for(TN, NTAP);
-    auto kern = igemm_fwd2_kernel<C::WCO, C::WPX, C::CT, C::PT, NTAP, KW, TPS, C::na(NTAP), nab_for(TN, NTAP), dws_for(TN, NTAP, C::PT)>;
+    auto kern = igemm_fwd2_kernel<C::WCO, C::WPX, C::CT, C::PT, NTAP, KW, TPS, C::na(NTAP), nab_for(TN, NTAP), dws_for(TN, NTAP, C::PT), MBITS>;
     const size_t lds = igemm_fwd2_lds_bytes(CFG, NTAP, p.g.npix_max);
     static size_t lds_set = 0;
     if (lds > lds_set) {
@@ -513,7 +528,7 @@
 template <int CFG>
 static hipError_t launch2_cfg(int ntap, const IgFwdParams& p, int gx, int gy, hipStream_t st) {
     switch (ntap) {
-        case 9: return launch2_one<CFG, 9, 3>(p, gx, gy, st);
+        case 9: return p.mask_bits ? launch2_one<CFG, 9, 3, true>(p, gx, gy, st) : launch2_one<CFG, 9, 3>(p, gx, gy, st);
         case 4: return launch2_one<CFG, 4, 2>(p, gx, gy, st);
         case 1: return launch2_one<CFG, 1, 1>(p, gx, gy, st);
     }
diff --git a/road_segmentation_unet_amd/csrc/igemm_pp.hip b/road_segmentation_unet_amd/csrc/igemm_pp.hip
--- a/road_segmentation_unet_amd/csrc/igemm_pp.hip
+++ b/road_segmentation_unet_amd/csrc/igemm_pp.hip
@@ -41,7 +41,8 @@
     return n;
 }
 }
-template <int WCO, int WPX, int CT, int PT, int LSW, int NAW, int WP0, bool STAMP, bool DBG, bool POOLK = false, bool KS = false, int DIL = PP_DIL>
+template <int WCO, int WPX, int CT, int PT, int LSW, int NAW, int WP0, bool STAMP, bool DBG, bool POOLK = false, bool KS = false, int DIL = PP_DIL,
+          bool BITS = false>
 __global__ void __launch_bounds__(512) __attribute__((amdgpu_waves_per_eu(2, 2)))
 igemm_pp_kernel(const IgFwdParams p) {
     constexpr int NW = 8, NG = 4, KW = 3, TPS = 3;
@@ -319,6 +320,7 @@
         ovoff[pt] = (unsigned)(((ty * p.oW + tx) * p.outC + 8 * g4) * 2);
     }
     const bool co_inside = cob * TN + TN <= p.Cout;
+    const bool wbits_fly = BITS && DIL == 1 && p.bits_out && !p.mask_bits;
     constexpr bool POOL_OK = POOLK && ((PT == 4 && (LSW == 4 || LSW == 5)) || (PT == 2 && LSW == 4));
     auto pool_body = [&](const Tile& T, f32x4(&acc)[CT][PT], const unsigned (&voffs)[NST], const __amdgpu_buffer_rsrc_t orsrc, const unsigned sbase)
                          __attribute__((always_inline)) {
@@ -430,8 +432,11 @@
                     for (int e = 0; e < NST; ++e) voffs[e] = out_voff(T, e, ql15, qg4);
                 }
             };
-            auto body = [&](const bool MASK) __attribute__((always_inline)) {
-                const bool TRS = MASK;
+            auto body = [&](const int MODE) __attribute__((always_inline)) {
+                const bool MASK = MODE == 1, MBITS = MODE == 2, WBITS = MODE == 3;
+                const bool TRS = MASK || MBITS;
+                const __amdgpu_buffer_rsrc_t brsrc = mk(MBITS ? (const void*)p.mask_bits : (WBITS ? (const void*)p.bits_out : (const void*)p.out));
+                const unsigned bbase = sbase >> 4;
                 const int tr_src = (((lane & 3) << 4) | (lane >> 2)) << 2;
                 fill_voffs(TRS);
                 seg_end(6);
@@ -443,6 +448,12 @@
                     for (int e = 0; e < NST; ++e)
                         asm volatile("buffer_load_dwordx4 %0, %1, %2, %3 offen" : "=&v"(mk4[e]) : "v"(voffs[e]), "s"(mrsrc), "s"(sbase) : "memory");
                 }
+                unsigned mb[NST];
+                if (MBITS) {
+#pragma unroll
+                    for (int e = 0; e < NST; ++e)
+                        asm volatile("s_nop 4\n\tbuffer_load_ubyte %0, %1, %2, %3 offen" : "=&v"(mb[e]) : "v"(relu_bits_voff(voffs[e])), "s"(brsrc), "s"(bbase) : "memory");
+                }
                 const int LA = TRS ? (NST < 8 ? NST : 8) : 1;
                 u32x4 rr[NST];
                 auto pack = [&](const int e) __attribute__((always_inline)) {
@@ -471,6 +482,11 @@
 #pragma unroll
                             for (int k = 0; k < NST; ++k) asm volatile("" : "+v"(mk4[k]));
                         }
+                        if (MBITS) {
+                            asm volatile("s_waitcnt vmcnt(0)" ::: "memory");
+#pragma unroll
+                            for (int k = 0; k < NST; ++k) asm volatile("" : "+v"(mb[k]));
+                        }
                     } else if (e + LA - 1 < NST) {
                         pack(e + LA - 1);
                     }
@@ -483,10 +499,18 @@
 #pragma unroll
                         for (int i = 0; i < 4; ++i) r[i] &= pos_mask_pk_bf16(mk4[e][i], ones_pk);
                     }
+                    if (MBITS) {
+#pragma unroll
+                        for (int i = 0; i < 4; ++i) r[i] &= relu_bits_mask2(mb[e], i);
+                    }
                     if (DBG && (p.dbg & 512)) {
                         asm volatile("" ::"v"(r));
                     } else {
                         PP_STORE(r, voffs[e]);
+                    }
+                    if (WBITS) {
+                        const unsigned b = relu_bits_of8(r);
+                        asm volatile("s_nop 4\n\tbuffer_store_byte %0, %1, %2, %3 offen\n\ts_nop 3" ::"v"(b), "v"(relu_bits_voff(voffs[e])), "s"(brsrc), "s"(bbase) : "memory");
                     }
                 }
             };
@@ -497,7 +521,12 @@
                     return;
                 }
             }
-            if (p.mask_src) body(true); else body(false);
+            if constexpr (BITS) {
+                if (p.mask_bits) body(2);
+                else if constexpr (DIL == 1) body(3);
+            } else {
+                if (p.mask_src) body(1); else body(0);
+            }
             return;
         }
     };
@@ -591,7 +620,8 @@
             seg_end(4);
             if constexpr (G == 1) {
                 if (J == 0 && after_epi) {
-                    RSU_WAIT_VMCNT(pp_na(NAW, 1, J) + WP1 + NST);
+                    if (wbits_fly) RSU_WAIT_VMCNT(pp_na(NAW, 1, J) + WP1 + 2 * NST);
+                    else RSU_WAIT_VMCNT(pp_na(NAW, 1, J) + WP1 + NST);
                 } else {
                     RSU_WAIT_VMCNT(pp_na(NAW, 1, J) + WP1);
                 }
@@ -618,7 +648,8 @@
             __builtin_amdgcn_sched_barrier(0);
             if constexpr (G == 0) {
                 if (J == 0 && after_epi) {
-                    RSU_WAIT_VMCNT(pp_na(NAW, 0, J) + WP0 + NST);
+                    if (wbits_fly) RSU_WAIT_VMCNT(pp_na(NAW, 0, J) + WP0 + 2 * NST);
+                    else RSU_WAIT_VMCNT(pp_na(NAW, 0, J) + WP0 + NST);
                 } else if (J == 2) {
                     RSU_WAIT_VMCNT(WP0);
                 } else {
@@ -731,6 +762,8 @@
     int nstrips, tiles_per_strip;
     bf16_t* out;
     const bf16_t* mask_src;
+    const unsigned char* mask_bits;
+    unsigned char* bits_out;
     int Ho, Wo, oH, oW, outC, Cout, relu;
 };
 __global__ void __launch_bounds__(256) k_pp_splitk_finish(const PpFinishParams q) {
@@ -774,7 +807,13 @@
 #pragma unroll
         for (int i = 0; i < 4; ++i) v[i] &= pos_mask_pk_bf16(m[i]);
     }
+    if (q.mask_bits) {
+        const unsigned b = q.mask_bits[off >> 3];
+#pragma unroll
+        for (int i = 0; i < 4; ++i) v[i] &= relu_bits_mask2(b, i);
+    }
     *(u32x4*)(q.out + off) = v;
+    if (q.bits_out) q.bits_out[off >> 3] = (unsigned char)relu_bits_of8(v);
 }
 
 #endif
@@ -786,9 +825,9 @@
 template <> struct PpCfg<IGF2_CFG_64x256> { static constexpr int WCO = 1, WPX = 8, CT = 4, PT = 2, NAS = PP_NAS(0, 2, 3, 1, 2), WP0 = 0; };
 template <> struct PpCfg<IGF2_CFG_128x192> { static constexpr int WCO = 2, WPX = 4, CT = 4, PT = 3, NAS = PP_NAS(0, 2, 3, 1, 2), WP0 = 2; };
 template <> struct PpCfg<IGF2_CFG_64x384> { static constexpr int WCO = 1, WPX = 8, CT = 4, PT = 3, NAS = PP_NAS(0, 3, 3, 2, 2), WP0 = 0; };
-template <int WCO, int WPX, int CT, int PT, int LSW, int NAS, int WP0, bool STAMP, bool DBG, bool POOLK = false, bool KS = false>
+template <int WCO, int WPX, int CT, int PT, int LSW, int NAS, int WP0, bool STAMP, bool DBG, bool POOLK = false, bool KS = false, bool BITS = false>
 static hipError_t pp_launch_kernel3(int cfg, const IgFwdParams& p, int gx, hipStream_t st) {
-    auto kern = igemm_pp_kernel<WCO, WPX, CT, PT, LSW, NAS, WP0, STAMP, DBG, POOLK, KS, PP_DIL>;
+    auto kern = igemm_pp_kernel<WCO, WPX, CT, PT, LSW, NAS, WP0, STAMP, DBG, POOLK, KS, PP_DIL, BITS>;
     const size_t lds = igemm_fwd2_lds_bytes(cfg, 9, p.g.npix_max) + (STAMP ? 8 * PP_NSTAMP * 4 : 0);
     static size_t lds_set = 0;
     if (lds > lds_set) {
@@ -811,6 +850,9 @@
             return pp_launch_kernel3<WCO, WPX, CT, PT, LSW, NAS, WP0, false, false, false, true>(cfg, p, gx, st);
         }
         return hipErrorInvalidValue;
+    }
+    if constexpr (!STAMP && !DBG) {
+        if (p.mask_bits || (PP_DIL == 1 && p.bits_out)) return pp_launch_kernel3<WCO, WPX, CT, PT, LSW, NAS, WP0, false, false, false, false, true>(cfg, p, gx, st);
     }
     return pp_launch_kernel3<WCO, WPX, CT, PT, LSW, NAS, WP0, STAMP, DBG, false>(cfg, p, gx, st);
 }
@@ -920,7 +962,7 @@
     q.nslots = p.N * p.g.nstrips * p.g.tiles_per_strip * p.ncob; q.ncob = p.ncob;
     q.lsw = p.lsw; q.TR = (q.WPX * q.PT * 16) >> p.lsw;
     q.nstrips = p.g.nstrips; q.tiles_per_strip = p.g.tiles_per_strip;
-    q.out = p.out; q.mask_src = p.mask_src;
+    q.out = p.out; q.mask_src = p.mask_src; q.mask_bits = p.mask_bits; q.bits_out = p.bits_out;
     q.Ho = p.Ho; q.Wo = p.Wo; q.oH = p.oH; q.oW = p.oW; q.outC = p.outC; q.Cout = p.Cout; q.relu = p.relu;
     const long threads = (long)q.nslots * 8 * (q.CT / 2) * q.PT * 64;
     hipLaunchKernelGGL(k_pp_splitk_finish, dim3((unsigned)((threads + 255) / 256)), dim3(256), 0, st, q);
diff --git a/road_segmentation_unet_amd/csrc/rsu_api.hip b/road_segmentation_unet_amd/csrc/rsu_api.hip
--- a/road_segmentation_unet_amd/csrc/rsu_api.hip
+++ b/road_segmentation_unet_amd/csrc/rsu_api.hip
@@ -16,6 +16,7 @@
 #include "../../include/rsu_lovasz.h"
 #include "../../include/rsu_components.h"
 #include "../../include/rsu_distance.h"
+#include "../../include/rsu_relu_bits.h"
 #include "affine_patches.h"
 #include "color_jitter.h"
 #include "border_map.h"
@@ -584,8 +585,9 @@
     return false;
 }
 
-static hipError_t launch_persistent(int pp, int cfg, int ntap, const IgFwdParams& p, int gx, int gy, hipStream_t st) {
+static hipError_t launch_persistent(int pp, int cfg, int ntap, const IgFwdParams& p, int gx, int gy, hipStream_t st, int* wrote_bits = nullptr) {
     if (pp && pp_supports(cfg, p)) {
+        if (wrote_bits && p.bits_out && p.dil == 1 && !p.pool_out) *wrote_bits = 1;
         hipError_t e = p.dil == 2 ? igemm_pp_d2_launch(cfg, p, gx, st) : igemm_pp_launch(cfg, p, gx, st);
         if (e == hipSuccess && p.ksplit > 1) e = igemm_pp_finish_launch(cfg, p, st);
         return e;
@@ -597,8 +599,12 @@
 static int run_fwd(const rsu_src_t* srcs, int nsrc, const void* wp, long wp_y_stride, int ntiles_w, int tile_off, const float* bias,
                    void* out, const void* mask_src, int N, int Hin, int Win, int Ho, int Wo, int Cout, int outC, int ntap, int kw,
                    int dil, int stride, int pad, int oH, int oW, int ostride, int gy, int relu, int accumulate, int ncu_arg, hipStream_t st,
-                   void* pool_out = nullptr, void* pool_code = nullptr, float* kws = nullptr, size_t kws_floats = 0) {
+                   void* pool_out = nullptr, void* pool_code = nullptr, float* kws = nullptr, size_t kws_floats = 0,
+                   const void* mask_bits = nullptr, void* bits_out = nullptr, int* wrote_bits = nullptr) {
     const int kh = ntap / kw;
+    if (wrote_bits) *wrote_bits = 0;
+    if (mask_bits && (mask_src || outC % 32 || ostride != 1 || gy != 1)) return RSU_EINVAL;
+    if (bits_out && (outC % 32 || ostride != 1 || gy != 1 || pool_out || accumulate)) bits_out = nullptr;
     const bool pool = pool_out != nullptr;
     const int ncu = launch_ncu(ncu_arg);
     if (ncu < 0) return RSU_EINVAL;
@@ -615,7 +621,8 @@
     const int tune_mode = env_int("RSU_AUTOTUNE", 1) != 0 ? g_autotune.load() : RSU_TUNE_OFF;
     const bool tunable = env_cfg < 0 && !accumulate && tune_mode != RSU_TUNE_OFF;
     std::array<int, 16> tkey = {N, Ho, Wo, Cout, outC, ntap, kw, dil, stride, pad, gy, ktot, nsrc,
-                                (mask_src ? 1 : 0) | (relu ? 2 : 0) | (bias ? 4 : 0) | (pool ? 8 : 0) | (pool_code ? 16 : 0), ostride, ncu * 8 + gen};
+                                (mask_src ? 1 : 0) | (relu ? 2 : 0) | (bias ? 4 : 0) | (pool ? 8 : 0) | (pool_code ? 16 : 0) | (mask_bits ? 32 : 0) | (bits_out ? 64 : 0),
+                                ostride, ncu * 8 + gen};
     int tuned_cfg = -1, tuned_pp = -1;
     if (!kws || accumulate) kws_floats = 0;
     Fwd2Plan pls;
@@ -663,6 +670,8 @@
     p.bias = bias;
     p.out = (bf16_t*)out;
     p.mask_src = (const bf16_t*)mask_src;
+    p.mask_bits = (const unsigned char*)mask_bits;
+    p.bits_out = (unsigned char*)bits_out;
     p.pool_out = (bf16_t*)pool_out;
     p.pool_code = (unsigned char*)pool_code;
     p.zero_page = zero_page();
@@ -728,11 +737,11 @@
                 for (int vpp = 0; vpp < 2; ++vpp) {
                     if (vpp == 1 && !(pp_ok && !accumulate && pp_supports(cfg, pt))) continue;
                     if (vpp == 0 && pool) continue;
-                    if (!vpp && gen >= 4 && pp_ok && !accumulate && pp_supports(cfg, pt)) continue;
+                    if (!vpp && (gen >= 4 || mask_bits || bits_out) && pp_ok && !accumulate && pp_supports(cfg, pt)) continue;
                     float ms_min = 1e30f;
                     for (int rep = 0; rep < 6; ++rep) {
                         HIP_CHECK_RET(hipEventRecord(e0, st));
-                        HIP_CHECK_RET(launch_persistent(vpp, pc.cfg, ntap, pt, pc.grid_x, gy, st));
+                        HIP_CHECK_RET(launch_persistent(vpp, pc.cfg, ntap, pt, pc.grid_x, gy, st, wrote_bits));
                         HIP_CHECK_RET(hipEventRecord(e1, st));
                         HIP_CHECK_RET(hipEventSynchronize(e1));
                         float ms = 0.f;
@@ -754,7 +763,7 @@
             g_tuned[tkey] = best_cfg;
             return RSU_OK;
         }
-        HIP_CHECK_RET(launch_persistent(pp, pl2.cfg, ntap, p, pl2.grid_x, gy, st));
+        HIP_CHECK_RET(launch_persistent(pp, pl2.cfg, ntap, p, pl2.grid_x, gy, st, wrote_bits));
         return RSU_OK;
     }
 }
@@ -762,11 +771,21 @@
 extern "C" size_t rsu_conv_splitk_ws_floats(void) { return (size_t)256 * 128 * 256 + 1024; }
 extern "C" int rsu_conv2d_fwd_k(const rsu_src_t* srcs, int nsrc, const void* packed_fwd, const float* bias, void* y, int N, int Hin,
                                 int Win, int Cout, int dil, int relu, int ncu, float* kws, size_t kws_floats, rsu_stream_t stream) {
-    if (!srcs || nsrc < 1 || nsrc > 3 || !packed_fwd || !y || Cout % 8 || (dil != 1 && dil != 2)) return RSU_EINVAL;
+    return rsu_conv2d_fwd_bits_k(srcs, nsrc, packed_fwd, bias, y, nullptr, nullptr, N, Hin, Win, Cout, dil, relu, ncu, kws, kws_floats, stream);
+}
+extern "C" size_t rsu_relu_bits_bytes(int N, int H, int W, int C) {
+    if (N < 1 || H < 1 || W < 1 || C < 1) return 0;
+    return (size_t)N * H * W * (size_t)cdiv(C, 32) * 4;
+}
+extern "C" int rsu_conv2d_fwd_bits_k(const rsu_src_t* srcs, int nsrc, const void* packed_fwd, const float* bias, void* y, void* bits_out,
+                                     int* wrote_bits, int N, int Hin, int Win, int Cout, int dil, int relu, int ncu, float* kws,
+                                     size_t kws_floats, rsu_stream_t stream) {
+    if (wrote_bits) *wrote_bits = 0;
+    if (!srcs || nsrc < 1 || nsrc > 3 || !packed_fwd || !y || Cout % 8 || (dil != 1 && dil != 2) || (bits_out && !wrote_bits)) return RSU_EINVAL;
     const int Ho = Hin - 2 * dil, Wo = Win - 2 * dil;
     if (Ho < 1 || Wo < 2) return RSU_EINVAL;
     return run_fwd(srcs, nsrc, packed_fwd, 0, rup(Cout, 128) / 16, 0, bias, y, nullptr, N, Hin, Win, Ho, Wo, Cout, Cout, 9, 3, dil, 1, 0,
-                   Ho, Wo, 1, 1, relu, 0, ncu, (hipStream_t)stream, nullptr, nullptr, kws, kws_floats);
+                   Ho, Wo, 1, 1, relu, 0, ncu, (hipStream_t)stream, nullptr, nullptr, kws, kws_floats, nullptr, bits_out, wrote_bits);
 }
 extern "C" int rsu_conv2d_fwd(const rsu_src_t* srcs, int nsrc, const void* packed_fwd, const float* bias, void* y, int N, int Hin,
                               int Win, int Cout, int dil, int relu, int ncu, rsu_stream_t stream) {
@@ -819,7 +838,12 @@
 }
 extern "C" int rsu_conv_first_fwd(const void* in16, const void* packed, const float* b, void* y, int N, int H, int W, int Cout, int dil,
                                   int ncu, rsu_stream_t stream) {
-    if (!in16 || !packed || !y || Cout % 8 || H <= 2 * dil || W <= 2 * dil + 1 || (dil != 1 && dil != 2)) return RSU_EINVAL;
+    return rsu_conv_first_fwd_bits(in16, packed, b, y, nullptr, nullptr, N, H, W, Cout, dil, ncu, stream);
+}
+extern "C" int rsu_conv_first_fwd_bits(const void* in16, const void* packed, const float* b, void* y, void* bits_out, int* wrote_bits, int N,
+                                       int H, int W, int Cout, int dil, int ncu, rsu_stream_t stream) {
+    if (wrote_bits) *wrote_bits = 0;
+    if (!in16 || !packed || !y || Cout % 8 || H <= 2 * dil || W <= 2 * dil + 1 || (dil != 1 && dil != 2) || (bits_out && !wrote_bits)) return RSU_EINVAL;
     rsu_src_t s;
     s.ptr = in16; s.H = H; s.W = W; s.C = 16; s.oy = 0; s.ox = 0;
     const int Ho = H - 2 * dil, Wo = W - 2 * dil;
@@ -827,11 +851,14 @@
         const int n = launch_ncu(ncu);
         if (n < 0) return RSU_EINVAL;
         if ((long)N * Ho * Wo * Cout * 2 >= 0x7ffffff0L || (long)N * H * W * 32 >= 0x7ffffff0L) return RSU_E2BIG;
-        HIP_CHECK_RET(conv_first_fwd_launch(in16, packed, rup(Cout, 128) / 16, b, y, N, H, W, Cout, dil, 1, n, (hipStream_t)stream));
+        const bool wb = bits_out && Cout % 32 == 0;
+        HIP_CHECK_RET(conv_first_fwd_launch(in16, packed, rup(Cout, 128) / 16, b, y, N, H, W, Cout, dil, 1, n, (hipStream_t)stream, nullptr, nullptr, nullptr,
+                                            wb ? bits_out : nullptr));
+        if (wb) *wrote_bits = 1;
         return RSU_OK;
     }
     return run_fwd(&s, 1, packed, 0, rup(Cout, 128) / 16, 0, b, y, nullptr, N, H, W, Ho, Wo, Cout, Cout, 9, 3, dil, 1, 0, Ho, Wo, 1, 1, 1, 0,
-                   ncu, (hipStream_t)stream);
+                   ncu, (hipStream_t)stream, nullptr, nullptr, nullptr, 0, nullptr, bits_out, wrote_bits);
 }
 
 extern "C" int rsu_color_conv_first_fwd(const float* x, const float* w0, const float* b0, const void* packed, const float* b, void* y, int N, int H,
@@ -853,14 +880,26 @@
 }
 extern "C" int rsu_conv2d_bwd_data_k(const void* dz, const void* packed_bwd, void* dx, const void* relu_src, int accumulate, int N, int H,
                                      int W, int Cin_total, int ci_off, int ci_cnt, int Cout, int dil, int ncu, float* kws, size_t kws_floats, rsu_stream_t stream) {
+    return rsu_conv2d_bwd_data_bits_k(dz, packed_bwd, dx, relu_src, nullptr, accumulate, N, H, W, Cin_total, ci_off, ci_cnt, Cout, dil, ncu, kws, kws_floats,
+                                      stream);
+}
+extern "C" int rsu_conv2d_bwd_data_bits(const void* dz, const void* packed_bwd, void* dx, const void* relu_src, const void* relu_bits, int accumulate,
+                                        int N, int H, int W, int Cin_total, int ci_off, int ci_cnt, int Cout, int dil, int ncu, rsu_stream_t stream) {
+    return rsu_conv2d_bwd_data_bits_k(dz, packed_bwd, dx, relu_src, relu_bits, accumulate, N, H, W, Cin_total, ci_off, ci_cnt, Cout, dil, ncu, nullptr, 0,
+                                      stream);
+}
+extern "C" int rsu_conv2d_bwd_data_bits_k(const void* dz, const void* packed_bwd, void* dx, const void* relu_src, const void* relu_bits, int accumulate,
+                                          int N, int H, int W, int Cin_total, int ci_off, int ci_cnt, int Cout, int dil, int ncu, float* kws,
+                                          size_t kws_floats, rsu_stream_t stream) {
     if (!dz || !packed_bwd || !dx || Cout % 8 || ci_cnt % 8 || ci_off % 32 || ci_off + ci_cnt > Cin_total || (dil != 1 && dil != 2))
         return RSU_EINVAL;
+    if (relu_bits && (relu_src || ci_cnt % 32)) return RSU_EINVAL;
     const int Hd = H - 2 * dil, Wd = W - 2 * dil;
     if (Hd < 1 || Wd < 1 || W < 2) return RSU_EINVAL;
     rsu_src_t s;
     s.ptr = dz; s.H = Hd; s.W = Wd; s.C = Cout; s.oy = 0; s.ox = 0;
     return run_fwd(&s, 1, packed_bwd, 0, rup(Cin_total, 128) / 16, ci_off / 16, nullptr, dx, relu_src, N, Hd, Wd, H, W, ci_cnt, ci_cnt, 9,
-                   3, dil, 1, 2 * dil, H, W, 1, 1, 0, accumulate, ncu, (hipStream_t)stream, nullptr, nullptr, kws, kws_floats);
+                   3, dil, 1, 2 * dil, H, W, 1, 1, 0, accumulate, ncu, (hipStream_t)stream, nullptr, nullptr, kws, kws_floats, relu_bits);
 }
 
 static unsigned magic_floor32(int d) { return d <= 1 ? 0xffffffffu : (unsigned)(0x100000000ull / (unsigned)d); }
diff --git a/road_segmentation_unet_amd/csrc/rsu_common.h b/road_segmentation_unet_amd/csrc/rsu_common.h
--- a/road_segmentation_unet_amd/csrc/rsu_common.h
+++ b/road_segmentation_unet_amd/csrc/rsu_common.h
@@ -46,6 +46,18 @@
     return t;
 }
 
+__device__ __forceinline__ unsigned relu_bits_of8(const u32x4 r) {
+    unsigned x = 0;
+#pragma unroll
+    for (int i = 0; i < 4; ++i) x |= pos_mask_pk_bf16(r[i]) & ((1u << (2 * i)) | (1u << (17 + 2 * i)));
+    return x | (x >> 16);
+}
+__device__ __forceinline__ unsigned relu_bits_mask2(unsigned b, int i) {
+    const unsigned lo = (unsigned)((int)(b << (31 - 2 * i)) >> 31), hi = (unsigned)((int)(b << (30 - 2 * i)) >> 31);
+    return __builtin_amdgcn_perm(hi, lo, 0x05040100u);
+}
+__device__ __forceinline__ unsigned relu_bits_voff(unsigned v) { return (unsigned)((int)v >> 4); }
+
 __device__ __forceinline__ void mfma_bf16_inplace(f32x4& acc, const bf16x8& a, const bf16x8& b) {
     asm volatile("v_mfma_f32_16x16x32_bf16 %0, %1, %2, %0" : "+v"(acc) : "v"(a), "v"(b));
 }
diff --git a/road_segmentation_unet_amd/hostio.py b/road_segmentation_unet_amd/hostio.py
--- a/road_segmentation_unet_amd/hostio.py
+++ b/road_segmentation_unet_amd/hostio.py
@@ -985,3 +985,25 @@
     f1 = 2.0 * precision * recall / (precision + recall) if precision + recall > 0.0 else 0.0
     return {"relaxed_precision": precision, "relaxed_recall": recall, "relaxed_f1": f1, "mean_dist_pred": mean[0], "mean_dist_true": mean[1],
             "far_pred": far[0], "far_true": far[1]}
+
+
+def relu_bits_pack(x):
+    x = np.asarray(x)
+    if x.ndim != 4 or x.shape[3] < 1:
+        raise ValueError("relu_bits_pack: an [N][H][W][C] tensor is needed")
+    if x.dtype in (np.uint16, np.int16):
+        pat = x.view(np.uint16)
+    elif x.dtype == np.float32:
+        u = np.ascontiguousarray(x).view(np.uint32)
+        if np.any(u & 0xffff):
+            raise ValueError("relu_bits_pack: float32 values that are no bf16 values")
+        pat = (u >> 16).astype(np.uint16)
+    else:
+        raise ValueError("relu_bits_pack: float32, uint16 or int16 data is needed")
+    pos = ((pat & 0x8000) == 0) & (pat != 0)
+    N, H, W, C = pos.shape
+    nw = (C + 31) // 32
+    padded = np.zeros((N, H, W, nw * 32), dtype=np.uint64)
+    padded[..., :C] = pos
+    weights = (np.uint64(1) << np.arange(32, dtype=np.uint64))
+    return (padded.reshape(N, H, W, nw, 32) * weights).sum(axis=4).astype(np.uint32)
diff --git a/road_segmentation_unet_amd/unet.py b/road_segmentation_unet_amd/unet.py
--- a/road_segmentation_unet_amd/unet.py
+++ b/road_segmentation_unet_amd/unet.py
@@ -80,7 +80,7 @@
     def __init__(self, num_layers, root_size, dilated_layers, batch_size, patch_size, device="cuda:0", params=None, seed=2017,
                  training=True, optimizer="momentum", class_weights=None, dice_weight=0.0, dice_smooth=1.0, border_weight=0.0, border_sigma=5.0,
                  clip_grad_norm=None, ema_decay=None, ema_warmup=True, accumulate_steps=None, weight_decay=None, weight_decay_mode="decoupled",
-                 focal_gamma=0.0, cldice_weight=0.0, cldice_iters=10, cldice_smooth=1.0, lovasz_weight=0.0):
+                 focal_gamma=0.0, cldice_weight=0.0, cldice_iters=10, cldice_smooth=1.0, lovasz_weight=0.0, relu_bits=True):
         self._init_optimizer(training, optimizer, clip_grad_norm, ema_decay, ema_warmup, accumulate_steps, weight_decay, weight_decay_mode)
         assert root_size % 8 == 0 and (root_size // 8) & (root_size // 8 - 1) == 0, "root_size must be 8 * 2^k for the HIP path"
         self.L, self.root, self.dilated = num_layers, root_size, bool(dilated_layers)
@@ -90,6 +90,8 @@
         if self.device.type == "cuda":
             torch.cuda.set_device(self.device)
         self.training = training
+        self.relu_bits = bool(relu_bits)
+        self.act_bits, self._bits_ok = {}, {}
         self.class_weights = class_weights
         self.pixel_weights = None
         self.dice_weight, self.dice_smooth = dice_weight, dice_smooth
@@ -424,6 +426,11 @@
             if self.border_weight > 0.0:
                 self.border_map = torch.zeros((B, self.P, self.P), dtype=torch.float32, device=dev)
                 self._border_ws = torch.zeros(int(lib.rsu_border_map_ws_bytes(B, self.P, self.P)) // 4, dtype=torch.int32, device=dev)
+            if self.root % 32 == 0:
+                for k, t in self.act.items():
+                    if k.startswith("c1_"):
+                        assert int(lib.rsu_relu_bits_bytes(*t.shape)) == t.numel() // 8
+                        self.act_bits[k] = torch.zeros(t.shape[:3] + (t.shape[3] // 32,), dtype=torch.int32, device=dev)
             if os.environ.get("RSU_POOL_CODE", "1") == "1":
                 for i in range(L - 1):
                     self.pool_code[i] = torch.zeros(self.act["pool_%d" % i].shape, dtype=torch.uint8, device=dev)
@@ -509,18 +516,34 @@
             self.sched.flush()
             self.on_grads(self._slices[name][0])
 
-    def _conv(self, name, srcs, hin, out, dil=1):
+    def _note_bits(self, key, wrote, first):
+        self._bits_ok[key] = bool(wrote.value) and (first or self._bits_ok.get(key, False))
+
+    def _conv(self, name, srcs, hin, out, dil=1, bits=None, bits_key=None, first=True):
         arr = (RsuSrc * len(srcs))(*srcs)
         cout = out.shape[3]
         cin = sum(s.C for s in srcs)
         ho = hin - 2 * dil
         kws = self.sched.kws_here()
         nb = out.shape[0]
+        if bits is not None:
+            wrote = ctypes.c_int(0)
+            self._timed("conv3x3_fwd", 2.0 * nb * ho * ho * cout * cin * 9, "rsu_conv2d_fwd_bits_k", arr, len(srcs),
+                        _ptr(self.pk[name + "/kernel", "fwd"]), _ptr(self.w[name + "/bias"]), _ptr(out), _ptr(bits), ctypes.byref(wrote), nb, hin, hin,
+                        cout, dil, 1, self.sched.ncu(), _ptr(kws), kws.numel() if kws is not None else 0, self._stream())
+            self._note_bits(bits_key, wrote, first)
+            return
         self._timed("conv3x3_fwd", 2.0 * nb * ho * ho * cout * cin * 9, "rsu_conv2d_fwd_k", arr, len(srcs),
                     _ptr(self.pk[name + "/kernel", "fwd"]), _ptr(self.w[name + "/bias"]), _ptr(out), nb, hin, hin, cout, dil, 1,
                     self.sched.ncu(), _ptr(kws), kws.numel() if kws is not None else 0, self._stream())
 
-    def _conv_first(self, name, out, h, dil, st, in16=None, x=None):
+    def _conv_first(self, name, out, h, dil, st, in16=None, x=None, bits=None, bits_key=None, first=True):
+        if x is None and bits is not None:
+            wrote = ctypes.c_int(0)
+            call("rsu_conv_first_fwd_bits", _ptr(self.in16 if in16 is None else in16), _ptr(self.pk[name + "/kernel", "fwd"]), _ptr(self.w[name + "/bias"]),
+                 _ptr(out), _ptr(bits), ctypes.byref(wrote), out.shape[0], h, h, self.root, dil, self.sched.ncu(), st)
+            self._note_bits(bits_key, wrote, first)
+            return
         if x is not None:
             call("rsu_color_conv_first_fwd", _ptr(x), _ptr(self.w["color_space_adjust/kernel"]), _ptr(self.w["color_space_adjust/bias"]),
                  _ptr(self.pk[name + "/kernel", "fwd"]), _ptr(self.w[name + "/bias"]), _ptr(out), out.shape[0], h, h, self.root, dil,
@@ -549,6 +572,7 @@
         a = {k: t[b0:b0 + nb] for k, t in self.act.items()}
         x, in16, prob, logits = self.x[b0:b0 + nb], self.in16[b0:b0 + nb], self.prob[b0:b0 + nb], self.logits[b0:b0 + nb]
         code = {k: t[b0:b0 + nb] for k, t in self.pool_code.items()}
+        bits = lambda k: self.act_bits[k][b0:b0 + nb] if (self.relu_bits and k in self.act_bits) else None
         steps = []
 
         def add(f):
@@ -571,9 +595,10 @@
                         self._conv("conv_dilut_%d/atrous_conv2" % i, [_src(a["d1_%d" % i], h - 4, h - 4)], h - 4, a["d2_%d" % i], dil=2)
                 add(twin)
             if i == 0:
-                add(lambda h=h: self._conv_first("conv_0/conv1", a["c1_0"], h, 1, self._stream(), in16, xin))
+                add(lambda h=h: self._conv_first("conv_0/conv1", a["c1_0"], h, 1, self._stream(), in16, xin, bits("c1_0"), "c1_0", b0 == 0))
             else:
-                add(lambda i=i, cur=cur, h=h: self._conv("conv_%d/conv1" % i, [_src(cur, h, h)], h, a["c1_%d" % i]))
+                add(lambda i=i, cur=cur, h=h: self._conv("conv_%d/conv1" % i, [_src(cur, h, h)], h, a["c1_%d" % i], bits=bits("c1_%d" % i),
+                                                         bits_key="c1_%d" % i, first=b0 == 0))
             if last:
                 add(lambda i=i, h=h: self._conv("conv_%d/conv2" % i, [_src(a["c1_%d" % i], h - 2, h - 2)], h - 2, a["c2_%d" % i]))
             else:
@@ -609,7 +634,7 @@
                 if self.dilated:
                     srcs.append(_src(a["d2_%d" % lvl], h, h))
                 srcs.append(_src(up, h, h))
-                self._conv("conv_%d/conv1" % j, srcs, h, a["c1_%d" % j])
+                self._conv("conv_%d/conv1" % j, srcs, h, a["c1_%d" % j], bits=bits("c1_%d" % j), bits_key="c1_%d" % j, first=b0 == 0)
             add(dec)
             add(lambda j=j, h=h: self._conv("conv_%d/conv2" % j, [_src(a["c1_%d" % j], h - 2, h - 2)], h - 2, a["c2_%d" % j]))
             net, h = a["c2_%d" % j], h - 4
@@ -686,11 +711,16 @@
             call("rsu_conv_first_bwd_weight", _ptr(self.in16), _ptr(dz), _ptr(self.g[name + "/kernel"]), _ptr(self.gfirst[dil - 1]),
                  _ptr(self.g[name + "/bias"]), _ptr(ws), self.B, h, h, self.root, dil, self.sched.ncu(), self._stream())
 
-    def _bwd_data(self, name, dz, dx, hin, relu_src=None, accumulate=0, src_index=0, dil=1):
+    def _bwd_data(self, name, dz, dx, hin, relu_src=None, accumulate=0, src_index=0, dil=1, bits_key=None):
         cout = self.w[name + "/kernel"].shape[3]
         cnt = dx.shape[3]
         ho = hin - 2 * dil
         kws = self.sched.kws_here()
+        if self.relu_bits and relu_src is not None and self._bits_ok.get(bits_key, False):
+            self._timed("conv3x3_bwd_data", 2.0 * self.B * ho * ho * cout * cnt * 9, "rsu_conv2d_bwd_data_bits_k", _ptr(dz),
+                        _ptr(self.pk[name + "/kernel", "bwd", src_index]), _ptr(dx), None, _ptr(self.act_bits[bits_key]), accumulate, self.B, hin, hin,
+                        cnt, 0, cnt, cout, dil, self.sched.ncu(), _ptr(kws), kws.numel() if kws is not None else 0, self._stream())
+            return
         self._timed("conv3x3_bwd_data", 2.0 * self.B * ho * ho * cout * cnt * 9, "rsu_conv2d_bwd_data_k", _ptr(dz),
                     _ptr(self.pk[name + "/kernel", "bwd", src_index]), _ptr(dx), _ptr(relu_src), accumulate, self.B, hin, hin, cnt, 0, cnt,
                     cout, dil, self.sched.ncu(), _ptr(kws), kws.numel() if kws is not None else 0, self._stream())
@@ -785,7 +815,7 @@
             nf = c2.shape[3]
             dz2, dz1 = g["c2_%d" % j], g["c1_%d" % j]
             self._wgrad("conv_%d/conv2" % j, [(c1, h - 2)], dz2, h - 4, block_done=True)
-            self._bwd_data("conv_%d/conv2" % j, dz2, dz1, h - 2, relu_src=c1)
+            self._bwd_data("conv_%d/conv2" % j, dz2, dz1, h - 2, relu_src=c1, bits_key="c1_%d" % j)
             srcs = [(a["c2_%d" % lvl], h)] + ([(a["d2_%d" % lvl], h)] if self.dilated else []) + [(up, h)]
             self._wgrad("conv_%d/conv1" % j, srcs, dz1, h - 2)
             self._bwd_data("conv_%d/conv1" % j, dz1, g["skip_%d" % i], h, src_index=0)
@@ -813,7 +843,7 @@
                 call("rsu_pool_skip_relu_bwd_code", _ptr(c2), _ptr(self.pool_code.get(i)), _ptr(g["pool_%d" % i]), _ptr(g["skip_%d" % dec]), _ptr(dz2), B, h - 4, h - 4, nf, hs, hs,
                      keep, self.dropout_key(i + 1), st)
             self._wgrad("conv_%d/conv2" % i, [(c1, h - 2)], dz2, h - 4, block_done=i > 0 or self.dilated)
-            self._bwd_data("conv_%d/conv2" % i, dz2, dz1, h - 2, relu_src=c1)
+            self._bwd_data("conv_%d/conv2" % i, dz2, dz1, h - 2, relu_src=c1, bits_key="c1_%d" % i)
             if i > 0:
                 pin = a["pool_%d" % (i - 1)]
                 self._wgrad("conv_%d/conv1" % i, [(pin, h)], dz1, h - 2)
```
